# zamling/PSALM

Measured on AMD Instinct MI355X. Metric: images/sec at 1024x1024 COCO-panoptic inference, higher is better.
Workload: dtype f16x3; 1 GPU; BASELINE.json configs[1]: COCO-panoptic 1024x1024 batch=1 per GPU, PSALM (Swin-B + Phi-1.5 24L + Mask2Former head), 134 class prompts, 100 queries, full semantic+instance+panoptic post-processing; parallelism=image-sharded x1 (replicated weights, RCCL broadcast at init), launch=hipGraph replay (one graph per input signature)

## Files before the change

include/psalm_hip.h:

```cpp
#ifndef PSALM_HIP_H
#define PSALM_HIP_H
#include <stdint.h>
#ifdef __cplusplus
extern "C" {
#endif

#define PSALM_F32 0
#define PSALM_BF16 1

const char* psalm_last_error(void);
#define PSALM_ABI_VERSION 15
int psalm_abi_version(void);
const char* psalm_backend(void);

#define PSALM_TUNE_GEMM_XCD_KSPLIT 0
#define PSALM_TUNE_ATTN_XCD_HEADS 1
#define PSALM_TUNE_GEMM_MID 2
#define PSALM_TUNE_DECODER_FUSE 3
#define PSALM_TUNE_ROW_GROUPS 4
#define PSALM_TUNE_MHA_QTILE_WAVES 5
#define PSALM_TUNE_COUNT 8
int psalm_set_tuning(int key, int value);
int psalm_get_tuning(int key);

int psalm_msda_forward(const void* value, int value_dtype, const int64_t* spatial_shapes_host,
                       const int64_t* level_start_host, const float* sampling_loc, const float* attn_weight, void* out,
                       int out_dtype, int B, int S, int M, int D, int L, int Lq, int P, void* stream);
int psalm_msda_forward_dev(const void* value, int value_dtype, const int64_t* spatial_shapes_dev, const int64_t* level_start_dev,
                           const float* sampling_loc, const float* attn_weight, void* out, int out_dtype, int B, int S, int M, int D,
                           int L, int Lq, int P, void* stream);


int psalm_msda_fused(const void* value, int value_dtype, const int64_t* spatial_shapes_host,
                     const int64_t* level_start_host, const float* offsets_logits, void* out, int out_dtype, int B, int S,
                     int M, int D, int L, int P, void* stream);
int psalm_msda_set_policy(int v);


int psalm_gemm(const void* A, int a_dtype, long lda, const void* W, int w_dtype, long ldw, const float* bias,
               const void* residual, long ldr, void* C, int c_dtype, long ldc, int M, int N, int K, int act,
               int act_col_start, void* workspace, long workspace_bytes, void* stream);

int psalm_gemm_ln(const void* A, int a_dtype, long lda, const void* W, int w_dtype, long ldw, const float* bias,
                  const void* residual, long ldr, void* C, int c_dtype, long ldc, int M, int N, int K, int act, int act_col_start,
                  const float* ln_gamma, const float* ln_beta, float ln_eps, void* ln_out, int ln_dtype, long ld_ln, void* workspace,
                  long workspace_bytes, void* stream);
int psalm_conv2d_nhwc(const void* x, int B, int H, int W, int Cin, const void* Wt, int Cout, int ksize, int stride, int pad,
                      const float* bias, const void* residual, long ldr, void* out, int c_dtype, long ldc, int act,
                      const void* zeros, void* workspace, long workspace_bytes, void* stream);
int psalm_split_f16(const float* x, long ldx, void* out, long ldo, float* inv_scale, int rows, int K, void* stream);
int psalm_gemm_x3_set_products(int n);
int psalm_im2col_split_f16(const float* x, void* out, float* inv_scale, int B, int H, int W, int C, int k, int stride, int pad, void* stream);
int psalm_layernorm_split(const float* x, long ldx, float* y, long ldy, const float* gamma, const float* beta, int rows, int C, float eps,
                          void* split1, float* inv1, const float* add, long add_rows, void* split2, float* inv2, void* stream);
int psalm_swin_window_gather_split(const float* x, void* out, float* inv_out, const float* gamma, const float* beta, int B, int H, int W, int C,
                                   int ws, int shift, float eps, void* stream);
int psalm_swin_window_merge_ln_split(const float* win, const float* shortcut, float* out_x, void* h_split, float* h_inv, const float* gamma,
                                     const float* beta, int B, int H, int W, int C, int ws, int shift, float eps, void* stream);
int psalm_gemm_x3(const void* A2, long lda, const float* a_scale, const void* W2, long ldw, const float* w_scale, int Kp,
                  const float* bias, const void* residual, long ldr, void* C, long ldc, int M, int N, int act, int act_col_start,
                  void* workspace, long workspace_bytes, void* stream);
int psalm_gemm_x3_ln_split(const void* A2, long lda, const float* a_scale, const void* W2, long ldw, const float* w_scale, int Kp,
                           const float* bias, const void* residual, long ldr, void* C, long ldc, int M, int N, const float* ln_gamma,
                           const float* ln_beta, float ln_eps, void* ln_out, long ld_ln, void* split_out, float* split_inv,
                           void* workspace, long workspace_bytes, void* stream);
int psalm_gemm_x3_split(const void* A2, long lda, const float* a_scale, const void* W2, long ldw, const float* w_scale, int Kp,
                        const float* bias, void* C, long ldc, int M, int N, int act, int act_col_start, void* split_out, long ld_split,
                        int split_kp, int split_col_off, int split_col_start, int paired, float* split_inv, const float* bound_par,
                        int global_rows, void* workspace, long workspace_bytes, void* stream);

int psalm_image_preprocess(const unsigned char* img, int H, int W, float* out, unsigned char* pad_mask, int S, int nh, int nw,
                           const int* bounds_h, const int* kk_h, int ksize_h, const int* bounds_v, const int* kk_v, int ksize_v,
                           unsigned char* tmp, const float* mean3_host, const float* std3_host, void* stream);

int psalm_semantic_labels(const float* sem, int* labels, int C, long HW, void* stream);
int psalm_confusion_accumulate(const int* pred, const int* gt, long n, int num_classes, int ignore_label, long long* conf, void* stream);
int psalm_panoptic_rgb(const int* ids, unsigned char* rgb, long n, void* stream);
int psalm_mask_rle_count(const void* masks, int dtype_is_u8, int n, int H, int W, int* col_cnt, int* col_off, int* total, void* stream);
int psalm_mask_rle_emit(const void* masks, int dtype_is_u8, int n, int H, int W, const int* col_off, const long* base, int* out, void* stream);
int psalm_iou_counts(const void* pred, int pred_is_u8, const unsigned char* tgt, const int* pred_idx, const int* tgt_idx, int npairs, long HW,
                     long long* counts_zeroed, void* stream);
int psalm_fuse_masks(const void* masks, int dtype_is_u8, const float* scores, int n, long HW, float thr, unsigned char* out, void* stream);

long psalm_mha_attention_f32_workspace(int B, int heads, int Lq, int Lk);
int psalm_mha_attention_f32(const float* q, long ldq, const float* k, long ldk, const float* v, long ldv, float* out, long ldo,
                            const unsigned char* mask, const unsigned char* row_all_masked, void* workspace, int B, int Lq, int Lk, int heads,
                            int head_dim, void* stream);
long psalm_mha_attention_f32_shared_workspace(int B, int heads, int Lq, int Lk);
int psalm_mha_attention_f32_shared(const float* q, long ldq, const float* k, long ldk, const float* v, long ldv, float* out, long ldo,
                                   const unsigned char* mask, const unsigned char* row_all_masked, void* workspace, int B, int Lq, int Lk,
                                   int heads, int head_dim, void* stream);

long psalm_causal_attention_f32_workspace(int B, int L, int heads);
int psalm_causal_attention_f32(const float* qkv, long ld, int q_off, int k_off, int v_off, float* out, long ldo, int o_off,
                               const float* cos_table, const float* sin_table, const unsigned char* key_mask, void* workspace, int B, int L,
                               int heads, int head_dim, int rot, void* stream);
int psalm_causal_attention_f32_split(const float* qkv, long ld, int q_off, int k_off, int v_off, void* split_out, long ld_split, int split_kp,
                                     int split_col_off, const float* split_inv, const float* cos_table, const float* sin_table,
                                     const unsigned char* key_mask, void* workspace, int B, int L, int heads, int head_dim, int rot,
                                     void* stream);

long psalm_causal_attention_f32_prefix_workspace(int N, int S, int heads);
int psalm_causal_attention_f32_prefix(const float* qkv, long ld, int q_off, int k_off, int v_off, const float* k_cache, const float* v_cache,
                                      long ldv, float* out, long ldo, int o_off, const float* cos_table, const float* sin_table,
                                      const unsigned char* key_mask, void* workspace, int N, int S, int P, int heads, int head_dim, int rot,
                                      void* stream);
int psalm_causal_attention_f32_prefix_split(const float* qkv, long ld, int q_off, int k_off, int v_off, const float* k_cache,
                                            const float* v_cache, long ldv, void* split_out, long ld_split, int split_kp, int split_col_off,
                                            const float* split_inv, const float* cos_table, const float* sin_table,
                                            const unsigned char* key_mask, void* workspace, int N, int S, int P, int heads, int head_dim,
                                            int rot, void* stream);
typedef struct {
    const float* k_cache;
    const float* v_cache;
    long ldv;
    int P;
    int pad;
} psalm_prefix_ref;
long psalm_causal_attention_f32_prefix_grouped_workspace(int N, int S, int heads);
int psalm_causal_attention_f32_prefix_grouped(const float* qkv, long ld, int q_off, int k_off, int v_off, const psalm_prefix_ref* refs, int P_max,
                                              float* out, long ldo, int o_off, const float* cos_table, const float* sin_table,
                                              const unsigned char* key_mask, void* workspace, int N, int S, int heads, int head_dim, int rot,
                                              void* stream);
int psalm_causal_attention_f32_prefix_grouped_split(const float* qkv, long ld, int q_off, int k_off, int v_off, const psalm_prefix_ref* refs,
                                                    int P_max, void* split_out, long ld_split, int split_kp, int split_col_off,
                                                    const float* split_inv, const float* cos_table, const float* sin_table,
                                                    const unsigned char* key_mask, void* workspace, int N, int S, int heads, int head_dim,
                                                    int rot, void* stream);
int psalm_phi_prefix_kv_store(const float* qkv, long ld, int k_off, int v_off, const float* cos_table, const float* sin_table, float* k_cache,
                              float* v_cache, long ldv, int P, int heads, int head_dim, int rot, void* stream);

int psalm_memset_zero(void* p, long bytes, void* stream);
int psalm_copy_d2d(void* dst, const void* src, long bytes, void* stream);
int psalm_cast_i32_i64(const int* src, long long* dst, long n, void* stream);
const char* psalm_gemm_last_kernel(void);
int psalm_gemm_describe(int M, int N, int K, int a_dtype, int w_dtype, long workspace_bytes, int* out4);
int psalm_gemm_set_tile_policy(int bm);

int psalm_layernorm(const void* x, int x_dtype, long ldx, void* y, int y_dtype, long ldy, void* y2_bf16, long ldy2,
                    const float* gamma, const float* beta, int rows, int C, float eps, void* stream);
int psalm_layernorm3(const void* x, int x_dtype, long ldx, void* y, int y_dtype, long ldy, void* y2_bf16, long ldy2, const float* add,
                     long add_rows, void* y3_bf16, long ldy3, const float* gamma, const float* beta, int rows, int C, float eps,
                     void* stream);
int psalm_layernorm_chain(const float* x, long ldx, float* y1, long ldy1, const float* g1, const float* b1, const float* add, long add_rows,
                          float* y2, long ldy2, const float* g2, const float* b2, float* y3, long ldy3, int rows, int C, float eps, void* stream);
int psalm_gemm_f32_pair(const float* A0, const float* W0, const float* bias0, float* C0, int M0, int N0, int K0, int act0, const float* A1,
                        const float* W1, const float* bias1, float* C1, int M1, int N1, int K1, int act1, void* stream);
int psalm_gemm_f32_rows(const float* A, long lda, const float* W, long ldw, const float* bias, const float* residual, long ldr, float* C, long ldc,
                        int M, int N, int K, int act, void* stream);
int psalm_gemm_f32_rows_pair(const float* A0, const float* W0, const float* bias0, float* C0, int M0, int N0, int K0, int act0, const float* A1,
                             const float* W1, const float* bias1, float* C1, int M1, int N1, int K1, int act1, void* stream);
int psalm_gemm_f32_grouped(const float* const* A_host, const float* const* W_host, float* const* C_host, const int* M_host, const int* N_host, int K,
                           int count, void* stream);
int psalm_swin_window_gather(const void* x, int x_dtype, void* out, int out_dtype, const float* gamma,
                             const float* beta, int B, int H, int W, int C, int ws, int shift, float eps, void* stream);
int psalm_swin_window_merge(const void* win, int win_dtype, const void* shortcut, void* out, int x_dtype, int B, int H,
                            int W, int C, int ws, int shift, void* stream);
int psalm_swin_window_merge_ln(const void* win, int win_dtype, const float* shortcut, float* out_x, void* out_h, int h_dtype,
                               const float* gamma, const float* beta, int B, int H, int W, int C, int ws, int shift, float eps,
                               void* stream);
int psalm_patch_merge_ln(const void* x, int x_dtype, void* out, int out_dtype, const float* gamma, const float* beta,
                         int B, int H, int W, int C, float eps, void* stream);
int psalm_groupnorm_nhwc(const void* x, int x_dtype, void* y, int y_dtype, const float* gamma, const float* beta,
                         float* workspace, int B, int HW, int C, int G, float eps, int relu, void* stream);
int psalm_add_bcast(const void* a, int a_dtype, const void* b, int b_dtype, void* out, int out_dtype, long rows, int C,
                    long b_rows, void* stream);
int psalm_gather_rows(const void* src0, int dt0, const void* src1, int dt1, const void* src2, int dt2, const void* src3,
                      int dt3, const int* src_id, const int* src_row, void* dst, int dst_dtype, long rows, int C,
                      void* stream);
int psalm_segment_mean(const void* x, int x_dtype, long ldx, const int* seg_offsets, const int* seg_rows, void* out,
                       int out_dtype, int nseg, int C, void* stream);

int psalm_window_attention(const void* qkv, const float* bias_table, void* out, int dtype, int B, int nWh, int nWw, int C,
                           int heads, int ws, int shift, void* stream);
int psalm_window_attention_split(const float* qkv, const float* bias_table, const float* a_inv, const float* bound_par, void* split_out,
                                 int split_kp, float* split_inv, int B, int nWh, int nWw, int C, int heads, int ws, int shift, void* stream);
int psalm_window_attention_mfma(const void* qkv, const float* bias_table, void* out, int B, int nWh, int nWw, int C, int heads,
                                int ws, int shift, void* stream);
int psalm_causal_attention(const void* qkv, int dtype, long ld, int q_off, int k_off, int v_off, void* out, long ldo,
                           int o_off, const float* cos_table, const float* sin_table, const unsigned char* key_mask, int B,
                           int L, int heads, int head_dim, int rot, void* stream);
long psalm_causal_attention_mfma_workspace(int B, int L, int heads);
int psalm_causal_attention_mfma(const void* qkv, long ld, int q_off, int k_off, int v_off, void* out, long ldo, int o_off,
                                const float* cos_table, const float* sin_table, const unsigned char* key_mask,
                                void* workspace, int B, int L, int heads, int head_dim, int rot, void* stream);
int psalm_mha_attention(const void* q, long ldq, const void* k, long ldk, const void* v, long ldv, void* out, long ldo,
                        int dtype, const unsigned char* mask, const unsigned char* row_all_masked, int B, int Lq, int Lk,
                        int heads, int head_dim, void* stream);
long psalm_mha_attention_mfma_workspace(int B, int heads, int Lk);
int psalm_mha_attention_mfma(const void* q, long ldq, const void* k, long ldk, const void* vt, long ldvt, void* out, long ldo,
                             const unsigned char* mask, const unsigned char* row_all_masked, void* workspace, int B, int Lq,
                             int Lk, int heads, int head_dim, void* stream);
int psalm_attn_mask(const float* masks, unsigned char* out, unsigned char* row_all_masked, int BQ, int h, int w, int Ht,
                    int Wt, void* stream);

int psalm_patch_im2col(const float* img, void* out, int out_dtype, int B, int Cin, int H, int W, int ps, int Kpad,
                       void* stream);
int psalm_im2col_nhwc(const void* x, void* out, int dtype, int B, int H, int W, int C, int k, int stride, int pad,
                      void* stream);
int psalm_resize_planes(const void* in, int in_dtype, void* out, int out_dtype, long N, int h, int w, int hc, int wc, int H,
                        int W, void* stream);
int psalm_upsample_add_nhwc(const void* lateral, int lat_dtype, const void* small, int small_dtype, void* out, int out_dtype,
                            int B, int h, int w, int H, int W, int C, void* stream);
int psalm_permute_layout(const void* in, int in_dtype, void* out, int out_dtype, int B, int C, long HW, int to_nhwc,
                         void* stream);
int psalm_region_pool(const float* tokens, const int* img_of_region, const float* pts, float* out, int R, int h, int w, int C,
                      int n, void* stream);

int psalm_class_softmax(const float* cls, float* probs, void* probsT, int probsT_dtype, float* score, int* label, int Q, int C1,
                        int Kpad, void* stream);
int psalm_sigmoid_transpose(const float* mask, void* out, int out_dtype, int Q, long HW, int Kpad, void* stream);
int psalm_semantic_from_masks(const float* mask, const void* probsT_bf16, float* out, float* mask_score, float* workspace, int Q, int C,
                              long HW, int Kpad, void* stream);
int psalm_semantic_from_masks_x3(const float* mask, const float* probsT_f32, float* out, float* mask_score, float* workspace, int Q, int C,
                                 long HW, int Kpad, void* stream);
int psalm_mask_scores(const float* mask, float* score, float* workspace, int Q, long HW, void* stream);
int psalm_topk_select(const float* vals, int Q, int C, int stride, int k, const int* is_thing, const float* mask_score,
                      float* out_score, int* out_class, int* out_query, int* count, int apply_sigmoid, void* stream);
int psalm_binarize_gather(const float* mask, const int* query, const int* count, float* out, int n, long HW, void* stream);
int psalm_panoptic(const float* mask, const float* score, const int* label, const int* is_thing, int* argq, int* counts,
                   int* final_id, int* pan, int* info, int* ninfo, int Q, long HW, int num_classes, float obj_thr,
                   float overlap_thr, void* stream);
int psalm_region_scores(const float* logits, const float* mask_score, float* out, int K, int Q, void* stream);

typedef struct psalm_phi_layer {
    const void* w1; const float* w1_scale; const float* b1;
    const void* w2; const float* w2_scale; const float* b2;
    const float* ln_g; const float* ln_b;
    const float* bnd;
    int paired;
} psalm_phi_layer;
typedef struct psalm_phi_desc {
    int num_layers, hidden, intermediate, heads, head_dim, rot;
    float ln_eps;
    const psalm_phi_layer* layers;
    const float* final_g; const float* final_b;
} psalm_phi_desc;
long psalm_phi_forward_workspace(const psalm_phi_desc* d, int B, int L);
int psalm_phi_forward(const psalm_phi_desc* d, const float* embeds, const unsigned char* key_mask, const float* cos_table, const float* sin_table,
                      int B, int L, float* hidden_out, void* workspace, long workspace_bytes, void* gemm_workspace, long gemm_workspace_bytes,
                      void* stream);

long psalm_phi_prefix_cache_bytes(const psalm_phi_desc* d, int P);
long psalm_phi_prefix_cache_layer_bytes(int hidden, int heads, int P, long* k_bytes, long* v_bytes);
long psalm_phi_prefix_workspace(const psalm_phi_desc* d, int P);
int psalm_phi_prefix(const psalm_phi_desc* d, const float* embeds, const unsigned char* key_mask, const float* cos_table, const float* sin_table,
                     int P, void* cache, long cache_bytes, void* workspace, long workspace_bytes, void* gemm_workspace,
                     long gemm_workspace_bytes, void* stream);
long psalm_phi_suffix_workspace(const psalm_phi_desc* d, int N, int S);
int psalm_phi_suffix(const psalm_phi_desc* d, const float* embeds, const unsigned char* key_mask, const float* cos_table, const float* sin_table,
                     int N, int S, int P, const void* cache, long cache_bytes, float* hidden_out, void* workspace, long workspace_bytes,
                     void* gemm_workspace, long gemm_workspace_bytes, void* stream);
long psalm_phi_suffix_grouped_workspace(const psalm_phi_desc* d, int N, int S);
int psalm_phi_suffix_grouped(const psalm_phi_desc* d, const float* embeds, const unsigned char* key_mask, const float* cos_table,
                             const float* sin_table, int N, int S, const psalm_prefix_ref* refs, int P_max, float* hidden_out, void* workspace,
                             long workspace_bytes, void* gemm_workspace, long gemm_workspace_bytes, void* stream);

typedef struct psalm_swin_block {
    const float* n1_g; const float* n1_b; const float* n2_g; const float* n2_b;
    const void* qkv_w; const float* qkv_ws; const float* qkv_b; const float* qkv_bnd;
    const void* proj_w; const float* proj_ws; const float* proj_b;
    const void* fc1_w; const float* fc1_ws; const float* fc1_b; const float* fc1_bnd; int fc1_paired;
    const void* fc2_w; const float* fc2_ws; const float* fc2_b;
    const float* rpb;
} psalm_swin_block;
typedef struct psalm_swin_stage {
    int depth, heads, dim;
    const psalm_swin_block* blocks;
    const float* out_g; const float* out_b;
    const float* ds_g; const float* ds_b; const void* ds_w; const float* ds_ws;
} psalm_swin_stage;
typedef struct psalm_swin_desc {
    int num_stages, patch, window, pe_kpad, mlp_ratio;
    const void* pe_w; const float* pe_ws; const float* pe_b; const float* pe_ln_g; const float* pe_ln_b;
    const psalm_swin_stage* stages;
} psalm_swin_desc;
long psalm_swin_forward_workspace(const psalm_swin_desc* d, int B, int H, int W);
int psalm_swin_forward(const psalm_swin_desc* d, const float* images, int B, int H, int W, float* const* outs_host, void* workspace,
                       long workspace_bytes, void* gemm_workspace, long gemm_workspace_bytes, void* stream);

typedef struct psalm_projector_desc {
    int in_dim, mid_dim, out_dim;
    const void* c1_w; const float* c1_ws; const float* c1_b;
    const void* c2_w; const float* c2_ws;
    const void* c2f_w; const float* c2f_ws; const float* c2f_b;
    const void* ds_w; const float* ds_ws; const float* ds_b;
    const void* fc_w; const float* fc_ws; const float* fc_b;
} psalm_projector_desc;
long psalm_projector_forward_workspace(const psalm_projector_desc* d, int B, int h, int w);
int psalm_projector_forward(const psalm_projector_desc* d, const float* res5, int B, int h, int w, float* out, void* workspace, long workspace_bytes,
                            void* gemm_workspace, long gemm_workspace_bytes, void* stream);

typedef struct psalm_pd_enc_layer {
    const void* value_w; const float* value_ws; const float* value_b;
    const void* ow_w; const float* ow_ws; const float* ow_b;
    const void* out_w; const float* out_ws; const float* out_b;
    const float* n1_g; const float* n1_b;
    const void* l1_w; const float* l1_ws; const float* l1_b; const float* l1_bnd; int l1_paired;
    const void* l2_w; const float* l2_ws; const float* l2_b;
    const float* n2_g; const float* n2_b;
} psalm_pd_enc_layer;
typedef struct psalm_pd_desc {
    int D, G, M, num_layers, ffn, mask_dim;
    int in_dims[4];
    const void* ip_w[3]; const float* ip_ws[3]; const float* ip_b[3]; const float* ip_gn_g[3]; const float* ip_gn_b[3];
    const void* adapter_w; const float* adapter_ws; const float* adapter_b; const float* adapter_gn_g; const float* adapter_gn_b;
    const void* layer_w; const float* layer_ws; const float* layer_b; const float* layer_gn_g; const float* layer_gn_b;
    const void* mf_w; const float* mf_ws; const float* mf_b;
    const psalm_pd_enc_layer* layers;
} psalm_pd_desc;
long psalm_pixel_decoder_forward_workspace(const psalm_pd_desc* d, const int* hw_host);
int psalm_pixel_decoder_forward(const psalm_pd_desc* d, const float* const* feats_host, const int* hw_host, const float* lvl_pos, float* mask_features,
                                float* ms_out, void* workspace, long workspace_bytes, void* gemm_workspace, long gemm_workspace_bytes, void* stream);

typedef struct psalm_pr_layer {
    const float* cq_w; const float* cq_b; const float* co_w; const float* co_b; const float* cn_g; const float* cn_b;
    const float* sqk_w; const float* sqk_b; const float* sv_w; const float* sv_b; const float* so_w; const float* so_b; const float* sn_g; const float* sn_b;
    const float* f1_w; const float* f1_b; const float* f2_w; const float* f2_b; const float* fn_g; const float* fn_b;
} psalm_pr_layer;
typedef struct psalm_pr_desc {
    int D, heads, Q, num_layers, num_levels, ffn, mask_dim;
    const void* lvl_k_w[3]; const float* lvl_k_ws[3]; const float* lvl_k_b[3];
    const void* lvl_v_w[3]; const float* lvl_v_ws[3]; const float* lvl_v_b[3];
    const float* level_embed; const float* query_embed; const float* dn_g; const float* dn_b;
// ... 82 lines not shown
```

psalm_amd/csrc/api.hip:

```cpp
#include "common.h"
#include "psalm_hip.h"

#include <atomic>
#include <cstring>

static thread_local char g_err[512] = "";

extern "C" void psalm_set_error(const char* msg) {
    strncpy(g_err, msg ? msg : "", sizeof(g_err) - 1);
    g_err[sizeof(g_err) - 1] = 0;
}
extern "C" const char* psalm_last_error() { return g_err; }
static std::atomic<int> g_tuning[PSALM_TUNE_COUNT] = {{1}, {1}, {1}, {1}, {1}, {1}, {0}, {0}};
extern "C" int psalm_set_tuning(int key, int value) {
    if (key < 0 || key >= PSALM_TUNE_COUNT) { psalm_set_error("psalm_set_tuning: unknown key"); return -1; }
    g_tuning[key].store(value, std::memory_order_relaxed);
    return 0;
}
extern "C" int psalm_get_tuning(int key) {
    if (key < 0 || key >= PSALM_TUNE_COUNT) return 0;
    return g_tuning[key].load(std::memory_order_relaxed);
}
extern "C" int psalm_abi_version() { return PSALM_ABI_VERSION; }
extern "C" const char* psalm_backend() {
#ifdef PSALM_EMU_BUILD
    return "emu";
#else
    return "hip-gfx950";
#endif
}

extern "C" int psalm_memset_zero(void* p, long bytes, void* stream) {
    if (bytes <= 0) return 0;
    PSALM_CHECK_ARG(p != nullptr, "psalm_memset_zero: null pointer");
    hipError_t e = hipMemsetAsync(p, 0, (size_t)bytes, (hipStream_t)stream);
    if (e != hipSuccess) { psalm_set_error("psalm_memset_zero: hipMemsetAsync failed"); return (int)e; }
    return 0;
}
__global__ void cast_i32_i64_kernel(const int* __restrict__ src, long long* __restrict__ dst, long n) {
    const long i = (long)blockIdx.x * blockDim.x + threadIdx.x;
    if (i < n) dst[i] = (long long)src[i];
}
extern "C" int psalm_cast_i32_i64(const int* src, long long* dst, long n, void* stream) {
    if (n <= 0) return 0;
    PSALM_CHECK_ARG(dst != nullptr && src != nullptr, "psalm_cast_i32_i64: null pointer");
    hipLaunchKernelGGL(cast_i32_i64_kernel, dim3((unsigned)((n + 255) / 256)), dim3(256), 0, (hipStream_t)stream, src, dst, n);
    PSALM_LAUNCH_END("psalm_cast_i32_i64");
}
extern "C" int psalm_copy_d2d(void* dst, const void* src, long bytes, void* stream) {
    if (bytes <= 0) return 0;
    PSALM_CHECK_ARG(dst != nullptr && src != nullptr, "psalm_copy_d2d: null pointer");
    hipError_t e = hipMemcpyAsync(dst, src, (size_t)bytes, hipMemcpyDeviceToDevice, (hipStream_t)stream);
    if (e != hipSuccess) { psalm_set_error("psalm_copy_d2d: hipMemcpyAsync failed"); return (int)e; }
    return 0;
}
```

psalm_amd/csrc/attention.hip:

```cpp
#include "common.h"
#include "psalm_hip.h"
#include <cstdlib>

template <typename T, int HD>
__global__ void __launch_bounds__(192) window_attention_kernel(const T* __restrict__ qkv, const float* __restrict__ bias_table,
                                                               T* __restrict__ out, int nWh, int nWw, int C, int heads, int ws,
                                                               int shift) {
    HIP_DYNAMIC_SHARED(float, smem)
    const int N = ws * ws;
    float* Ks = smem;
    float* Vs = Ks + N * (HD + 1);
    float* Bs = Vs + N * (HD + 1);
    const int win = blockIdx.x, h = blockIdx.y, tid = threadIdx.x;
    const int nbias = (2 * ws - 1) * (2 * ws - 1);
    const long row0 = (long)win * N;
    for (int e = tid; e < N * HD; e += blockDim.x) {
        const int r = e / HD, c = e % HD;
        const T* p = qkv + (row0 + r) * 3 * C + h * HD + c;
        Ks[r * (HD + 1) + c] = ldf(p + C);
        Vs[r * (HD + 1) + c] = ldf(p + 2 * C);
    }
    for (int e = tid; e < nbias; e += blockDim.x) Bs[e] = bias_table[(long)e * heads + h];
    __syncthreads();
    if (tid >= N) return;
// ... 525 lines not shown
            for (int r = 0; r < 16; ++r) {
                const float p = sacc[r] > -1.0e38f ? __expf(sacc[r] - mn) : 0.f;
                sacc[r] = p;
                psum += p;
            }
            psum += __shfl_xor(psum, 32);
            l = l * alpha + psum;
            m = mn;
#pragma unroll
            for (int r = 0; r < 16; ++r) { o0[r] *= alpha; o1[r] *= alpha; }
            {
                const float* v0 = &Vt[buf][n32 * VS + 4 * hi];
                const float* v1 = &Vt[buf][(32 + n32) * VS + 4 * hi];
#pragma unroll
                for (int g = 0; g < 4; ++g) {
                    const psalm_f32x4 a0 = *reinterpret_cast<const psalm_f32x4*>(v0 + 8 * g);
                    const psalm_f32x4 a1 = *reinterpret_cast<const psalm_f32x4*>(v1 + 8 * g);
                    o0 = __builtin_amdgcn_mfma_f32_32x32x2f32(a0.x, sacc[4 * g], o0, 0, 0, 0);
                    o1 = __builtin_amdgcn_mfma_f32_32x32x2f32(a1.x, sacc[4 * g], o1, 0, 0, 0);
                    o0 = __builtin_amdgcn_mfma_f32_32x32x2f32(a0.y, sacc[4 * g + 1], o0, 0, 0, 0);
                    o1 = __builtin_amdgcn_mfma_f32_32x32x2f32(a1.y, sacc[4 * g + 1], o1, 0, 0, 0);
                    o0 = __builtin_amdgcn_mfma_f32_32x32x2f32(a0.z, sacc[4 * g + 2], o0, 0, 0, 0);
                    o1 = __builtin_amdgcn_mfma_f32_32x32x2f32(a1.z, sacc[4 * g + 2], o1, 0, 0, 0);
                    o0 = __builtin_amdgcn_mfma_f32_32x32x2f32(a0.w, sacc[4 * g + 3], o0, 0, 0, 0);
                    o1 = __builtin_amdgcn_mfma_f32_32x32x2f32(a1.w, sacc[4 * g + 3], o1, 0, 0, 0);
                }
            }
        }
        if (kt + 1 < ntiles) stage(buf ^ 1);
        __syncthreads();
    }
    if (qi < L) {
        const float inv = l > 0.f ? 1.f / l : 0.f;
        float* op = out + (tok0 + qi) * ldo + o_off + h * HD + 4 * hi;
#pragma unroll
        for (int g = 0; g < 4; ++g) {
            *reinterpret_cast<psalm_f32x4*>(op + 8 * g) = psalm_f32x4{o0[4 * g] * inv, o0[4 * g + 1] * inv, o0[4 * g + 2] * inv, o0[4 * g + 3] * inv};
            *reinterpret_cast<psalm_f32x4*>(op + 32 + 8 * g) = psalm_f32x4{o1[4 * g] * inv, o1[4 * g + 1] * inv, o1[4 * g + 2] * inv, o1[4 * g + 3] * inv};
        }
    }
}

template <bool GR = false>
__global__ void __launch_bounds__(256) phi_rope_prep_f32_kernel(const float* __restrict__ base, long ld, int q_off, int k_off,
                                                                const float* __restrict__ cosT, const float* __restrict__ sinT,
                                                                const unsigned char* __restrict__ key_mask, float* __restrict__ Qr,
                                                                float* __restrict__ Kr, unsigned char* __restrict__ Mk,
                                                                unsigned char* __restrict__ Tk, int L, int Lp, int heads, float scale,
                                                                const psalm_prefix_ref* __restrict__ refs) {
    constexpr int HD = 64, ROT = 32, half = 16;
    const int h = blockIdx.y, b = blockIdx.z;
    long pos0 = 0;
    if constexpr (GR) pos0 = refs[b].P;
    const int t = blockIdx.x * 32 + (threadIdx.x >> 3), c0 = (threadIdx.x & 7) * 8;
    if (t >= Lp) return;
    float* qd = Qr + (((long)b * heads + h) * Lp + t) * HD + c0;
    float* kd = Kr + (((long)b * heads + h) * Lp + t) * HD + c0;
    __shared__ int tile_all;
    if (h == 0) {
        const bool valid = t < L && key_mask[(long)b * L + min(t, L - 1)] != 0;
        if (threadIdx.x == 0) tile_all = 1;
        __syncthreads();
        if (c0 == 0) {
            if (t < Lp) Mk[(long)b * Lp + t] = valid ? 1 : 0;
            if (!valid) tile_all = 0;
        }
        __syncthreads();
        if (threadIdx.x == 0) Tk[(long)b * (Lp / 32) + blockIdx.x] = tile_all ? 1 : 0;
    }
    float q[8], k[8];
    if (t < L) {
        const float* p = base + ((long)b * L + t) * ld;
        ld8(p + q_off + h * HD + c0, q);
        ld8(p + k_off + h * HD + c0, k);
        if (c0 < ROT) {
            float qo[8], ko[8], cs[8], sn[8];
            const int oc = c0 < half ? c0 + half : c0 - half;
            ld8(p + q_off + h * HD + oc, qo);
            ld8(p + k_off + h * HD + oc, ko);
            ld8(cosT + (pos0 + t) * ROT + c0, cs);
            ld8(sinT + (pos0 + t) * ROT + c0, sn);
#pragma unroll
            for (int i = 0; i < 8; ++i) {
                q[i] = q[i] * cs[i] + (c0 < half ? -qo[i] : qo[i]) * sn[i];
                k[i] = k[i] * cs[i] + (c0 < half ? -ko[i] : ko[i]) * sn[i];
            }
        }
#pragma unroll
        for (int i = 0; i < 8; ++i) q[i] *= scale;
    } else {
#pragma unroll
        for (int i = 0; i < 8; ++i) { q[i] = 0.f; k[i] = 0.f; }
    }
    st8(qd, q);
    st8(kd, k);
}

template <bool SO>
__global__ void __launch_bounds__(256) PSALM_WAVES_PER_EU(3)
causal_attention_f32_splitk_kernel(const float* __restrict__ Qr, const float* __restrict__ Kr, const unsigned char* __restrict__ Mk,
                                   const unsigned char* __restrict__ Tk, const float* __restrict__ base, long ld, int v_off, float* out, long ldo,
                                   int o_off, int L, int Lp, int heads, const float* __restrict__ so_inv, int so_kp, int pair, int xcd_heads) {
    typedef float f32x16 __attribute__((ext_vector_type(16)));
    constexpr int HD = 64, OS = HD + 4;
    __shared__ __attribute__((aligned(16))) float Os[4][32 * OS];
    __shared__ float Ml[4][2][32];
    const int tid = threadIdx.x, lane = tid & 63, wave = tid >> 6, n32 = lane & 31, hi = lane >> 5;
    const int nqt = Lp / 32;
    int bx = blockIdx.x, h = blockIdx.y, b = blockIdx.z;
    if (xcd_heads) {
        const int lin = (int)(blockIdx.x + gridDim.x * (blockIdx.y + gridDim.y * blockIdx.z));
        const int j = lin >> 3, hb = (lin & 7) + 8 * (j / (int)gridDim.x);
        bx = j % (int)gridDim.x;
        h = hb % heads;
        b = hb / heads;
    }
    const long bh = (long)b * heads + h;
    const int npass = pair ? ((int)(nqt - 1 - bx) > bx ? 2 : 1) : 1;
    for (int pass = 0; pass < npass; ++pass) {
    const int qt = pair ? (pass == 0 ? nqt - 1 - bx : bx) : (int)(gridDim.x - 1 - bx);
    const int w0 = pass ? 3 - wave : wave;
    if (pass) __syncthreads();
    const int qi = qt * 32 + n32;
    float qv[32];
    {
        const float* p = Qr + (bh * Lp + qi) * HD + 32 * hi;
#pragma unroll
        for (int c = 0; c < 32; c += 4) {
            const psalm_f32x4 t = *reinterpret_cast<const psalm_f32x4*>(p + c);
            qv[c] = t.x; qv[c + 1] = t.y; qv[c + 2] = t.z; qv[c + 3] = t.w;
        }
    }
    f32x16 o0, o1;
#pragma unroll
    for (int r = 0; r < 16; ++r) { o0[r] = 0.f; o1[r] = 0.f; }
    float m = -3.0e38f, l = 0.f;
    const psalm_rsrc vrs = psalm_make_rsrc(base + (long)b * L * ld + v_off + h * HD, (unsigned)((((long)L - 1) * ld + HD) * 4));
    const unsigned vvo = (unsigned)((4L * hi * ld + n32) * 4);
    const unsigned vrow = (unsigned)(ld * 4);
    const psalm_rsrc krs = psalm_make_rsrc(Kr + bh * Lp * HD, (unsigned)((long)Lp * HD * 4));
    const unsigned kvo = (unsigned)((n32 * HD + 32 * hi) * 4);
    const int nkt = Lp / 32;
    for (int kt = __builtin_amdgcn_readfirstlane(w0); kt <= qt; kt += 4) {
        psalm_f32x4 kf[8];
#pragma unroll
        for (int c = 0; c < 8; ++c) {
            const psalm_u32x4 t = psalm_buf_load_b128_s(krs, kvo + 16u * c, (unsigned)(kt * 32 * HD * 4));
            kf[c] = psalm_f32x4{__builtin_bit_cast(float, t.x), __builtin_bit_cast(float, t.y), __builtin_bit_cast(float, t.z), __builtin_bit_cast(float, t.w)};
        }
        float va[16], vb[16];
#pragma unroll
        for (int g = 0; g < 4; ++g)
#pragma unroll
            for (int i = 0; i < 4; ++i) {
                const unsigned so_ = (unsigned)(kt * 32 + 8 * g + i) * vrow;
                va[4 * g + i] = psalm_buf_load_f32_s(vrs, vvo, so_);
                vb[4 * g + i] = psalm_buf_load_f32_s(vrs, vvo + 128u, so_);
            }
        const bool plain = __builtin_amdgcn_readfirstlane((int)(kt < qt && Tk[(long)b * nkt + kt] != 0)) != 0;
        f32x16 sacc;
#pragma unroll
        for (int r = 0; r < 16; ++r) sacc[r] = 0.f;
#pragma unroll
        for (int c = 0; c < 8; ++c) {
            sacc = __builtin_amdgcn_mfma_f32_32x32x2f32(kf[c].x, qv[4 * c], sacc, 0, 0, 0);
            sacc = __builtin_amdgcn_mfma_f32_32x32x2f32(kf[c].y, qv[4 * c + 1], sacc, 0, 0, 0);
            sacc = __builtin_amdgcn_mfma_f32_32x32x2f32(kf[c].z, qv[4 * c + 2], sacc, 0, 0, 0);
            sacc = __builtin_amdgcn_mfma_f32_32x32x2f32(kf[c].w, qv[4 * c + 3], sacc, 0, 0, 0);
        }
        float mc = -3.0e38f, mn, alpha, psum = 0.f;
        if (plain) {
#pragma unroll
            for (int r = 0; r < 16; ++r) mc = fmaxf(mc, sacc[r]);
            mc = fmaxf(mc, __shfl_xor(mc, 32));
            mn = fmaxf(m, mc);
            alpha = __expf(m - mn);
#pragma unroll
            for (int r = 0; r < 16; ++r) {
// ... 60 lines not shown
                const psalm_f32x4 c = *reinterpret_cast<const psalm_f32x4*>(&Os[w][q * OS + d0 + 4]);
                acc[0] += a.x * f; acc[1] += a.y * f; acc[2] += a.z * f; acc[3] += a.w * f;
                acc[4] += c.x * f; acc[5] += c.y * f; acc[6] += c.z * f; acc[7] += c.w * f;
            }
            const float inv = Lsum > 0.f ? 1.f / Lsum : 0.f;
#pragma unroll
            for (int i = 0; i < 8; ++i) acc[i] *= inv;
            if constexpr (SO) {
                const long row = (long)b * L + tq;
                const float sc = 1.f / so_inv[row];
                unsigned hw[4], lw[4];
#pragma unroll
                for (int k = 0; k < 4; ++k) {
                    unsigned h0, h1, l0, l1;
                    psalm_split_words(acc[2 * k] * sc, h0, l0);
                    psalm_split_words(acc[2 * k + 1] * sc, h1, l1);
                    hw[k] = h0 | (h1 << 16);
                    lw[k] = l0 | (l1 << 16);
                }
                unsigned short* d = reinterpret_cast<unsigned short*>(out) + row * ldo + o_off + h * HD + d0;
                *reinterpret_cast<psalm_u32x4*>(d) = psalm_u32x4{hw[0], hw[1], hw[2], hw[3]};
                *reinterpret_cast<psalm_u32x4*>(d + so_kp) = psalm_u32x4{lw[0], lw[1], lw[2], lw[3]};
            } else {
                st8(out + ((long)b * L + tq) * ldo + o_off + h * HD + d0, acc);
            }
        }
    }
    }
}

extern "C" long psalm_causal_attention_f32_workspace(int B, int L, int heads) {
    const long Lp = (L + 31) / 32 * 32;
    return 2L * B * heads * Lp * 64 * (long)sizeof(float) + (long)B * Lp + (long)B * (Lp / 32) + 64;
}

static int causal_attention_f32_impl(const float* qkv, long ld, int q_off, int k_off, int v_off, void* out, long ldo, int o_off,
                                     const float* cos_table, const float* sin_table, const unsigned char* key_mask, void* workspace,
                                     int B, int L, int heads, int head_dim, int rot, void* stream, const float* so_inv, int so_kp,
                                     const char* name) {
    PSALM_CHECK_ARG(head_dim == 64 && rot == 32, "psalm_causal_attention_f32: head_dim 64, rotary dim 32 (Phi-1.5)");
    PSALM_CHECK_ARG(ld % 4 == 0 && q_off % 4 == 0 && k_off % 4 == 0 && v_off % 4 == 0 && (uintptr_t)qkv % 16 == 0 &&
                        (uintptr_t)out % 16 == 0 && workspace && (uintptr_t)workspace % 16 == 0 &&
                        (so_inv ? (ldo % 8 == 0 && o_off % 8 == 0 && so_kp % 8 == 0) : (ldo % 4 == 0 && o_off % 4 == 0)),
                    "psalm_causal_attention_f32: 16-byte aligned rows / offsets and a workspace");
    if (B == 0 || L == 0) return 0;
    const int Lp = (L + 31) / 32 * 32;
    float* Qr = (float*)workspace;
    float* Kr = Qr + (long)B * heads * Lp * 64;
    unsigned char* Mk = (unsigned char*)(Kr + (long)B * heads * Lp * 64);
    unsigned char* Tk = Mk + (long)B * Lp;
    PSALM_CHECK_ARG(((long)L - 1) * ld * 4 + 256 < 0x7fffffffL, "psalm_causal_attention_f32: L * ld * 4 must stay below 2 GiB (buffer-descriptor fetches)");
    const float scale = 1.0f / sqrtf((float)head_dim);
    hipStream_t s = (hipStream_t)stream;
    hipLaunchKernelGGL(phi_rope_prep_f32_kernel<false>, dim3(Lp / 32, heads, B), dim3(256), 0, s, qkv, ld, q_off, k_off, cos_table, sin_table, key_mask,
                       Qr, Kr, Mk, Tk, L, Lp, heads, scale, (const psalm_prefix_ref*)nullptr);
    const int pair = 1;
    const int nqt = Lp / 32;
    const dim3 grid(pair ? (nqt + 1) / 2 : nqt, heads, B);
    const int xcd_heads = ((heads * B) % 8 == 0 && psalm_get_tuning(PSALM_TUNE_ATTN_XCD_HEADS)) ? 1 : 0;
    if (so_inv)
        hipLaunchKernelGGL(causal_attention_f32_splitk_kernel<true>, grid, dim3(256), 0, s, (const float*)Qr, (const float*)Kr,
                           (const unsigned char*)Mk, (const unsigned char*)Tk, qkv, ld, v_off, (float*)out, ldo, o_off, L, Lp, heads, so_inv, so_kp, pair, xcd_heads);
    else
        hipLaunchKernelGGL(causal_attention_f32_splitk_kernel<false>, grid, dim3(256), 0, s, (const float*)Qr, (const float*)Kr,
                           (const unsigned char*)Mk, (const unsigned char*)Tk, qkv, ld, v_off, (float*)out, ldo, o_off, L, Lp, heads, (const float*)nullptr, 0, pair, xcd_heads);
    PSALM_LAUNCH_END(name);
}
extern "C" int psalm_causal_attention_f32(const float* qkv, long ld, int q_off, int k_off, int v_off, float* out, long ldo, int o_off,
                                          const float* cos_table, const float* sin_table, const unsigned char* key_mask, void* workspace,
                                          int B, int L, int heads, int head_dim, int rot, void* stream) {
    return causal_attention_f32_impl(qkv, ld, q_off, k_off, v_off, out, ldo, o_off, cos_table, sin_table, key_mask, workspace, B, L, heads,
                                     head_dim, rot, stream, nullptr, 0, "psalm_causal_attention_f32");
}
extern "C" int psalm_causal_attention_f32_split(const float* qkv, long ld, int q_off, int k_off, int v_off, void* split_out, long ld_split,
                                                int split_kp, int split_col_off, const float* split_inv, const float* cos_table,
                                                const float* sin_table, const unsigned char* key_mask, void* workspace, int B, int L,
                                                int heads, int head_dim, int rot, void* stream) {
    PSALM_CHECK_ARG(split_out && split_inv && ld_split >= 2L * split_kp && split_col_off + heads * 64 <= split_kp,
                    "psalm_causal_attention_f32_split: split buffer rows of >= 2*split_kp f16 and the row scales");
    return causal_attention_f32_impl(qkv, ld, q_off, k_off, v_off, split_out, ld_split, split_col_off, cos_table, sin_table, key_mask, workspace,
                                     B, L, heads, head_dim, rot, stream, split_inv, split_kp, "psalm_causal_attention_f32_split");
}

__global__ void __launch_bounds__(256) phi_prefix_kv_store_kernel(const float* __restrict__ base, long ld, int k_off, int v_off,
                                                                  const float* __restrict__ cosT, const float* __restrict__ sinT,
                                                                  float* __restrict__ Kc, float* __restrict__ Vc, long ldv, int P, int Pp, int heads) {
    constexpr int HD = 64, ROT = 32, half = 16;
    const int h = blockIdx.y;
    const int t = blockIdx.x * 32 + (threadIdx.x >> 3), c0 = (threadIdx.x & 7) * 8;
    if (t >= Pp) return;
    float* kd = Kc + ((long)h * Pp + t) * HD + c0;
    float k[8];
    if (t < P) {
        const float* p = base + (long)t * ld;
        ld8(p + k_off + h * HD + c0, k);
        if (c0 < ROT) {
            float ko[8], cs[8], sn[8];
            const int oc = c0 < half ? c0 + half : c0 - half;
            ld8(p + k_off + h * HD + oc, ko);
            ld8(cosT + (long)t * ROT + c0, cs);
            ld8(sinT + (long)t * ROT + c0, sn);
#pragma unroll
            for (int i = 0; i < 8; ++i) k[i] = k[i] * cs[i] + (c0 < half ? -ko[i] : ko[i]) * sn[i];
        }
        float v[8];
        ld8(p + v_off + h * HD + c0, v);
        st8(Vc + (long)t * ldv + h * HD + c0, v);
    } else {
#pragma unroll
        for (int i = 0; i < 8; ++i) k[i] = 0.f;
    }
    st8(kd, k);
}

extern "C" int psalm_phi_prefix_kv_store(const float* qkv, long ld, int k_off, int v_off, const float* cos_table, const float* sin_table,
                                         float* k_cache, float* v_cache, long ldv, int P, int heads, int head_dim, int rot, void* stream) {
    PSALM_CHECK_ARG(head_dim == 64 && rot == 32, "psalm_phi_prefix_kv_store: head_dim 64, rotary dim 32 (Phi-1.5)");
    PSALM_CHECK_ARG(qkv && cos_table && sin_table && k_cache && v_cache && P >= 1 && heads >= 1, "psalm_phi_prefix_kv_store: null argument / empty prefix");
    PSALM_CHECK_ARG(ld % 4 == 0 && k_off % 4 == 0 && v_off % 4 == 0 && ldv % 4 == 0 && ldv >= (long)heads * 64 && (uintptr_t)qkv % 16 == 0 &&
                        (uintptr_t)k_cache % 16 == 0 && (uintptr_t)v_cache % 16 == 0,
                    "psalm_phi_prefix_kv_store: 16-byte aligned rows / offsets, v_cache rows of >= heads * 64 floats");
    const int Pp = (P + 31) / 32 * 32;
    hipLaunchKernelGGL(phi_prefix_kv_store_kernel, dim3(Pp / 32, heads), dim3(256), 0, (hipStream_t)stream, qkv, ld, k_off, v_off, cos_table,
                       sin_table, k_cache, v_cache, ldv, P, Pp, heads);
    PSALM_LAUNCH_END("psalm_phi_prefix_kv_store");
}

template <bool SO, bool GR = false>
__global__ void __launch_bounds__(256) PSALM_WAVES_PER_EU(3)
causal_attention_f32_prefix_kernel(const float* __restrict__ Qr, const float* __restrict__ Kr, const unsigned char* __restrict__ Mk,
                                   const unsigned char* __restrict__ Tk, const float* __restrict__ base, long ld, int v_off,
                                   const float* __restrict__ Kc_, const float* __restrict__ Vc_, long ldv_, int P_, int Pp_, float* out, long ldo,
                                   int o_off, int S, int Sp, int heads, const float* __restrict__ so_inv, int so_kp, int xcd_heads,
                                   const psalm_prefix_ref* __restrict__ refs) {
    typedef float f32x16 __attribute__((ext_vector_type(16)));
    constexpr int HD = 64, OS = HD + 4;
    __shared__ __attribute__((aligned(16))) float Os[4][32 * OS];
    __shared__ float Ml[4][2][32];
    const int tid = threadIdx.x, lane = tid & 63, wave = tid >> 6, n32 = lane & 31, hi = lane >> 5;
    const int nqt = Sp / 32;
    int bx = blockIdx.x, h = blockIdx.y, b = blockIdx.z;
    if (xcd_heads) {
        const int lin = (int)(blockIdx.x + gridDim.x * (blockIdx.y + gridDim.y * blockIdx.z));
        const int j = lin >> 3, hb = (lin & 7) + 8 * (j / (int)gridDim.x);
        bx = j % (int)gridDim.x;
        h = hb % heads;
        b = hb / heads;
    }
    const float* Kc = Kc_;
    const float* Vc = Vc_;
    long ldv = ldv_;
    int P = P_, Pp = Pp_;
    if constexpr (GR) {
        const psalm_prefix_ref r = refs[b];
        Kc = r.k_cache;
        Vc = r.v_cache;
        ldv = r.ldv;
        P = r.P;
        Pp = (P + 31) / 32 * 32;
    }
    const int npt = Pp / 32;
    const long bh = (long)b * heads + h;
    const int qt = nqt - 1 - bx;
    const int qi = qt * 32 + n32;
    float qv[32];
    {
        const float* p = Qr + (bh * Sp + qi) * HD + 32 * hi;
#pragma unroll
        for (int c = 0; c < 32; c += 4) {
            const psalm_f32x4 t = *reinterpret_cast<const psalm_f32x4*>(p + c);
            qv[c] = t.x; qv[c + 1] = t.y; qv[c + 2] = t.z; qv[c + 3] = t.w;
        }
    }
    f32x16 o0, o1;
#pragma unroll
    for (int r = 0; r < 16; ++r) { o0[r] = 0.f; o1[r] = 0.f; }
    float m = -3.0e38f, l = 0.f;
    auto tile = [&](const bool pre, const psalm_rsrc krs, const psalm_rsrc vrs, const unsigned vvo, const unsigned vrow, const int kt) {
        const unsigned kvo = (unsigned)((n32 * HD + 32 * hi) * 4);
        psalm_f32x4 kf[8];
#pragma unroll
        for (int c = 0; c < 8; ++c) {
            const psalm_u32x4 t = psalm_buf_load_b128_s(krs, kvo + 16u * c, (unsigned)(kt * 32 * HD * 4));
            kf[c] = psalm_f32x4{__builtin_bit_cast(float, t.x), __builtin_bit_cast(float, t.y), __builtin_bit_cast(float, t.z), __builtin_bit_cast(float, t.w)};
        }
        float va[16], vb[16];
// ... 748 lines not shown
```

psalm_amd/csrc/common.h:

```cpp
#pragma once
#include <hip/hip_runtime.h>

#include <cstdint>
#include <cstdio>

#define PSALM_F32 0
#define PSALM_BF16 1

typedef unsigned short bf16_t;

__device__ __forceinline__ float bf16_to_f32(bf16_t v) {
    unsigned u = ((unsigned)v) << 16;
    return __builtin_bit_cast(float, u);
}
__device__ __forceinline__ bf16_t f32_to_bf16(float f) {
    unsigned u = __builtin_bit_cast(unsigned, f);
    u += 0x7fffu + ((u >> 16) & 1u);
    return (bf16_t)(u >> 16);
}
typedef float psalm_f32x2_v __attribute__((ext_vector_type(2)));
typedef __bf16 psalm_bf16x2_v __attribute__((ext_vector_type(2)));
__device__ __forceinline__ unsigned pack_bf16x2(float a, float b) {
    const psalm_f32x2_v v = {a, b};
    return __builtin_bit_cast(unsigned, __builtin_convertvector(v, psalm_bf16x2_v));
// ... 12 lines not shown
}
__device__ __forceinline__ void ld8(const bf16_t* p, float* d) {
    const psalm_u32x4 a = *reinterpret_cast<const psalm_u32x4*>(p);
    const unsigned w[4] = {a.x, a.y, a.z, a.w};
#pragma unroll
    for (int i = 0; i < 4; ++i) {
        d[2 * i] = __builtin_bit_cast(float, w[i] << 16);
        d[2 * i + 1] = __builtin_bit_cast(float, w[i] & 0xffff0000u);
    }
}
__device__ __forceinline__ void st8(float* p, const float* v) {
    reinterpret_cast<psalm_f32x4*>(p)[0] = psalm_f32x4{v[0], v[1], v[2], v[3]};
    reinterpret_cast<psalm_f32x4*>(p)[1] = psalm_f32x4{v[4], v[5], v[6], v[7]};
}
__device__ __forceinline__ void st8(bf16_t* p, const float* v) {
    *reinterpret_cast<psalm_u32x4*>(p) =
        psalm_u32x4{pack_bf16x2(v[0], v[1]), pack_bf16x2(v[2], v[3]), pack_bf16x2(v[4], v[5]), pack_bf16x2(v[6], v[7])};
}

__device__ __forceinline__ float wave_sum(float v) {
#pragma unroll
    for (int o = 32; o > 0; o >>= 1) v += __shfl_xor(v, o);
    return v;
}
__device__ __forceinline__ float wave_max(float v) {
#pragma unroll
    for (int o = 32; o > 0; o >>= 1) v = fmaxf(v, __shfl_xor(v, o));
    return v;
}

template <int LPR> __device__ __forceinline__ float seg_sum(float v) {
#pragma unroll
    for (int o = LPR / 2; o > 0; o >>= 1) v += __shfl_xor(v, o);
    return v;
}
template <int LPR> __device__ __forceinline__ float seg_max(float v) {
#pragma unroll
    for (int o = LPR / 2; o > 0; o >>= 1) v = fmaxf(v, __shfl_xor(v, o));
    return v;
}

#ifdef PSALM_EMU_BUILD
#define PSALM_WAVES_PER_EU(n)
#else
#define PSALM_WAVES_PER_EU(n) __attribute__((amdgpu_waves_per_eu(n)))
#endif
#ifdef PSALM_EMU_BUILD
__device__ __forceinline__ void psalm_glds16(const void* g, void* lds_wave_base) { emu::global_load_lds(g, lds_wave_base, 16); }
#else
__device__ __forceinline__ void psalm_glds16(const void* g, void* lds_wave_base) {
    __builtin_amdgcn_global_load_lds((const __attribute__((address_space(1))) void*)g,
                                     (__attribute__((address_space(3))) void*)lds_wave_base, 16, 0, 0);
}
#endif

#ifdef PSALM_EMU_BUILD
#define PSALM_WAIT_VMCNT(N) do { } while (0)
#define PSALM_RAW_BARRIER() __syncthreads()
#define PSALM_SCHED_FENCE() do { } while (0)
#define PSALM_OPAQUE_VGPR(x) do { } while (0)
#define PSALM_OPAQUE_SGPR(x) do { } while (0)
__device__ __forceinline__ float psalm_rcp(float x) { return 1.0f / x; }
__device__ __forceinline__ float psalm_exp2(float x) { return exp2f(x); }
#else
#define PSALM_OPAQUE_VGPR(x) asm volatile("" : "+v"(x))
#define PSALM_OPAQUE_SGPR(x) asm volatile("" : "+s"(x))
#define PSALM_WAIT_VMCNT(N) asm volatile("s_waitcnt vmcnt(" #N ")" ::: "memory")
#define PSALM_RAW_BARRIER() do { asm volatile("s_waitcnt lgkmcnt(0)" ::: "memory"); __builtin_amdgcn_s_barrier(); } while (0)
#define PSALM_SCHED_FENCE() __builtin_amdgcn_sched_barrier(0)
__device__ __forceinline__ float psalm_rcp(float x) { return __builtin_amdgcn_rcpf(x); }
__device__ __forceinline__ float psalm_exp2(float x) { return __builtin_amdgcn_exp2f(x); }
#endif

__device__ __forceinline__ void psalm_split_words(float y, unsigned& hw, unsigned& sw) {
    const _Float16 h = (_Float16)y;
    hw = (unsigned)__builtin_bit_cast(unsigned short, h);
    sw = (unsigned)__builtin_bit_cast(unsigned short, (_Float16)(y - (float)h));
}

#define PSALM_BUF_OOB 0x80000000u
#ifdef PSALM_EMU_BUILD
__device__ __forceinline__ unsigned psalm_swap_adjacent(unsigned v) { return __shfl_xor(v, 1); }
__device__ __forceinline__ unsigned psalm_quad_swap2(unsigned v) { return __shfl_xor(v, 2); }
template <int P> __device__ __forceinline__ unsigned psalm_quad_bcast(unsigned v) { return __shfl(v, ((threadIdx.x & 63) & ~3) | P); }
struct psalm_rsrc { char* base; unsigned bytes; };
__device__ __forceinline__ psalm_rsrc psalm_make_rsrc(const void* p, unsigned bytes) { return psalm_rsrc{(char*)p, bytes}; }
__device__ __forceinline__ void psalm_buf_store_f32(float v, psalm_rsrc r, unsigned off) { if (off < r.bytes && r.bytes - off >= 4u) *reinterpret_cast<float*>(r.base + off) = v; }
__device__ __forceinline__ void psalm_buf_store_u32(unsigned v, psalm_rsrc r, unsigned off) { if (off < r.bytes && r.bytes - off >= 4u) *reinterpret_cast<unsigned*>(r.base + off) = v; }
__device__ __forceinline__ float psalm_buf_load_f32(psalm_rsrc r, unsigned off) { return (off < r.bytes && r.bytes - off >= 4u) ? *reinterpret_cast<const float*>(r.base + off) : 0.f; }
__device__ __forceinline__ psalm_u32x4 psalm_buf_load_b128(psalm_rsrc r, unsigned off) {
    return (off < r.bytes && r.bytes - off >= 16u) ? *reinterpret_cast<const psalm_u32x4*>(r.base + off) : psalm_u32x4{0u, 0u, 0u, 0u};
}
__device__ __forceinline__ void psalm_buf_store_f32_s(float v, psalm_rsrc r, unsigned voff, unsigned soff) { if (voff < PSALM_BUF_OOB) psalm_buf_store_f32(v, r, voff + soff); }
__device__ __forceinline__ float psalm_buf_load_f32_s(psalm_rsrc r, unsigned voff, unsigned soff) { return voff < PSALM_BUF_OOB ? psalm_buf_load_f32(r, voff + soff) : 0.f; }
__device__ __forceinline__ psalm_u32x4 psalm_buf_load_b128_s(psalm_rsrc r, unsigned voff, unsigned soff) {
    return voff < PSALM_BUF_OOB ? psalm_buf_load_b128(r, voff + soff) : psalm_u32x4{0u, 0u, 0u, 0u};
}
#else
__device__ __forceinline__ unsigned psalm_swap_adjacent(unsigned v) {
    return (unsigned)__builtin_amdgcn_mov_dpp((int)v, 0xB1, 0xF, 0xF, true);
}
__device__ __forceinline__ unsigned psalm_quad_swap2(unsigned v) {
    return (unsigned)__builtin_amdgcn_mov_dpp((int)v, 0x4E, 0xF, 0xF, true);
}
template <int P> __device__ __forceinline__ unsigned psalm_quad_bcast(unsigned v) {
    return (unsigned)__builtin_amdgcn_mov_dpp((int)v, P * 0x55, 0xF, 0xF, true);
}
typedef __amdgpu_buffer_rsrc_t psalm_rsrc;
__device__ __forceinline__ psalm_rsrc psalm_make_rsrc(const void* p, unsigned bytes) {
    return __builtin_amdgcn_make_buffer_rsrc(const_cast<void*>(p), 0, (int)bytes, 0x00020000);
}
__device__ __forceinline__ void psalm_buf_store_f32(float v, psalm_rsrc r, unsigned off) {
    __builtin_amdgcn_raw_buffer_store_b32(__builtin_bit_cast(unsigned, v), r, (int)off, 0, 0);
}
__device__ __forceinline__ void psalm_buf_store_u32(unsigned v, psalm_rsrc r, unsigned off) { __builtin_amdgcn_raw_buffer_store_b32(v, r, (int)off, 0, 0); }
__device__ __forceinline__ float psalm_buf_load_f32(psalm_rsrc r, unsigned off) {
    return __builtin_bit_cast(float, __builtin_amdgcn_raw_buffer_load_b32(r, (int)off, 0, 0));
}
typedef unsigned psalm_u32x4_v __attribute__((ext_vector_type(4)));
__device__ __forceinline__ psalm_u32x4 psalm_buf_load_b128(psalm_rsrc r, unsigned off) {
    const psalm_u32x4_v v = __builtin_amdgcn_raw_buffer_load_b128(r, (int)off, 0, 0);
    return psalm_u32x4{v.x, v.y, v.z, v.w};
}
__device__ __forceinline__ void psalm_buf_store_f32_s(float v, psalm_rsrc r, unsigned voff, unsigned soff) {
    __builtin_amdgcn_raw_buffer_store_b32(__builtin_bit_cast(unsigned, v), r, (int)voff, (int)soff, 0);
}
__device__ __forceinline__ float psalm_buf_load_f32_s(psalm_rsrc r, unsigned voff, unsigned soff) {
    return __builtin_bit_cast(float, __builtin_amdgcn_raw_buffer_load_b32(r, (int)voff, (int)soff, 0));
}
__device__ __forceinline__ psalm_u32x4 psalm_buf_load_b128_s(psalm_rsrc r, unsigned voff, unsigned soff) {
    const psalm_u32x4_v v = __builtin_amdgcn_raw_buffer_load_b128(r, (int)voff, (int)soff, 0);
    return psalm_u32x4{v.x, v.y, v.z, v.w};
}
#endif

extern "C" void psalm_set_error(const char* msg);
extern "C" int psalm_get_tuning(int key);
#ifndef PSALM_TUNE_COUNT
#define PSALM_TUNE_GEMM_XCD_KSPLIT 0
#define PSALM_TUNE_ATTN_XCD_HEADS 1
#define PSALM_TUNE_GEMM_MID 2
#define PSALM_TUNE_DECODER_FUSE 3
#define PSALM_TUNE_ROW_GROUPS 4
#define PSALM_TUNE_MHA_QTILE_WAVES 5
#define PSALM_TUNE_COUNT 8
#endif

#define PSALM_CHECK_ARG(cond, msg)                                  \
    do {                                                            \
        if (!(cond)) { psalm_set_error(msg); return -1; }           \
    } while (0)

#define PSALM_LAUNCH_END(name)                                      \
    do {                                                            \
        hipError_t e__ = hipGetLastError();                         \
        if (e__ != hipSuccess) {                                    \
            char buf__[256];                                        \
            snprintf(buf__, sizeof(buf__), "%s: launch failed: %s", name, hipGetErrorString(e__)); \
            psalm_set_error(buf__);                                 \
            return (int)e__ ? (int)e__ : -2;                        \
        }                                                           \
        return 0;                                                   \
    } while (0)

#define PSALM_DISPATCH(code, T, ...)                                \
    do {                                                            \
        if ((code) == PSALM_F32) { typedef float T; __VA_ARGS__; }  \
        else if ((code) == PSALM_BF16) { typedef bf16_t T; __VA_ARGS__; } \
        else { psalm_set_error("bad dtype code"); return -1; }      \
    } while (0)

static inline int cdiv(long a, long b) { return (int)((a + b - 1) / b); }
```

psalm_amd/csrc/gemm.hip:

```cpp
#include "common.h"
#include <algorithm>
#include <atomic>
#include <cstring>
#include <type_traits>

#define ACT_NONE 0
#define ACT_RELU 1
#define ACT_GELU 2
#define ACT_GELU_NEW 3
#define ACT_POST_RESIDUAL 16
#define ACT_BIAS_ROW 32

#ifdef PSALM_GEMM_TIMELINE
__device__ unsigned long long* g_psalm_tl = nullptr;
extern "C" int psalm_gemm_timeline_buffer(void* p) { return (int)hipMemcpyToSymbol(HIP_SYMBOL(g_psalm_tl), &p, sizeof(p)); }
#define PSALM_TL(i)                                                                                                                      \
    do {                                                                                                                                 \
        if (g_psalm_tl && threadIdx.x == 0)                                                                                              \
            g_psalm_tl[((size_t)blockIdx.y * gridDim.x + blockIdx.x) * 8 + (i)] = __builtin_amdgcn_s_memrealtime();                    \
    } while (0)
#define PSALM_TL_DRAIN() asm volatile("s_waitcnt vmcnt(0)" ::: "memory")
__device__ int g_psalm_ablate = 0;
extern "C" int psalm_gemm_ablate(int v) { return (int)hipMemcpyToSymbol(HIP_SYMBOL(g_psalm_ablate), &v, sizeof(v)); }
#define PSALM_ABL() g_psalm_ablate
#else
#define PSALM_TL(i) do { } while (0)
#define PSALM_TL_DRAIN() do { } while (0)
#define PSALM_ABL() 0
#endif

typedef float f32x16 __attribute__((ext_vector_type(16)));
typedef __bf16 bf16x8 __attribute__((ext_vector_type(8)));
typedef _Float16 f16x8 __attribute__((ext_vector_type(8)));
struct alignas(16) u32x4_s { unsigned x, y, z, w; };
struct alignas(8) u32x2_s { unsigned x, y; };
struct alignas(16) f32x4_g { float x, y, z, w; };

__device__ __forceinline__ float psalm_erff(float a) {
    const float t = fabsf(a), s = a * a;
    float r = fmaf(-1.72853470e-5f, t, 3.83197126e-4f);
    const float u = fmaf(-3.88396438e-3f, t, 2.42546219e-2f);
    r = fmaf(r, s, u);
    r = fmaf(r, t, -1.06777877e-1f);
    r = fmaf(r, t, -6.34846687e-1f);
    r = fmaf(r, t, -1.28717512e-1f);
    r = fmaf(r, t, -t);
    r = copysignf(1.0f - __expf(r), a);
    float q = -5.96761703e-4f;
    q = fmaf(q, s, 4.99119423e-3f);
    q = fmaf(q, s, -2.67681349e-2f);
    q = fmaf(q, s, 1.12819925e-1f);
    q = fmaf(q, s, -3.76125336e-1f);
    q = fmaf(q, s, 1.28379166e-1f);
    q = fmaf(q, a, a);
    return t > 0.927734375f ? r : q;
}

__device__ __forceinline__ float apply_act(float v, int act) {
    if (act == ACT_RELU) return fmaxf(v, 0.f);
    if (act == ACT_GELU) { const float hv = 0.5f * v; return fmaf(hv, psalm_erff(v * 0.70710678118654752440f), hv); }
    if (act == ACT_GELU_NEW) {
        const float p = fmaf(v * v, -0.10294324f, -2.3022082f);
        return v * psalm_rcp(1.f + psalm_exp2(v * p));
    }
    return v;
}

template <int A> __device__ __forceinline__ float apply_act_t(float v, int act_rt) { return apply_act(v, A < 0 ? act_rt : A); }
template <int V> struct psalm_ic { static constexpr int value = V; };

__device__ __forceinline__ unsigned pack2(float a, float b) { return pack_bf16x2(a, b); }

__device__ __forceinline__ u32x4_s load8_bf16(const bf16_t* p, bool ok) {
    if (!ok) return u32x4_s{0, 0, 0, 0};
    return *reinterpret_cast<const u32x4_s*>(p);
}
__device__ __forceinline__ u32x4_s load8_bf16(const float* p, bool ok) {
    if (!ok) return u32x4_s{0, 0, 0, 0};
    const f32x4_g a = *reinterpret_cast<const f32x4_g*>(p);
    const f32x4_g b = *reinterpret_cast<const f32x4_g*>(p + 4);
    return u32x4_s{pack2(a.x, a.y), pack2(a.z, a.w), pack2(b.x, b.y), pack2(b.z, b.w)};
}

// ... 94 lines not shown
#pragma unroll
        for (int i = 0; i < B_CHUNKS; ++i) {
            const int c = tid + 256 * i, row = c >> 2, kc = (c & 3) * 8;
            *reinterpret_cast<u32x4_s*>(&Bs[buf][row * LDS_STRIDE + kc]) = rb[i];
        }
    };

    const int nk = (g.K + BK - 1) / BK;
    gload(0);
    lstore(0);
    __syncthreads();
    for (int kt = 0; kt < nk; ++kt) {
        const int buf = kt & 1;
        if (kt + 1 < nk) gload((kt + 1) * BK);
#pragma unroll
        for (int ks = 0; ks < 2; ++ks) {
            bf16x8 af[TM], bfr[2];
            const int koff = ks * 16 + 8 * (lane >> 5);
#pragma unroll
            for (int i = 0; i < TM; ++i) {
                const int row = wm * (BM / 2) + i * 32 + (lane & 31);
                af[i] = __builtin_bit_cast(bf16x8, *reinterpret_cast<const u32x4_s*>(&As[buf][row * LDS_STRIDE + koff]));
            }
#pragma unroll
            for (int j = 0; j < 2; ++j) {
                const int row = wn * 64 + j * 32 + (lane & 31);
                bfr[j] = __builtin_bit_cast(bf16x8, *reinterpret_cast<const u32x4_s*>(&Bs[buf][row * LDS_STRIDE + koff]));
            }
#pragma unroll
            for (int i = 0; i < TM; ++i)
#pragma unroll
                for (int j = 0; j < 2; ++j)
                    acc[i][j] = __builtin_amdgcn_mfma_f32_32x32x16_bf16(af[i], bfr[j], acc[i][j], 0, 0, 0);
        }
        if (kt + 1 < nk) lstore(buf ^ 1);
        __syncthreads();
    }
#pragma unroll
    for (int i = 0; i < TM; ++i)
#pragma unroll
        for (int j = 0; j < 2; ++j)
            epilogue_store<TC>(g, acc[i][j], bm + wm * (BM / 2) + i * 32, bn + wn * 64 + j * 32 + (lane & 31), lane);
}


__device__ __forceinline__ void load8_f32(const float* p, float* d) {
    const f32x4_g a = reinterpret_cast<const f32x4_g*>(p)[0], b = reinterpret_cast<const f32x4_g*>(p)[1];
    d[0] = a.x; d[1] = a.y; d[2] = a.z; d[3] = a.w; d[4] = b.x; d[5] = b.y; d[6] = b.z; d[7] = b.w;
}
__device__ __forceinline__ void load8_f32(const bf16_t* p, float* d) {
    const u32x4_s a = *reinterpret_cast<const u32x4_s*>(p);
    const unsigned w[4] = {a.x, a.y, a.z, a.w};
#pragma unroll
    for (int i = 0; i < 4; ++i) {
        d[2 * i] = __builtin_bit_cast(float, w[i] << 16);
        d[2 * i + 1] = __builtin_bit_cast(float, w[i] & 0xffff0000u);
    }
}
__device__ __forceinline__ void store8(float* p, const float* v) {
    reinterpret_cast<f32x4_g*>(p)[0] = f32x4_g{v[0], v[1], v[2], v[3]};
    reinterpret_cast<f32x4_g*>(p)[1] = f32x4_g{v[4], v[5], v[6], v[7]};
}
__device__ __forceinline__ void store8(bf16_t* p, const float* v) {
    *reinterpret_cast<u32x4_s*>(p) = u32x4_s{pack2(v[0], v[1]), pack2(v[2], v[3]), pack2(v[4], v[5]), pack2(v[6], v[7])};
}

struct GemmFastArgs {
    GemmArgs g;
    float* slab;
    int k_per_split;
    int vec_store;
    int cH, cW, cC, cK, cS, cP, cHo, cWo;
    const bf16_t* zeros;
    const float* a_scale;
    const float* w_scale;
    int x3_kp;
    unsigned short* so = nullptr;
    long ldso = 0;
    int so_kp = 0, so_col_off = 0, so_col_start = 0, so_global = 0;
    int so_paired = 0;
    float* so_inv = nullptr;
    const float* so_par = nullptr;
    int xcd_ksplit = 0;
};
__device__ __forceinline__ void split_scale_from_bound(float bound, float& sc, float& inv) {
    bound = fminf(fmaxf(bound, 7.888609e-31f), 1.2676506e30f);
    const unsigned eb = (__builtin_bit_cast(unsigned, bound) >> 23) & 0xffu;
    sc = __builtin_bit_cast(float, (266u - eb) << 23);
    inv = __builtin_bit_cast(float, (eb - 12u) << 23);
}

template <int N> __device__ __forceinline__ void wait_vmcnt_le() {
    static_assert(N == 0 || N == 4 || N == 6 || N == 8 || N == 12 || N == 16 || N == 18 || N == 24, "add the literal");
    if constexpr (N == 0) PSALM_WAIT_VMCNT(0);
    else if constexpr (N == 4) PSALM_WAIT_VMCNT(4);
    else if constexpr (N == 6) PSALM_WAIT_VMCNT(6);
    else if constexpr (N == 8) PSALM_WAIT_VMCNT(8);
    else if constexpr (N == 12) PSALM_WAIT_VMCNT(12);
    else if constexpr (N == 16) PSALM_WAIT_VMCNT(16);
    else if constexpr (N == 18) PSALM_WAIT_VMCNT(18);
    else PSALM_WAIT_VMCNT(24);
}

template <typename TC, int BM, int BN, int WM, int WN, int NS, bool CONV = false, int BK = 64, int PH8_ = 0, int X3 = 0,
          bool SO = false, bool PAIR = false>
__global__ void __launch_bounds__(64 * (WM * WN + (PH8_ == 6 ? 2 : (PH8_ == 7 ? 4 : 0)))) gemm_bf16_glds_kernel(GemmFastArgs fa) {
    constexpr int PH8 = (PH8_ >= 1 && PH8_ <= 4) ? PH8_ : 0;
    constexpr int NLW = PH8_ == 6 ? 2 : (PH8_ == 7 ? 4 : 0);
    constexpr bool LW = NLW > 0;
    static_assert(PH8_ >= 0 && PH8_ <= 7 && PH8_ != 5, "PH8_: 0 generic loop, 1 - 4 phased 256 x 256 loops, 6 / 7 loader waves");
    static_assert(!LW || (X3 == 2 && (NS == 3 || NS == 2) && BK == 32 && !CONV), "LW: slice form on 32-deep slices, three (or two) stages");
    static_assert(!PAIR || SO, "paired stores: a form of the split-f16 output");
    static_assert(!SO || X3 == 1 || (X3 == 2 && BK == 32 && (NS == 2 || LW)), "split-f16 output: K-panel form, or 32-deep slices in two stages (three with loader waves)");
    static_assert(X3 >= 0 && X3 <= 2, "X3: 0 bf16 operands, 1 split-f16 K-panel form, 2 split-f16 slice form");
    static_assert(!PH8 || (BM == 256 && BN == 256 && WM == 2 && WN == 4 && NS == 2 && (BK == 64 || (BK == 32 && X3 == 2 && (PH8 == 3 || PH8 == 4))) && !CONV), "PH8 configuration");
    static_assert(!X3 || !CONV, "split-f16 variants: plain GEMM");
    static_assert(X3 != 1 || BK == 64, "split-f16 K-panel form: 64-deep K tiles");
    static_assert(X3 != 2 || ((!PH8 && (BK == 64 || BK == 32)) || ((PH8 == 3 || PH8 == 4) && BK == 32)), "split-f16 slice form: generic K loop, or the phased 256 x 256 loop on 32-deep slices");
    constexpr int XS = X3 == 2 ? 2 : 1;
    const GemmArgs& g = fa.g;
    constexpr int NW = WM * WN, NT = 64 * NW;
    constexpr int TM = BM / WM / 32, TN = BN / WN / 32;
    constexpr int RPC = 512 / BK;
    constexpr int SLOTS = BK / 8;
    constexpr int SWS = BK == 128 ? 0 : (BK == 64 ? 1 : 2);
    static_assert(BK == 128 || BK == 64 || BK == 32, "BK");
    static_assert(!CONV || BK == 64, "implicit-GEMM convolution uses 64-deep K tiles");
    constexpr int NCW = LW ? NLW : NW;
    constexpr int A_CH = BM / RPC / NCW, B_CH = BN / RPC / NCW;
    static_assert(A_CH >= 1 && B_CH >= 1 && TM >= 1 && TN >= 1, "tile / wave configuration");
    constexpr int SMEM_BYTES = NS * (BM + BN) * BK * 2 * XS;
    constexpr int EP = (BM * BN * 4 > SMEM_BYTES) ? WM : 1;
    static_assert(BM / EP * BN * 4 <= SMEM_BYTES, "epilogue slab must fit in the operand buffers");
    static_assert(NS >= 2 && NS <= 4, "ring depth");
    __shared__ __attribute__((aligned(16))) bf16_t smem[NS][(BM + BN) * BK * XS];

    const int tid = threadIdx.x, lane = tid & 63;
    PSALM_TL(0);
    const int wave = (PH8 || LW) ? __builtin_amdgcn_readfirstlane(tid >> 6) : tid >> 6;
    const int cw = LW ? max(wave - NW, 0) : wave;
    const int wm = wave / WN, wn = wave % WN;
    int tile, ksl;
    if (fa.xcd_ksplit) {
        const int lin = blockIdx.x + gridDim.x * blockIdx.y;
        ksl = lin % (int)gridDim.y;
        tile = lin / (int)gridDim.y;
    } else {
        tile = xcd_remap(blockIdx.x, g.tiles_m * g.tiles_n);
        ksl = blockIdx.y;
    }
    const int bm = (g.row_fast ? tile % g.tiles_m : tile / g.tiles_n) * BM;
    const int bn = (g.row_fast ? tile / g.tiles_m : tile % g.tiles_n) * BN;
    const int kbeg = ksl * fa.k_per_split;
    const int kend = min(g.K, kbeg + fa.k_per_split);
    const bf16_t* A = (const bf16_t*)g.A;
    const bf16_t* W = (const bf16_t*)g.W;

    constexpr bool PHS = PH8 != 0 && X3 == 2;
    auto a_chunk = [&](int i) -> int {
        if constexpr (PHS) return 4 * i + (wave & 3) + 8 * (wave >> 2);
        else return cw + NCW * i;
    };
    const bf16_t* asrc[A_CH];
    const bf16_t* bsrc[B_CH];
    const int lrow = lane / SLOTS, slot = lane % SLOTS;
    int ay[A_CH], ax[A_CH];
// ... 372 lines not shown
#undef PH8_BAR
    } else {
#pragma unroll
    for (int p = 0; p < NS - 1; ++p)
        if (p < nk) issue(p, p * BK);
    PSALM_TL(1);
    for (int kt = 0; kt < nk; ++kt) {
        const int buf = kt % NS;
        if constexpr (NS == 2) {
            wait_vmcnt_le<0>();
        } else {
            const int ahead = min(nk - 1 - kt, NS - 2);
            if (NS >= 4 && ahead >= 2) wait_vmcnt_le<(NS >= 4 ? 2 * LPT : 0)>();
            else if (ahead >= 1) wait_vmcnt_le<LPT>();
            else wait_vmcnt_le<0>();
        }
        if (!(PSALM_ABL() & 8)) PSALM_RAW_BARRIER();
        if (kt == 0) PSALM_TL(2);
        if (kt + NS - 1 < nk && !(PSALM_ABL() & 1)) issue((kt + NS - 1) % NS, (kt + NS - 1) * BK);
        const bf16_t* As = smem[buf];
        const bf16_t* Bs = smem[buf] + BM * BK;
        bf16x8 af[2][TM], bfr[2][TN];
        auto load_frags = [&](int kk, int slot_) {
            const int co = ((2 * kk + hi) ^ fsw) * 8;
#pragma unroll
            for (int i = 0; i < TM; ++i)
                af[slot_][i] = __builtin_bit_cast(bf16x8, *reinterpret_cast<const u32x4_s*>(&As[(a_row0 + 32 * i) * BK + co]));
#pragma unroll
            for (int j = 0; j < TN; ++j)
                bfr[slot_][j] = __builtin_bit_cast(bf16x8, *reinterpret_cast<const u32x4_s*>(&Bs[(b_row0 + 32 * j) * BK + co]));
        };
        if constexpr (X3 == 2) {
            const bf16_t* Al = As + (BM + BN) * BK;
            const bf16_t* Bl = Al + BM * BK;
#pragma unroll
            for (int kk = 0; kk < BK / 16; ++kk) {
                const int co = ((2 * kk + hi) ^ fsw) * 8;
                bf16x8 ah[TM] = {}, al[TM] = {}, bh[TN] = {}, bl[TN] = {};
                if (!(PSALM_ABL() & 2)) {
#pragma unroll
                    for (int i = 0; i < TM; ++i) {
                        ah[i] = __builtin_bit_cast(bf16x8, *reinterpret_cast<const u32x4_s*>(&As[(a_row0 + 32 * i) * BK + co]));
                        al[i] = __builtin_bit_cast(bf16x8, *reinterpret_cast<const u32x4_s*>(&Al[(a_row0 + 32 * i) * BK + co]));
                    }
#pragma unroll
                    for (int j = 0; j < TN; ++j) {
                        bh[j] = __builtin_bit_cast(bf16x8, *reinterpret_cast<const u32x4_s*>(&Bs[(b_row0 + 32 * j) * BK + co]));
                        bl[j] = __builtin_bit_cast(bf16x8, *reinterpret_cast<const u32x4_s*>(&Bl[(b_row0 + 32 * j) * BK + co]));
                    }
                }
                if (PSALM_ABL() & 4) continue;
#pragma unroll
                for (int i = 0; i < TM; ++i)
#pragma unroll
                    for (int j = 0; j < TN; ++j) {
                        acc[i][j] = mma16(ah[i], bh[j], acc[i][j]);
                        acc[i][j] = mma16(al[i], bh[j], acc[i][j]);
                        acc[i][j] = mma16(ah[i], bl[j], acc[i][j]);
                    }
            }
            continue;
        }
        constexpr bool PIN = (TM * TN <= 4);
        load_frags(0, 0);
#pragma unroll
        for (int kk = 0; kk < BK / 16; ++kk) {
            if (kk + 1 < BK / 16) load_frags(kk + 1, (kk + 1) & 1);
            if constexpr (PIN) __builtin_amdgcn_sched_barrier(0);
#pragma unroll
            for (int i = 0; i < TM; ++i)
#pragma unroll
                for (int j = 0; j < TN; ++j)
                    acc[i][j] = mma16(af[kk & 1][i], bfr[kk & 1][j], acc[i][j]);
        }
    }
    }
    PSALM_TL(3);
    if constexpr (std::is_same<TC, float>::value) {
        const bool split = fa.slab != nullptr;
        const int act = g.act & 15;
        bool lds_path = !split && ((act != ACT_NONE && act != ACT_RELU && bn + BN > g.act_col_start) || (g.act & ACT_BIAS_ROW) != 0);
        if constexpr (SO) lds_path = lds_path || (fa.so != nullptr && bn + BN > fa.so_col_start);
        if (!lds_path) {
            const bool post = (g.act & ACT_POST_RESIDUAL) != 0;
            float* Cb = split ? fa.slab + (long)ksl * g.M * g.N : (float*)g.C;
            const long ldo = split ? (long)g.N : g.ldc;
            const int rows_here = min(g.M - bm, BM);
            const psalm_rsrc rc = psalm_make_rsrc(Cb + (long)bm * ldo, (unsigned)min((long)rows_here * ldo * 4, 0x7ffff000L));
            const float* R = split ? nullptr : (const float*)g.res;
            const psalm_rsrc rr = psalm_make_rsrc(R ? R + (long)bm * g.ldr : Cb, R ? (unsigned)min((long)rows_here * g.ldr * 4, 0x7ffff000L) : 0u);
            float wsc[TN], bias_c[TN];
            unsigned coff[TN];
            bool actc[TN];
#pragma unroll
            for (int j = 0; j < TN; ++j) {
                const int col = bn + wn * (BN / WN) + j * 32 + n32;
                const bool ok = col < g.N;
                coff[j] = ok ? (unsigned)col * 4u : PSALM_BUF_OOB;
                if constexpr (EPF) {
                    wsc[j] = pf_wsc[j];
                    bias_c[j] = pf_bias[j];
                } else {
                    wsc[j] = 1.f;
                    if constexpr (X3) wsc[j] = fa.w_scale[min(col, g.N - 1)];
                    bias_c[j] = (!split && g.bias) ? g.bias[min(col, g.N - 1)] : 0.f;
                }
                actc[j] = !split && act != ACT_NONE && col >= g.act_col_start;
            }
            auto row_off = [&](int i, int r) { return wm * (BM / WM) + i * 32 + 4 * hi + (r & 3) + 8 * (r >> 2); };
            float asc[16], rv[16];
#pragma unroll
            for (int r = 0; r < 16; ++r) {
                if constexpr (EPF) asc[r] = pf_asc[r];
                else {
                    asc[r] = 1.f;
                    if constexpr (X3) asc[r] = fa.a_scale[min(bm + row_off(0, r), g.M - 1)];
                }
                rv[r] = psalm_buf_load_f32(rr, (unsigned)((long)row_off(0, r) * g.ldr * 4) + coff[0]);
            }
#pragma unroll
            for (int t = 0; t < TM * TN; ++t) {
                const int i = t / TN, j = t % TN, i2 = (t + 1) / TN, j2 = (t + 1) % TN;
                float x[16];
#pragma unroll
                for (int r = 0; r < 16; ++r) {
                    x[r] = acc[i][j][r];
                    if constexpr (X3) x[r] = fmaf(x[r], asc[r] * wsc[j], bias_c[j]);
                    else x[r] += bias_c[j];
                    if (actc[j] && !post) x[r] = fmaxf(x[r], 0.f);
                    x[r] += rv[r];
                    if (actc[j] && post) x[r] = fmaxf(x[r], 0.f);
                }
                if (t + 1 < TM * TN) {
#pragma unroll
                    for (int r = 0; r < 16; ++r) {
                        if constexpr (X3) { if (j2 == 0) asc[r] = fa.a_scale[min(bm + row_off(i2, r), g.M - 1)]; }
                        rv[r] = psalm_buf_load_f32(rr, (unsigned)((long)row_off(i2, r) * g.ldr * 4) + coff[j2]);
                    }
                }
#pragma unroll
                for (int r = 0; r < 16; ++r) psalm_buf_store_f32(x[r], rc, (unsigned)((long)row_off(i, r) * ldo * 4) + coff[j]);
            }
            PSALM_TL(4);
            PSALM_TL_DRAIN();
            PSALM_TL(5);
            return;
        }
    }
    __syncthreads();
    if constexpr (SO) {
        if (fa.so != nullptr && bn + BN > fa.so_col_start) {
            constexpr int EPS = (BM * BN * 4 > SMEM_BYTES) ? 2 : 1;
            static_assert(TM % EPS == 0 && BM / EPS * BN * 4 <= SMEM_BYTES, "split-output epilogue: pass geometry");
            constexpr int TMP = TM / EPS, ROWS_P = BM / EPS, BAND = ROWS_P / WM;
            constexpr int TPR = BN / 8, RPI = NT / TPR, NIT = ROWS_P / RPI;
            unsigned* Cw = reinterpret_cast<unsigned*>(&smem[0][0]);
            const int act = g.act & 15;
            float gmax = 0.f;
            if (fa.so_global) {
                for (int r0 = 0; r0 < g.M; r0 += 512) {
                    float t8[8];
#pragma unroll
                    for (int k = 0; k < 8; ++k) t8[k] = fa.a_scale[min(r0 + 64 * k + lane, g.M - 1)];
#pragma unroll
                    for (int k = 0; k < 8; ++k) gmax = fmaxf(gmax, t8[k]);
                }
// ... 1249 lines not shown
    for (int c = sub * 8; c < Kp; c += LPR * 8) {
        float v[8];
        if (c < K) load8_f32(xr + c, v);
        else {
#pragma unroll
            for (int k = 0; k < 8; ++k) v[k] = 0.f;
        }
        unsigned hw[4], lw[4];
#pragma unroll
        for (int k = 0; k < 4; ++k) {
            unsigned h0, h1, l0, l1;
            psalm_split_words(v[2 * k] * sc, h0, l0);
            psalm_split_words(v[2 * k + 1] * sc, h1, l1);
            hw[k] = h0 | (h1 << 16);
            lw[k] = l0 | (l1 << 16);
        }
        *reinterpret_cast<u32x4_s*>(orow + c) = u32x4_s{hw[0], hw[1], hw[2], hw[3]};
        *reinterpret_cast<u32x4_s*>(orow + Kp + c) = u32x4_s{lw[0], lw[1], lw[2], lw[3]};
    }
}

__global__ void __launch_bounds__(256) split_f16_row_kernel(const float* __restrict__ x, long ldx, unsigned short* __restrict__ out, long ldo,
                                                            float* __restrict__ inv_scale, int K, int Kp) {
    __shared__ float red[4];
    const int tid = threadIdx.x;
    const long row = blockIdx.x;
    const float* xr = x + row * ldx;
    float amax = 0.f;
    for (int c = tid * 8; c < K; c += 2048) {
        float v[8];
        load8_f32(xr + c, v);
#pragma unroll
        for (int k = 0; k < 8; ++k) amax = fmaxf(amax, fabsf(v[k]));
    }
    amax = wave_max(amax);
    if ((tid & 63) == 0) red[tid >> 6] = amax;
    __syncthreads();
    amax = fmaxf(fmaxf(red[0], red[1]), fmaxf(red[2], red[3]));
    int e = (int)((__builtin_bit_cast(unsigned, amax) >> 23) & 0xffu) - 127;
    int se = 13 - e;
    se = se > 100 ? 100 : (se < -100 ? -100 : se);
    const bool zero = !(amax > 0.f) || !(amax < 3.0e38f);
    const float sc = zero ? 1.f : __builtin_bit_cast(float, (unsigned)(127 + se) << 23);
    const float inv = zero ? 1.f : __builtin_bit_cast(float, (unsigned)(127 - se) << 23);
    if (tid == 0) inv_scale[row] = inv;
    unsigned short* orow = out + row * ldo;
    for (int c = tid * 8; c < Kp; c += 2048) {
        float v[8];
        if (c < K) load8_f32(xr + c, v);
        else {
#pragma unroll
            for (int k = 0; k < 8; ++k) v[k] = 0.f;
        }
        unsigned hw[4], lw[4];
#pragma unroll
        for (int k = 0; k < 4; ++k) {
            unsigned h0, h1, l0, l1;
            psalm_split_words(v[2 * k] * sc, h0, l0);
            psalm_split_words(v[2 * k + 1] * sc, h1, l1);
            hw[k] = h0 | (h1 << 16);
            lw[k] = l0 | (l1 << 16);
        }
        *reinterpret_cast<u32x4_s*>(orow + c) = u32x4_s{hw[0], hw[1], hw[2], hw[3]};
        *reinterpret_cast<u32x4_s*>(orow + Kp + c) = u32x4_s{lw[0], lw[1], lw[2], lw[3]};
    }
}

extern "C" int psalm_split_f16(const float* x, long ldx, void* out, long ldo, float* inv_scale, int rows, int K, void* stream) {
    if (rows == 0) return 0;
    const int Kp = (K + 63) / 64 * 64;
    PSALM_CHECK_ARG(K > 0 && K % 8 == 0 && (uintptr_t)x % 16 == 0 && (ldx * 4) % 16 == 0, "psalm_split_f16: K % 8 == 0, 16-byte aligned input rows");
    PSALM_CHECK_ARG((uintptr_t)out % 16 == 0 && (ldo * 2) % 16 == 0 && ldo >= 2L * Kp, "psalm_split_f16: output rows of >= 2*ceil64(K) f16, 16-byte aligned");
    hipStream_t s = (hipStream_t)stream;
    if (Kp >= 1024 && rows <= 4096) {
        hipLaunchKernelGGL(split_f16_row_kernel, dim3(rows), dim3(256), 0, s, x, ldx, (unsigned short*)out, ldo, inv_scale, K, Kp);
        PSALM_LAUNCH_END("psalm_split_f16");
    }
    if (Kp <= 128) hipLaunchKernelGGL((split_f16_kernel<16>), dim3(cdiv(rows, 16)), dim3(256), 0, s, x, ldx, (unsigned short*)out, ldo, inv_scale, rows, K, Kp);
    else if (Kp <= 256) hipLaunchKernelGGL((split_f16_kernel<32>), dim3(cdiv(rows, 8)), dim3(256), 0, s, x, ldx, (unsigned short*)out, ldo, inv_scale, rows, K, Kp);
    else hipLaunchKernelGGL((split_f16_kernel<64>), dim3(cdiv(rows, 4)), dim3(256), 0, s, x, ldx, (unsigned short*)out, ldo, inv_scale, rows, K, Kp);
    PSALM_LAUNCH_END("psalm_split_f16");
}

struct SplitOut { void* so; long ldso; int so_kp, so_col_off, so_col_start, so_global; float* so_inv; const float* so_par; int so_paired; };
static int gemm_x3_impl(const void* A2, long lda, const float* a_scale, const void* W2, long ldw, const float* w_scale, int Kp,
                        const float* bias, const void* residual, long ldr, void* C, long ldc, int M, int N, int act,
                        int act_col_start, void* workspace, long workspace_bytes, void* stream, const SplitOut* so, const char* name,
                        const LnEpilogue* ln = nullptr, int select_m = 0) {
    if (M == 0 || N == 0) return 0;
    PSALM_CHECK_ARG(Kp > 0 && Kp % 64 == 0, "psalm_gemm_x3: Kp must be a positive multiple of 64");
    PSALM_CHECK_ARG((uintptr_t)A2 % 16 == 0 && (lda * 2) % 16 == 0 && (uintptr_t)W2 % 16 == 0 && (ldw * 2) % 16 == 0 && lda >= 2L * Kp && ldw >= 2L * Kp,
                    "psalm_gemm_x3: 16-byte aligned operand rows of >= 2*Kp f16");
    PSALM_CHECK_ARG(a_scale && w_scale, "psalm_gemm_x3: scales required");
    GemmArgs g;
    g.A = A2; g.W = W2; g.bias = bias; g.res = residual; g.C = C;
    g.lda = lda; g.ldw = ldw; g.ldr = ldr; g.ldc = ldc;
    g.M = M; g.N = N; g.K = 3 * Kp; g.act = act; g.act_col_start = act_col_start;
    g.row_fast = 0; g.tiles_m = g.tiles_n = 0;
    hipStream_t s = (hipStream_t)stream;
    if (!so && !ln && (select_m > 0 ? select_m : M) <= 128 && N <= g_skinny_nmax && !g_tile_policy) {
        const dim3 grid(cdiv(N, 32), cdiv(M, 32));
        g.K = g_x3_products * Kp;
        snprintf(g_last_kernel, sizeof(g_last_kernel), "gemm_bf16_skinny_kernel<float, true>");
        hipLaunchKernelGGL((gemm_bf16_skinny_kernel<float, true>), grid, dim3(256), 0, s, g, SkinnyX3{a_scale, w_scale, Kp});
        PSALM_LAUNCH_END(name);
    }
    GemmFastArgs fa;
    fa.cH = fa.cW = fa.cC = fa.cK = fa.cS = fa.cP = fa.cHo = fa.cWo = 0;
    fa.zeros = nullptr;
    fa.a_scale = a_scale; fa.w_scale = w_scale;
    fa.x3_kp = Kp;
    if (so) {
        fa.so = (unsigned short*)so->so; fa.ldso = so->ldso; fa.so_kp = so->so_kp; fa.so_col_off = so->so_col_off;
        fa.so_col_start = so->so_col_start; fa.so_global = so->so_global; fa.so_inv = so->so_inv; fa.so_par = so->so_par;
        fa.so_paired = so->so_paired;
    }
    return launch_fast(g, fa, false, PSALM_F32, workspace, workspace_bytes, s, ln, true, select_m);
}
int gemm_x3_select_rows(const void* A2, long lda, const float* a_scale, const void* W2, long ldw, const float* w_scale, int Kp, void* C, long ldc,
                        int M, int N, int select_m, void* workspace, long workspace_bytes, void* stream) {
    return gemm_x3_impl(A2, lda, a_scale, W2, ldw, w_scale, Kp, nullptr, nullptr, 0, C, ldc, M, N, 0, 0, workspace, workspace_bytes, stream, nullptr,
                        "psalm_gemm_x3", nullptr, select_m);
}
extern "C" int psalm_gemm_x3(const void* A2, long lda, const float* a_scale, const void* W2, long ldw, const float* w_scale, int Kp,
                             const float* bias, const void* residual, long ldr, void* C, long ldc, int M, int N, int act,
                             int act_col_start, void* workspace, long workspace_bytes, void* stream) {
    return gemm_x3_impl(A2, lda, a_scale, W2, ldw, w_scale, Kp, bias, residual, ldr, C, ldc, M, N, act, act_col_start, workspace,
                        workspace_bytes, stream, nullptr, "psalm_gemm_x3");
}

extern "C" int psalm_gemm_x3_split(const void* A2, long lda, const float* a_scale, const void* W2, long ldw, const float* w_scale, int Kp,
                                   const float* bias, void* C, long ldc, int M, int N, int act, int act_col_start, void* split_out,
                                   long ld_split, int split_kp, int split_col_off, int split_col_start, int paired, float* split_inv,
                                   const float* bound_par, int global_rows, void* workspace, long workspace_bytes, void* stream) {
    PSALM_CHECK_ARG(paired == 0 || paired == 1, "psalm_gemm_x3_split: paired is 0 or 1");
    PSALM_CHECK_ARG(!paired || (split_col_start % 256 == 0 && (N - split_col_start) % 64 == 0 && (long)M * ld_split * 2 < (1L << 31)),
                    "psalm_gemm_x3_split: paired output needs split_col_start % 256 == 0, (N - split_col_start) % 64 == 0, split_out < 2 GiB");
    PSALM_CHECK_ARG(split_out && split_inv && bound_par, "psalm_gemm_x3_split: split output, scale array and bound parameters required");
    PSALM_CHECK_ARG(N % 8 == 0 && split_col_start % 8 == 0 && split_col_start >= 0 && split_col_start < N && split_col_off % 8 == 0 &&
                        split_col_off >= 0 && split_kp % 8 == 0 && (uintptr_t)split_out % 16 == 0 && (ld_split * 2) % 16 == 0 &&
                        split_col_off + (N - split_col_start) <= split_kp && ld_split >= 2L * split_kp,
                    "psalm_gemm_x3_split: N / column offsets multiples of 8, 16-byte aligned split rows of >= 2*split_kp f16");
    PSALM_CHECK_ARG(C || split_col_start == 0, "psalm_gemm_x3_split: C required for the columns below split_col_start");
    SplitOut so{split_out, ld_split, split_kp, split_col_off, split_col_start, global_rows, split_inv, bound_par, paired};
    return gemm_x3_impl(A2, lda, a_scale, W2, ldw, w_scale, Kp, bias, nullptr, 0, C, ldc, M, N, act, act_col_start, workspace, workspace_bytes,
                        stream, &so, "psalm_gemm_x3_split");
}


extern "C" int psalm_gemm_x3_ln_split(const void* A2, long lda, const float* a_scale, const void* W2, long ldw, const float* w_scale, int Kp,
                                      const float* bias, const void* residual, long ldr, void* C, long ldc, int M, int N,
                                      const float* ln_gamma, const float* ln_beta, float ln_eps, void* ln_out, long ld_ln, void* split_out,
                                      float* split_inv, void* workspace, long workspace_bytes, void* stream) {
    PSALM_CHECK_ARG(N % 64 == 0 && N <= 2048 && split_out && split_inv && C, "psalm_gemm_x3_ln_split: N % 64 == 0, N <= 2048, outputs required");
    PSALM_CHECK_ARG((uintptr_t)C % 16 == 0 && (ldc * 4) % 16 == 0 && (uintptr_t)ln_gamma % 16 == 0 && (uintptr_t)ln_beta % 16 == 0 &&
                        (uintptr_t)split_out % 16 == 0 && (!ln_out || ((uintptr_t)ln_out % 16 == 0 && (ld_ln * 4) % 16 == 0)) &&
                        (!residual || ((uintptr_t)residual % 16 == 0 && (ldr * 4) % 16 == 0)),
                    "psalm_gemm_x3_ln_split: 16-byte aligned rows");
    LnEpilogue ln{ln_gamma, ln_beta, ln_eps, ln_out, PSALM_F32, ld_ln, split_out, split_inv};
    return gemm_x3_impl(A2, lda, a_scale, W2, ldw, w_scale, Kp, bias, residual, ldr, C, ldc, M, N, 0, 0, workspace, workspace_bytes, stream,
                        nullptr, "psalm_gemm_x3_ln_split", &ln);
}
```

psalm_amd/csrc/stages.hip:

```cpp
#include "common.h"
#include "psalm_hip.h"

static inline long al256(long v) { return (v + 255) / 256 * 256; }

struct PhiLayout {
    long x0, x1, h, hinv, big, a2, inv2, attn, total;
    int Kp;
};
static PhiLayout phi_layout(const psalm_phi_desc* d, int B, int L) {
    PhiLayout o;
    const long M = (long)B * L, H = d->hidden, I = d->intermediate;
    o.Kp = (int)((H + 63) / 64 * 64);
    long p = 0;
    o.x0 = p; p += al256(M * H * 4);
    o.x1 = p; p += al256(M * H * 4);
    o.h = p; p += al256(M * 2 * o.Kp * 2);
    o.hinv = p; p += al256(M * 4);
    o.big = p; p += al256(M * 3 * H * 4);
    o.a2 = p; p += al256(M * 2 * (H + I) * 2);
    o.inv2 = p; p += al256(M * 4);
    o.attn = p; p += al256(psalm_causal_attention_f32_workspace(B, L, d->heads));
    o.total = p;
    return o;
}

static int phi_check(const psalm_phi_desc* d) {
    PSALM_CHECK_ARG(d && d->layers && d->num_layers >= 1, "psalm_phi_forward: descriptor with >= 1 layer");
    PSALM_CHECK_ARG(d->head_dim == 64 && d->rot == 32 && d->hidden == d->heads * d->head_dim, "psalm_phi_forward: head_dim 64, rotary dim 32 (Phi-1.5)");
    PSALM_CHECK_ARG((d->hidden + d->intermediate) % 64 == 0 && d->hidden % 8 == 0 && d->intermediate % 8 == 0,
                    "psalm_phi_forward: (hidden + intermediate) % 64 == 0, hidden % 8 == 0");
    return 0;
}

extern "C" long psalm_phi_forward_workspace(const psalm_phi_desc* d, int B, int L) {
    if (phi_check(d) != 0 || B <= 0 || L <= 0) return -1;
    return phi_layout(d, B, L).total;
}

extern "C" int psalm_phi_forward(const psalm_phi_desc* d, const float* embeds, const unsigned char* key_mask, const float* cos_table,
                                 const float* sin_table, int B, int L, float* hidden_out, void* workspace, long workspace_bytes,
                                 void* gemm_workspace, long gemm_workspace_bytes, void* stream) {
    if (phi_check(d) != 0) return -1;
    PSALM_CHECK_ARG(embeds && key_mask && cos_table && sin_table && hidden_out && workspace && B > 0 && L > 0, "psalm_phi_forward: null argument");
    const PhiLayout lo = phi_layout(d, B, L);
    PSALM_CHECK_ARG(workspace_bytes >= lo.total && (uintptr_t)workspace % 256 == 0, "psalm_phi_forward: workspace of psalm_phi_forward_workspace() bytes, 256-byte aligned");
    char* ws = (char*)workspace;
    const int M = B * L, H = d->hidden, I = d->intermediate, Kp = lo.Kp, K2 = H + I;
    float* x[2] = {(float*)(ws + lo.x0), (float*)(ws + lo.x1)};
    void* h = ws + lo.h;
    float* hinv = (float*)(ws + lo.hinv);
    float* big = (float*)(ws + lo.big);
    void* a2 = ws + lo.a2;
    float* inv2 = (float*)(ws + lo.inv2);
    void* attn = ws + lo.attn;
    int rc;
    const psalm_phi_layer* l0 = &d->layers[0];
    rc = psalm_layernorm_split(embeds, H, nullptr, H, l0->ln_g, l0->ln_b, M, H, d->ln_eps, h, hinv, nullptr, 0, nullptr, nullptr, stream);
    if (rc) return rc;
    const float* xin = embeds;
    int cur = 0;
    for (int i = 0; i < d->num_layers; ++i) {
        const psalm_phi_layer* ly = &d->layers[i];
        const bool last = i == d->num_layers - 1;
        PSALM_CHECK_ARG(ly->w1 && ly->w1_scale && ly->b1 && ly->w2 && ly->w2_scale && ly->b2 && ly->bnd, "psalm_phi_forward: layer weights missing");
        rc = psalm_gemm_x3_split(h, 2L * Kp, hinv, ly->w1, 2L * Kp, ly->w1_scale, Kp, ly->b1, big, 3L * H, M, 3 * H + I,  3, 3 * H, a2,
                                 2L * K2, K2, H, 3 * H, ly->paired, inv2, ly->bnd, 1, gemm_workspace, gemm_workspace_bytes, stream);
        if (rc) return rc;
        rc = psalm_causal_attention_f32_split(big, 3L * H, 2 * H, 0, H, a2, 2L * K2, K2, 0, inv2, cos_table, sin_table, key_mask, attn, B, L, d->heads,
                                              d->head_dim, d->rot, stream);
        if (rc) return rc;
        float* xout = x[cur];
        if (last || H % 64 != 0 || H > 2048) {
            rc = psalm_gemm_x3(a2, 2L * K2, inv2, ly->w2, 2L * K2, ly->w2_scale, K2, ly->b2, xin, H, xout, H, M, H, 0, 0, gemm_workspace,
                               gemm_workspace_bytes, stream);
            if (rc) return rc;
            if (last) {
                rc = psalm_layernorm(xout, PSALM_F32, H, hidden_out, PSALM_F32, H, nullptr, 0, d->final_g, d->final_b, M, H, d->ln_eps, stream);
            } else {
                const psalm_phi_layer* nx = &d->layers[i + 1];
                rc = psalm_layernorm_split(xout, H, nullptr, H, nx->ln_g, nx->ln_b, M, H, d->ln_eps, h, hinv, nullptr, 0, nullptr, nullptr, stream);
            }
            if (rc) return rc;
        } else {
            const psalm_phi_layer* nx = &d->layers[i + 1];
            rc = psalm_gemm_x3_ln_split(a2, 2L * K2, inv2, ly->w2, 2L * K2, ly->w2_scale, K2, ly->b2, xin, H, xout, H, M, H, nx->ln_g, nx->ln_b,
                                        d->ln_eps, nullptr, H, h, hinv, gemm_workspace, gemm_workspace_bytes, stream);
            if (rc) return rc;
        }
        xin = xout;
        cur ^= 1;
    }
    return 0;
}

struct PhiCacheLayout { long k_bytes, v_bytes, stride; int Pp; };
static PhiCacheLayout phi_cache_layout(int hidden, int heads, int P) {
    PhiCacheLayout c;
    c.Pp = (P + 31) / 32 * 32;
    c.k_bytes = al256((long)heads * c.Pp * 64 * 4);
    c.v_bytes = al256((long)P * hidden * 4);
    c.stride = c.k_bytes + c.v_bytes;
    return c;
}
static PhiCacheLayout phi_cache_layout(const psalm_phi_desc* d, int P) { return phi_cache_layout(d->hidden, d->heads, P); }

extern "C" long psalm_phi_prefix_cache_layer_bytes(int hidden, int heads, int P, long* k_bytes, long* v_bytes) {
    if (hidden <= 0 || heads <= 0 || P <= 0) return -1;
    const PhiCacheLayout c = phi_cache_layout(hidden, heads, P);
    if (k_bytes) *k_bytes = c.k_bytes;
    if (v_bytes) *v_bytes = c.v_bytes;
    return c.stride;
}

extern "C" long psalm_phi_prefix_cache_bytes(const psalm_phi_desc* d, int P) {
    if (phi_check(d) != 0 || P <= 0) return -1;
    return phi_cache_layout(d, P).stride * d->num_layers;
}
extern "C" long psalm_phi_prefix_workspace(const psalm_phi_desc* d, int P) {
    if (phi_check(d) != 0 || P <= 0) return -1;
    return phi_layout(d, 1, P).total;
}
extern "C" long psalm_phi_suffix_workspace(const psalm_phi_desc* d, int N, int S) {
    if (phi_check(d) != 0 || N <= 0 || S <= 0) return -1;
    return phi_layout(d, N, S).total;
}

static int phi_session_pass(const psalm_phi_desc* d, bool suffix, const float* embeds, const unsigned char* key_mask, const float* cos_table,
                            const float* sin_table, int B, int L, int P, char* cache, long cache_bytes, float* hidden_out, void* workspace,
                            long workspace_bytes, void* gemm_workspace, long gemm_workspace_bytes, void* stream,
                            const psalm_prefix_ref* refs = nullptr) {
    const PhiLayout lo = phi_layout(d, B, L);
    const PhiCacheLayout cl = phi_cache_layout(d, P);
    PSALM_CHECK_ARG(workspace_bytes >= lo.total && (uintptr_t)workspace % 256 == 0, "psalm_phi_prefix / _suffix: workspace of the _workspace() function's bytes, 256-byte aligned");
    PSALM_CHECK_ARG(refs || (cache_bytes >= cl.stride * d->num_layers && (uintptr_t)cache % 256 == 0), "psalm_phi_prefix / _suffix: cache of psalm_phi_prefix_cache_bytes() bytes, 256-byte aligned");
    char* ws = (char*)workspace;
    const int M = B * L, H = d->hidden, I = d->intermediate, Kp = lo.Kp, K2 = H + I;
    float* x[2] = {(float*)(ws + lo.x0), (float*)(ws + lo.x1)};
    void* h = ws + lo.h;
    float* hinv = (float*)(ws + lo.hinv);
    float* big = (float*)(ws + lo.big);
    void* a2 = ws + lo.a2;
    float* inv2 = (float*)(ws + lo.inv2);
    void* attn = ws + lo.attn;
    int rc;
    const psalm_phi_layer* l0 = &d->layers[0];
    rc = psalm_layernorm_split(embeds, H, nullptr, H, l0->ln_g, l0->ln_b, M, H, d->ln_eps, h, hinv, nullptr, 0, nullptr, nullptr, stream);
    if (rc) return rc;
    const float* xin = embeds;
    int cur = 0;
    for (int i = 0; i < d->num_layers; ++i) {
        const psalm_phi_layer* ly = &d->layers[i];
        const bool last = i == d->num_layers - 1;
        PSALM_CHECK_ARG(ly->w1 && ly->w1_scale && ly->b1 && ly->w2 && ly->w2_scale && ly->b2 && ly->bnd, "psalm_phi_prefix / _suffix: layer weights missing");
// ... 945 lines not shown
```

psalm_amd/hip_ops.py:

```python
from __future__ import annotations

import ctypes
import math
import os
import sys
from ctypes import c_char_p, c_float, c_int, c_long, c_void_p
from typing import Optional, Sequence

import numpy as np
import torch

_HERE = os.path.dirname(os.path.abspath(__file__))
DEFAULT_LIB = os.path.join(_HERE, "lib", "libpsalm_hip.so")

F32, BF16 = 0, 1
ACT_NONE, ACT_RELU, ACT_GELU, ACT_GELU_NEW = 0, 1, 2, 3
ACT_POST_RESIDUAL = 16
ACT_BIAS_ROW = 32
_DT = {torch.float32: F32, torch.bfloat16: BF16}


_DEBUG_SYNC = os.environ.get("PSALM_DEBUG_SYNC", "0") not in ("", "0")
_DEBUG_BOUNDS = os.environ.get("PSALM_DEBUG_BOUNDS", "0") not in ("", "0")
BOUND_LOOSENESS_LIMIT = 2.0 ** 14


class PsalmHipError(RuntimeError):
    pass


def _dt(t: torch.Tensor) -> int:
    try:
        return _DT[t.dtype]
    except KeyError:
        raise PsalmHipError(f"unsupported dtype {t.dtype} (float32 / bfloat16 only)")


ABI_VERSION = 15


class _ProfiledLib:

    def __init__(self, cdll):
        object.__setattr__(self, "_cdll", cdll)
        object.__setattr__(self, "records", None)
        object.__setattr__(self, "calls", None)

    def __getattr__(self, name):
        fn = getattr(self._cdll, name)
        if not name.startswith("psalm_") or name in ("psalm_last_error", "psalm_backend", "psalm_abi_version", "psalm_gemm_last_kernel",
                                                         "psalm_gemm_set_tile_policy", "psalm_gemm_x3_set_products", "psalm_set_tuning",
                                                         "psalm_get_tuning") or name.endswith("_workspace"):
            return fn

        def call(*args):
            rec = self.records
            if self.calls is not None:
                self.calls.append(name)
            if _DEBUG_SYNC:
                sys.stderr.write(f"[psalm launch] {name}\n"); sys.stderr.flush()
                rc = fn(*args)
                if torch.cuda.is_available() and not torch.cuda.is_current_stream_capturing():
                    torch.cuda.synchronize()
                sys.stderr.write(f"[psalm ok] {name}\n"); sys.stderr.flush()
                return rc
            if rec is None:
                return fn(*args)
            e0, e1 = torch.cuda.Event(enable_timing=True), torch.cuda.Event(enable_timing=True)
            e0.record()
            rc = fn(*args)
            e1.record()
            kern = None
            if name.startswith(("psalm_gemm", "psalm_conv2d")):
                kern = self._cdll.psalm_gemm_last_kernel().decode()
            rec.append((name, tuple(a.value if hasattr(a, "value") else a for a in args), e0, e1, kern))
            return rc
        return call

    def __setattr__(self, k, v):
        if k in ("records", "calls"):
            object.__setattr__(self, k, v)
        else:
            setattr(self._cdll, k, v)


class SplitF16:
    __slots__ = ("t", "inv_scale", "K", "Kp")

    def __init__(self, t, inv_scale, K):
        self.t, self.inv_scale, self.K, self.Kp = t, inv_scale, K, t.shape[1] // 2

    @property
    def shape(self):
        return (self.t.shape[0], self.K)

    @property
    def dtype(self):
        return torch.float32


class _PostDesc(ctypes.Structure):
    _fields_ = [(n, c_int) for n in ("task", "Q", "h", "w", "Hpad", "Wpad", "crop_h", "crop_w", "out_h", "out_w", "C1", "n_region")] + \
               [("obj_thr", c_float), ("overlap_thr", c_float)]


class _PostIO(ctypes.Structure):
    _fields_ = [(n, c_void_p) for n in ("pred_masks", "mask_up", "cls_logits", "seg_logits", "region_logits", "is_thing", "mask_pred", "sem_seg", "scores",
                                        "classes", "query", "inst_masks", "boxes", "pan", "counts")]


class _PhiLayer(ctypes.Structure):
    _fields_ = [("w1", c_void_p), ("w1_scale", c_void_p), ("b1", c_void_p), ("w2", c_void_p), ("w2_scale", c_void_p), ("b2", c_void_p),
                ("ln_g", c_void_p), ("ln_b", c_void_p), ("bnd", c_void_p), ("paired", c_int)]


class _PhiDesc(ctypes.Structure):
    _fields_ = [("num_layers", c_int), ("hidden", c_int), ("intermediate", c_int), ("heads", c_int), ("head_dim", c_int), ("rot", c_int),
                ("ln_eps", c_float), ("layers", ctypes.POINTER(_PhiLayer)), ("final_g", c_void_p), ("final_b", c_void_p)]


class _SwinBlock(ctypes.Structure):
    _fields_ = [(n, c_void_p) for n in ("n1_g", "n1_b", "n2_g", "n2_b", "qkv_w", "qkv_ws", "qkv_b", "qkv_bnd", "proj_w", "proj_ws", "proj_b",
                                         "fc1_w", "fc1_ws", "fc1_b", "fc1_bnd")] + [("fc1_paired", c_int)] + \
               [(n, c_void_p) for n in ("fc2_w", "fc2_ws", "fc2_b", "rpb")]


class _SwinStage(ctypes.Structure):
    _fields_ = [("depth", c_int), ("heads", c_int), ("dim", c_int), ("blocks", ctypes.POINTER(_SwinBlock)), ("out_g", c_void_p), ("out_b", c_void_p),
                ("ds_g", c_void_p), ("ds_b", c_void_p), ("ds_w", c_void_p), ("ds_ws", c_void_p)]


class _SwinDesc(ctypes.Structure):
    _fields_ = [("num_stages", c_int), ("patch", c_int), ("window", c_int), ("pe_kpad", c_int), ("mlp_ratio", c_int), ("pe_w", c_void_p),
                ("pe_ws", c_void_p), ("pe_b", c_void_p), ("pe_ln_g", c_void_p), ("pe_ln_b", c_void_p), ("stages", ctypes.POINTER(_SwinStage))]


class _ProjDesc(ctypes.Structure):
    _fields_ = [("in_dim", c_int), ("mid_dim", c_int), ("out_dim", c_int)] + \
               [(n, c_void_p) for n in ("c1_w", "c1_ws", "c1_b", "c2_w", "c2_ws", "c2f_w", "c2f_ws", "c2f_b", "ds_w", "ds_ws", "ds_b", "fc_w", "fc_ws", "fc_b")]


class _PdEncLayer(ctypes.Structure):
    _fields_ = [(n, c_void_p) for n in ("value_w", "value_ws", "value_b", "ow_w", "ow_ws", "ow_b", "out_w", "out_ws", "out_b", "n1_g", "n1_b",
                                         "l1_w", "l1_ws", "l1_b", "l1_bnd")] + [("l1_paired", c_int)] + \
               [(n, c_void_p) for n in ("l2_w", "l2_ws", "l2_b", "n2_g", "n2_b")]


class _PdDesc(ctypes.Structure):
    _fields_ = [("D", c_int), ("G", c_int), ("M", c_int), ("num_layers", c_int), ("ffn", c_int), ("mask_dim", c_int), ("in_dims", c_int * 4),
                ("ip_w", c_void_p * 3), ("ip_ws", c_void_p * 3), ("ip_b", c_void_p * 3), ("ip_gn_g", c_void_p * 3), ("ip_gn_b", c_void_p * 3)] + \
               [(n, c_void_p) for n in ("adapter_w", "adapter_ws", "adapter_b", "adapter_gn_g", "adapter_gn_b", "layer_w", "layer_ws", "layer_b",
                                         "layer_gn_g", "layer_gn_b", "mf_w", "mf_ws", "mf_b")] + [("layers", ctypes.POINTER(_PdEncLayer))]


class _PrLayer(ctypes.Structure):
    _fields_ = [(n, c_void_p) for n in ("cq_w", "cq_b", "co_w", "co_b", "cn_g", "cn_b", "sqk_w", "sqk_b", "sv_w", "sv_b", "so_w", "so_b", "sn_g", "sn_b",
                                         "f1_w", "f1_b", "f2_w", "f2_b", "fn_g", "fn_b")]


class _PrDesc(ctypes.Structure):
    _fields_ = [(n, c_int) for n in ("D", "heads", "Q", "num_layers", "num_levels", "ffn", "mask_dim")] + \
               [(n, c_void_p * 3) for n in ("lvl_k_w", "lvl_k_ws", "lvl_k_b", "lvl_v_w", "lvl_v_ws", "lvl_v_b")] + \
               [(n, c_void_p) for n in ("level_embed", "query_embed", "dn_g", "dn_b")] + [("mask_embed_w", c_void_p * 3), ("mask_embed_b", c_void_p * 3)] + \
               [(n, c_void_p * 2) for n in ("SEG_w", "SEG_b", "CLASS_w", "CLASS_b", "REGION_w", "REGION_b")] + [("layers", ctypes.POINTER(_PrLayer))]


class Ops:
    GEMM_X3_256_DEFAULT = 2582

    def __init__(self, lib_path: str = DEFAULT_LIB):
        if not os.path.exists(lib_path):
            raise PsalmHipError(
                f"{lib_path} not found: build the HIP kernels first (python -m psalm_amd.build). "
                "psalm_amd has no CPU / PyTorch fallback by design.")
        cdll = ctypes.CDLL(lib_path)
        got = cdll.psalm_abi_version() if hasattr(cdll, "psalm_abi_version") else -1
        if got != ABI_VERSION:
            raise PsalmHipError(f"{lib_path}: psalm_abi_version() = {got}, this binding needs {ABI_VERSION}: rebuild the library "
                                "(python -m psalm_amd.build --force)")
        cdll.psalm_last_error.restype = c_char_p
        cdll.psalm_backend.restype = c_char_p
        cdll.psalm_gemm_last_kernel.restype = c_char_p
        self._cdll_raw = cdll
        self.lib = _ProfiledLib(cdll)
        self.backend = self.lib.psalm_backend().decode()
        self.is_emu = self.backend == "emu"
        self.device = torch.device("cpu") if self.is_emu else torch.device("cuda", torch.cuda.current_device())
        self.lib_path = lib_path
        self._ws = {}
        self._msda_tables = set()
        self.debug_bounds = False
        self.bound_looseness_max = 1.0
        self.x3 = False

    def _stream(self):
        if self.is_emu:
# ... 61 lines not shown
            dst.copy_(src)
            return dst
        self._check(self.lib.psalm_copy_d2d(self._p(dst), self._p(src), c_long(dst.numel() * dst.element_size()), self._stream()), "psalm_copy_d2d")
        return dst

    def gemm(self, a, w, bias=None, residual=None, act=ACT_NONE, act_col_start=0, out=None, out_dtype=None):
        if isinstance(a, SplitF16) or isinstance(w, SplitF16) or (self.x3 and a.dtype == torch.float32 and w.dtype == torch.float32):
            return self.gemm_x3(a, w, bias, residual, act, act_col_start, out, out_dtype)
        if a.dim() != 2 or w.dim() != 2 or a.shape[1] != w.shape[1]:
            raise PsalmHipError(f"gemm shape mismatch {tuple(a.shape)} x {tuple(w.shape)}")
        M, K = a.shape
        N = w.shape[0]
        if out is None:
            out = self.empty(M, N, dtype=out_dtype or (torch.float32 if w.dtype == torch.float32 else a.dtype))
        for t in (a, w, out) + ((residual,) if residual is not None else ()):
            if t.stride(-1) != 1:
                raise PsalmHipError("gemm operands need a contiguous last dimension")
        if residual is not None and (residual.dtype != out.dtype or residual.shape != out.shape):
            raise PsalmHipError("gemm residual must match the output's dtype and shape")
        if bias is not None and (bias.dtype != torch.float32 or bias.numel() != (M if act & ACT_BIAS_ROW else N)):
            raise PsalmHipError("gemm bias must be float32 (N,) -- or (M,) with ACT_BIAS_ROW")
        rc = self.lib.psalm_gemm(self._pv(a), _dt(a), c_long(a.stride(0)), self._pv(w), _dt(w), c_long(w.stride(0)),
                                 self._pv(bias), self._pv(residual), c_long(residual.stride(0) if residual is not None else 0),
                                 self._pv(out), _dt(out), c_long(out.stride(0)), M, N, K, act, act_col_start,
                                 self._p(self._gemm_ws()), c_long(self.GEMM_WS_BYTES), self._stream())
        self._check(rc, "psalm_gemm")
        return out

    def split_f16(self, x):
        if isinstance(x, SplitF16):
            return x
        if x.dim() != 2 or x.dtype != torch.float32 or x.stride(1) != 1:
            raise PsalmHipError("split_f16: 2-D float32 input with a contiguous last dimension")
        rows, K = x.shape
        Kp = (K + 63) // 64 * 64
        t = self.empty(rows, 2 * Kp, dtype=torch.float16)
        inv = self.empty(rows, dtype=torch.float32)
        rc = self.lib.psalm_split_f16(self._pv(x), c_long(x.stride(0)), self._p(t), c_long(2 * Kp), self._p(inv), rows, K, self._stream())
        self._check(rc, "psalm_split_f16")
        return SplitF16(t, inv, K)

    def _x3_operands(self, a, w):
        a, w = self.split_f16(a), self.split_f16(w)
        if a.K != w.K or a.Kp != w.Kp:
            raise PsalmHipError(f"gemm shape mismatch {a.shape} x {w.shape}")
        return a, w

    def gemm_x3(self, a, w, bias=None, residual=None, act=ACT_NONE, act_col_start=0, out=None, out_dtype=None):
        a, w = self._x3_operands(a, w)
        M, N = a.t.shape[0], w.t.shape[0]
        if out is None:
            if out_dtype not in (None, torch.float32):
                raise PsalmHipError("gemm_x3: float32 output only")
            out = self.empty(M, N, dtype=torch.float32)
        for t in (out,) + ((residual,) if residual is not None else ()):
            if t.dtype != torch.float32 or t.stride(-1) != 1 or tuple(t.shape) != (M, N):
                raise PsalmHipError("gemm_x3: float32 (M,N) output / residual with a contiguous last dimension")
        if bias is not None and (bias.dtype != torch.float32 or bias.numel() != (M if act & ACT_BIAS_ROW else N)):
            raise PsalmHipError("gemm bias must be float32 (N,) -- or (M,) with ACT_BIAS_ROW")
        rc = self.lib.psalm_gemm_x3(self._p(a.t), c_long(a.t.stride(0)), self._p(a.inv_scale), self._p(w.t), c_long(w.t.stride(0)),
                                    self._p(w.inv_scale), a.Kp, self._pv(bias), self._pv(residual),
                                    c_long(residual.stride(0) if residual is not None else 0), self._pv(out), c_long(out.stride(0)),
                                    M, N, act, act_col_start, self._p(self._gemm_ws()), c_long(self.GEMM_WS_BYTES), self._stream())
        self._check(rc, "psalm_gemm_x3")
        return out

    def gemm_x3_ln_split(self, a, w, bias, residual, gamma, beta, eps, want_y=False):
        a, w = self._x3_operands(a, w)
        M, N = a.t.shape[0], w.t.shape[0]
        if residual is not None and (residual.dtype != torch.float32 or tuple(residual.shape) != (M, N) or residual.stride(-1) != 1):
            raise PsalmHipError("gemm_x3_ln_split: float32 (M,N) residual")
        x = self.empty(M, N, dtype=torch.float32)
        y = self.empty(M, N, dtype=torch.float32) if want_y else None
        so, inv = self.empty(M, 2 * N, dtype=torch.float16), self.empty(M, dtype=torch.float32)
        rc = self.lib.psalm_gemm_x3_ln_split(self._p(a.t), c_long(a.t.stride(0)), self._p(a.inv_scale), self._p(w.t), c_long(w.t.stride(0)),
                                             self._p(w.inv_scale), a.Kp, self._pv(bias), self._pv(residual),
                                             c_long(residual.stride(0) if residual is not None else 0), self._p(x), c_long(N), M, N,
                                             self._p(gamma), self._p(beta), c_float(eps), self._pv(y), c_long(N), self._p(so), self._p(inv),
                                             self._p(self._gemm_ws()), c_long(self.GEMM_WS_BYTES), self._stream())
        self._check(rc, "psalm_gemm_x3_ln_split")
        return x, SplitF16(so, inv, N), y

    def gemm_x3_split(self, a, w, bias, act, split_out, split_inv, bound_par, split_col_off=0, split_col_start=0, act_col_start=0,
                      out=None, global_rows=False, paired=False):
        a, w = self._x3_operands(a, w)
        M, N = a.t.shape[0], w.t.shape[0]
        if split_out.dtype != torch.float16 or split_out.dim() != 2 or split_out.shape[0] != M or split_out.stride(1) != 1:
            raise PsalmHipError("gemm_x3_split: split_out must be a (M, 2*Kp) float16 buffer")
        if split_inv.dtype != torch.float32 or split_inv.numel() != M or bound_par.dtype != torch.float32 or bound_par.numel() != 4:
            raise PsalmHipError("gemm_x3_split: split_inv (M,) / bound_par (4,) float32")
        if split_col_start > 0 and (out is None or out.dtype != torch.float32 or out.shape[0] != M or out.stride(-1) != 1):
            raise PsalmHipError("gemm_x3_split: float32 `out` required for the columns below split_col_start")
        if bias is not None and (bias.dtype != torch.float32 or bias.numel() != N):
            raise PsalmHipError("gemm bias must be float32 (N,)")
        rc = self.lib.psalm_gemm_x3_split(self._p(a.t), c_long(a.t.stride(0)), self._p(a.inv_scale), self._p(w.t), c_long(w.t.stride(0)),
                                          self._p(w.inv_scale), a.Kp, self._pv(bias), self._pv(out),
                                          c_long(out.stride(0) if out is not None else 0), M, N, act, act_col_start,
                                          self._p(split_out), c_long(split_out.stride(0)), split_out.shape[1] // 2, split_col_off,
                                          split_col_start, int(bool(paired)), self._p(split_inv), self._p(bound_par), int(bool(global_rows)),
                                          self._p(self._gemm_ws()), c_long(self.GEMM_WS_BYTES), self._stream())
        self._check(rc, "psalm_gemm_x3_split")
        if _DEBUG_BOUNDS or self.debug_bounds:
            self.check_split_bound(split_out, split_col_off, N - split_col_start, "gemm_x3_split")
        return split_out

    @staticmethod
    def so_pair_perm(n: int) -> torch.Tensor:
        if n % 64:
            raise PsalmHipError("so_pair_perm: n % 64 == 0")
        p = torch.arange(n)
        return (p // 64) * 64 + 2 * (p % 32) + (p % 64) // 32

    def check_split_bound(self, split_out, col_off, ncols, what=""):
        hi = split_out[:, col_off:col_off + ncols].float().abs().amax(1)
        live = hi > 0
        if not bool(live.any()):
            return 1.0
        loose = float((2.0 ** 13 / hi[live]).max())
        self.bound_looseness_max = max(self.bound_looseness_max, loose)
        if loose > BOUND_LOOSENESS_LIMIT:
            raise PsalmHipError(f"{what}: the magnitude bound behind the split-f16 output scale is 2^{math.log2(loose):.1f} above the "
                                f"actual row maximum (limit 2^14): lo is reaching the f16 subnormal floor -- run this GEMM without the "
                                "fused split output (PSALM.fuse_split = False) or tighten its bound")
        return loose

    def gemm_ln(self, a, w, bias, residual, gamma, beta, eps=1e-5, ln_dtype=torch.bfloat16, act=ACT_NONE):
        M, K = a.shape
        N = w.shape[0]
        out = self.empty(M, N, dtype=torch.float32)
        ln_out = self.empty(M, N, dtype=ln_dtype)
        if residual is not None and (residual.dtype != torch.float32 or residual.shape != out.shape):
            raise PsalmHipError("gemm_ln: residual must be float32 (M,N)")
        rc = self.lib.psalm_gemm_ln(self._pv(a), _dt(a), c_long(a.stride(0)), self._pv(w), _dt(w), c_long(w.stride(0)), self._p(bias),
                                    self._pv(residual), c_long(residual.stride(0) if residual is not None else 0), self._p(out), F32,
                                    c_long(N), M, N, K, act, 0, self._p(gamma), self._p(beta), c_float(eps), self._p(ln_out), _dt(ln_out),
                                    c_long(N), self._p(self._gemm_ws()), c_long(self.GEMM_WS_BYTES), self._stream())
        self._check(rc, "psalm_gemm_ln")
        return out, ln_out

    def conv2d_nhwc(self, x, B, H, W, wt, ksize, stride, pad, bias=None, residual=None, act=ACT_NONE, out_dtype=None):
        Cin, Cout = x.shape[-1], wt.shape[0]
        if x.dtype != torch.bfloat16 or wt.dtype != torch.bfloat16 or wt.shape[1] != ksize * ksize * Cin:
            raise PsalmHipError("conv2d_nhwc: bf16 operands, weight (Cout, k*k*Cin)")
        Ho, Wo = (H + 2 * pad - ksize) // stride + 1, (W + 2 * pad - ksize) // stride + 1
        out = self.empty(B * Ho * Wo, Cout, dtype=out_dtype or x.dtype)
        if residual is not None and (residual.dtype != out.dtype or residual.shape != out.shape):
            raise PsalmHipError("conv2d_nhwc: residual must match the output")
        z = self._ws.get("zeros")
        if z is None:
            z = self._ws["zeros"] = torch.zeros(256, dtype=torch.uint8, device=self.device)
        rc = self.lib.psalm_conv2d_nhwc(self._p(x), B, H, W, Cin, self._p(wt), Cout, ksize, stride, pad, self._p(bias), self._pv(residual),
                                        c_long(residual.stride(0) if residual is not None else 0), self._p(out), _dt(out),
                                        c_long(out.stride(0)), act, self._p(z), self._p(self._gemm_ws()), c_long(self.GEMM_WS_BYTES),
                                        self._stream())
        self._check(rc, "psalm_conv2d_nhwc")
        return out

    def gemm_describe(self, M, N, K, a_bf16=True, w_bf16=True, x3=False):
        out = (c_int * 4)()
        if x3:
            self._cdll_raw.psalm_gemm_describe(M, N, K, 2, 2, c_long(self.GEMM_WS_BYTES), out)
            return tuple(out)
        self._cdll_raw.psalm_gemm_describe(M, N, K, BF16 if a_bf16 else F32, BF16 if w_bf16 else F32, c_long(self.GEMM_WS_BYTES), out)
        return tuple(out)

    def gemm_last_kernel(self) -> str:
        return self._cdll_raw.psalm_gemm_last_kernel().decode()

    def phi_desc(self, layers, hidden, intermediate, heads, head_dim, rot, ln_eps, final_g, final_b):
        arr = (_PhiLayer * len(layers))()
        keep = []
        for i, ly in enumerate(layers):
            w1, w2 = ly["w1"], ly["w2"]
            if not (isinstance(w1, SplitF16) and isinstance(w2, SplitF16)):
                raise PsalmHipError("phi_desc: split-f16 weights (precision 'f16x3')")
            arr[i] = _PhiLayer(self._p(w1.t), self._p(w1.inv_scale), self._p(ly["b1"]), self._p(w2.t), self._p(w2.inv_scale), self._p(ly["b2"]),
                               self._p(ly["ln_g"]), self._p(ly["ln_b"]), self._p(ly["bnd"]), int(bool(ly["paired"])))
            keep.append(ly)
        d = _PhiDesc(len(layers), hidden, intermediate, heads, head_dim, rot, ln_eps, ctypes.cast(arr, ctypes.POINTER(_PhiLayer)),
                     self._p(final_g), self._p(final_b))
        d._keep = (arr, keep, final_g, final_b)
        return d

    def swin_desc(self, w, depths, heads, dims, patch, window, pe_kpad, mlp_ratio, paired):
# ... 229 lines not shown
                    raise PsalmHipError(f"predictor_forward_batched: the {name} counts do not add up to the embedding rows")
            o_ = [int(v) for v in o_]
            if len(o_) != B + 1 or o_[-1] > emb.shape[0]:
                raise PsalmHipError(f"predictor_forward_batched: (B + 1) {name} offsets within the embedding rows")
            return (c_int * (B + 1))(*o_), max(o_[-1], 0)

        c_off, n_c = offs("cls", class_emb, cls_counts)
        s_off, n_s = offs("seg", seg_emb, seg_counts)
        r_off, n_r = offs("region", region_emb, reg_counts)
        hw = (c_int * (2 * len(shapes)))(*[int(v) for s_ in shapes for v in s_])
        self.lib.psalm_predictor_forward_batched_workspace.restype = c_long
        nbytes = self.lib.psalm_predictor_forward_batched_workspace(ctypes.byref(desc), hw, H2, W2, B, n_r)
        if nbytes < 0:
            raise PsalmHipError(f"psalm_predictor_forward_batched_workspace: {self.lib.psalm_last_error().decode()}")
        kws, koff, kbytes, _ = kv
        if kbytes < self.predictor_kv_bytes(desc, shapes, mf_size):
            raise PsalmHipError("predictor_forward_batched: the K / V workspace was prepared for another geometry")
        ws = self._stage_ws("predictor_batched", nbytes + 256)
        off = (-ws.data_ptr()) % 256
        masks = self.empty(B * Q, H2 * W2, dtype=torch.float32)
        cls = self.empty(Q * n_c, dtype=torch.float32) if class_emb is not None else None
        seg = self.empty(Q * n_s, dtype=torch.float32) if seg_emb is not None else None
        reg = self.empty(n_r * Q, dtype=torch.float32) if region_emb is not None else None
        rc = self.lib.psalm_predictor_forward_batched(ctypes.byref(desc), hw, c_void_p(kws.data_ptr() + koff), self._p(mf), H2, W2, B, self._p(seg_query),
                                                      self._p(class_emb), c_off, self._p(seg_emb), s_off, self._p(region_emb), r_off, self._p(masks),
                                                      self._p(cls), self._p(seg), self._p(reg), c_void_p(ws.data_ptr() + off), c_long(nbytes),
                                                      self._p(self._gemm_ws()), c_long(self.GEMM_WS_BYTES), self._stream())
        self._check(rc, "psalm_predictor_forward_batched")
        return masks, cls, seg, reg

    POST_TASKS = {"semantic": 0, "instance": 1, "panoptic": 2, "referring": 3, "region": 4}

    def postprocess(self, task, sizes, pred_masks=None, mask_up=None, cls_logits=None, seg_logits=None, region_logits=None, is_thing=None,
                    obj_thr=0.8, overlap_thr=0.8, counts_extra=0):
        Hpad, Wpad, oh, ow, height, width = [int(v) for v in sizes]
        src = pred_masks if pred_masks is not None else mask_up
        Q = int(src.shape[0])
        h_, w_ = (int(pred_masks.shape[1]), int(pred_masks.shape[2])) if pred_masks is not None else (Hpad, Wpad)
        C1 = int(cls_logits.shape[1]) if cls_logits is not None else 0
        k = int(region_logits.shape[0]) if region_logits is not None else 0
        code = self.POST_TASKS[task]
        d = _PostDesc(code, Q, h_, w_, Hpad, Wpad, oh, ow, height, width, C1, k, float(obj_thr), float(overlap_thr))
        self.lib.psalm_postprocess_workspace.restype = c_long
        nbytes = self.lib.psalm_postprocess_workspace(ctypes.byref(d), 1 if mask_up is not None else 0)
        if nbytes < 0:
            raise PsalmHipError(f"psalm_postprocess_workspace: {self.lib.psalm_last_error().decode()}")
        ws = self._stage_ws("postprocess", nbytes + 256)
        off = (-ws.data_ptr()) % 256
        resize_after = (oh, ow, height, width) != (Hpad, Wpad, Hpad, Wpad)
        out = {}
        if task == "semantic":
            if mask_up is None:
                out["mask_pred"] = self.empty(Q, Hpad, Wpad)
            out["sem_seg"] = self.empty(C1 - 1, height, width)
        else:
            if resize_after or mask_up is None:
                out["mask_pred"] = self.empty(Q, height, width)
            out["scores"] = self.empty(Q, k) if task == "region" else self.empty(Q)
            out["inst_masks"] = self.empty(Q, height, width)
            out["boxes"] = self.empty(Q, 4)
            out["counts"] = self.empty(2 + 3 * Q + int(counts_extra), dtype=torch.int32)
            if task in ("instance", "panoptic"):
                out["classes"] = self.empty(Q, dtype=torch.int64)
            if task != "region":
                out["query"] = self.empty(Q, dtype=torch.int64)
            if task == "panoptic":
                out["sem_seg"] = self.empty(C1 - 1, height, width)
                out["pan"] = self.empty(height, width, dtype=torch.int32)
        io = _PostIO(*[self._pi(t) for t in (pred_masks, mask_up, cls_logits, seg_logits, region_logits, is_thing, out.get("mask_pred"), out.get("sem_seg"),
                                             out.get("scores"), out.get("classes"), out.get("query"), out.get("inst_masks"), out.get("boxes"), out.get("pan"),
                                             out.get("counts"))])
        which = c_int(0)
        fn = getattr(self.lib, "psalm_postprocess_" + task)
        rc = fn(ctypes.byref(d), ctypes.byref(io), ctypes.byref(which), c_void_p(ws.data_ptr() + off), c_long(nbytes), self._stream())
        self._check(rc, "psalm_postprocess_" + task)
        if which.value == 1:
            out["mask_pred"] = mask_up
        return out

    @staticmethod
    def _pi(t):
        return None if t is None else t.data_ptr()

    def phi_forward(self, desc, embeds, key_mask, cos, sin, B, L):
        if embeds.dtype != torch.float32 or embeds.dim() != 2 or embeds.shape[0] != B * L or embeds.shape[1] != desc.hidden:
            raise PsalmHipError("phi_forward: float32 (B*L, hidden) embeddings")
        self.lib.psalm_phi_forward_workspace.restype = c_long
        nbytes = self.lib.psalm_phi_forward_workspace(ctypes.byref(desc), B, L)
        if nbytes < 0:
            raise PsalmHipError(f"psalm_phi_forward_workspace: {self.lib.psalm_last_error().decode()}")
        ws = self._stage_ws("phi", nbytes + 256)
        off = (-ws.data_ptr()) % 256
        out = self.empty(B * L, desc.hidden, dtype=torch.float32)
        rc = self.lib.psalm_phi_forward(ctypes.byref(desc), self._p(embeds), self._p(key_mask), self._p(cos), self._p(sin), B, L, self._p(out),
                                        c_void_p(ws.data_ptr() + off), c_long(nbytes), self._p(self._gemm_ws()), c_long(self.GEMM_WS_BYTES),
                                        self._stream())
        self._check(rc, "psalm_phi_forward")
        return out

    def phi_prefix_cache(self, hidden, heads, P, num_layers):
        self.lib.psalm_phi_prefix_cache_layer_bytes.restype = c_long
        kb, vb = c_long(0), c_long(0)
        stride = self.lib.psalm_phi_prefix_cache_layer_bytes(hidden, heads, P, ctypes.byref(kb), ctypes.byref(vb))
        if stride <= 0:
            raise PsalmHipError("phi_prefix_cache: hidden, heads, P >= 1")
        kb, Pp = kb.value, (P + 31) // 32 * 32
        raw = torch.empty(stride * num_layers + 256, dtype=torch.uint8, device=self.device)
        off = (-raw.data_ptr()) % 256
        buf = raw[off:off + stride * num_layers]
        views = []
        for i in range(num_layers):
            o0 = stride * i
            views.append((buf[o0:o0 + heads * Pp * 64 * 4].view(torch.float32).view(heads, Pp, 64),
                          buf[o0 + kb:o0 + kb + P * hidden * 4].view(torch.float32).view(P, hidden)))
        return buf, views

    def phi_prefix(self, desc, embeds, key_mask, cos, sin, P, cache):
        if embeds.dtype != torch.float32 or embeds.dim() != 2 or embeds.shape[0] != P or embeds.shape[1] != desc.hidden or key_mask.numel() != P:
            raise PsalmHipError("phi_prefix: float32 (P, hidden) embeddings, key mask of P bytes")
        self.lib.psalm_phi_prefix_workspace.restype = c_long
        self.lib.psalm_phi_prefix_cache_bytes.restype = c_long
        nbytes = self.lib.psalm_phi_prefix_workspace(ctypes.byref(desc), P)
        cbytes = self.lib.psalm_phi_prefix_cache_bytes(ctypes.byref(desc), P)
        if nbytes < 0 or cbytes < 0:
            raise PsalmHipError(f"psalm_phi_prefix_workspace: {self.lib.psalm_last_error().decode()}")
        if cache.numel() < cbytes or cache.data_ptr() % 256:
            raise PsalmHipError("phi_prefix: cache of psalm_phi_prefix_cache_bytes() bytes, 256-byte aligned")
        ws = self._stage_ws("phi_prefix", nbytes + 256)
        off = (-ws.data_ptr()) % 256
        rc = self.lib.psalm_phi_prefix(ctypes.byref(desc), self._p(embeds), self._p(key_mask), self._p(cos), self._p(sin), P, self._p(cache),
                                       c_long(cache.numel()), c_void_p(ws.data_ptr() + off), c_long(nbytes), self._p(self._gemm_ws()),
                                       c_long(self.GEMM_WS_BYTES), self._stream())
        self._check(rc, "psalm_phi_prefix")

    def phi_suffix(self, desc, embeds, key_mask, cos, sin, N, S, P, cache):
        if embeds.dtype != torch.float32 or embeds.dim() != 2 or embeds.shape[0] != N * S or embeds.shape[1] != desc.hidden or key_mask.numel() != N * S \
                or cos.shape[0] < P + S:
            raise PsalmHipError("phi_suffix: float32 (N*S, hidden) embeddings, key mask (N, S), tables of >= P + S rows")
        self.lib.psalm_phi_suffix_workspace.restype = c_long
        self.lib.psalm_phi_prefix_cache_bytes.restype = c_long
        nbytes = self.lib.psalm_phi_suffix_workspace(ctypes.byref(desc), N, S)
        cbytes = self.lib.psalm_phi_prefix_cache_bytes(ctypes.byref(desc), P)
        if nbytes < 0 or cbytes < 0:
            raise PsalmHipError(f"psalm_phi_suffix_workspace: {self.lib.psalm_last_error().decode()}")
        if cache.numel() < cbytes or cache.data_ptr() % 256:
            raise PsalmHipError("phi_suffix: cache of psalm_phi_prefix_cache_bytes() bytes, 256-byte aligned")
        ws = self._stage_ws("phi_suffix", nbytes + 256)
        off = (-ws.data_ptr()) % 256
        out = self.empty(N * S, desc.hidden, dtype=torch.float32)
        rc = self.lib.psalm_phi_suffix(ctypes.byref(desc), self._p(embeds), self._p(key_mask), self._p(cos), self._p(sin), N, S, P, self._p(cache),
                                       c_long(cache.numel()), self._p(out), c_void_p(ws.data_ptr() + off), c_long(nbytes),
                                       self._p(self._gemm_ws()), c_long(self.GEMM_WS_BYTES), self._stream())
        self._check(rc, "psalm_phi_suffix")
        return out

    def phi_suffix_grouped(self, desc, embeds, key_mask, cos, sin, N, S, refs, P_max, table=None):
        if embeds.dtype != torch.float32 or embeds.dim() != 2 or embeds.shape[0] != N * S or embeds.shape[1] != desc.hidden or key_mask.numel() != N * S \
                or cos.shape[0] < P_max + S:
            raise PsalmHipError("phi_suffix_grouped: float32 (N*S, hidden) embeddings, key mask (N, S), tables of >= P_max + S rows")
        refs = self._prefix_refs(refs, table, desc.num_layers * N, P_max, desc.heads, "phi_suffix_grouped")
        self.lib.psalm_phi_suffix_grouped_workspace.restype = c_long
        nbytes = self.lib.psalm_phi_suffix_grouped_workspace(ctypes.byref(desc), N, S)
        if nbytes < 0:
            raise PsalmHipError(f"psalm_phi_suffix_grouped_workspace: {self.lib.psalm_last_error().decode()}")
        ws = self._stage_ws("phi_suffix", nbytes + 256)
        off = (-ws.data_ptr()) % 256
        out = self.empty(N * S, desc.hidden, dtype=torch.float32)
        rc = self.lib.psalm_phi_suffix_grouped(ctypes.byref(desc), self._p(embeds), self._p(key_mask), self._p(cos), self._p(sin), N, S,
                                               self._p(refs) if refs is not None else None, P_max, self._p(out),
                                               c_void_p(ws.data_ptr() + off), c_long(nbytes), self._p(self._gemm_ws()),
                                               c_long(self.GEMM_WS_BYTES), self._stream())
        self._check(rc, "psalm_phi_suffix_grouped")
        return out

    def x3_products(self, n: int):
        self._check(self.lib.psalm_gemm_x3_set_products(int(n)), "psalm_gemm_x3_set_products")

    TUNE_GEMM_XCD_KSPLIT, TUNE_ATTN_XCD_HEADS, TUNE_GEMM_MID, TUNE_DECODER_FUSE, TUNE_ROW_GROUPS, TUNE_MHA_QTILE_WAVES = 0, 1, 2, 3, 4, 5

    def set_tuning(self, key: int, value: int):
        self._check(self.lib.psalm_set_tuning(int(key), int(value)), "psalm_set_tuning")

    def get_tuning(self, key: int) -> int:
        return int(self.lib.psalm_get_tuning(int(key)))

    def gemm_tile_policy(self, bm: int):
        self._check(self.lib.psalm_gemm_set_tile_policy(bm), "psalm_gemm_set_tile_policy")

    def layernorm(self, x, gamma, beta, eps=1e-5, out=None, out_dtype=None, out2=None, add=None, out3=None):
        rows, C = x.shape
        if out is None:
            out = self.empty(rows, C, dtype=out_dtype or x.dtype)
        for t in (out2, out3):
            if t is not None and t.dtype != torch.bfloat16:
                raise PsalmHipError("layernorm: out2 / out3 must be bfloat16")
        if out3 is not None and (add is None or add.dtype != torch.float32 or add.shape[1] != C):
            raise PsalmHipError("layernorm: out3 needs a float32 (r,C) `add` table")
        rc = self.lib.psalm_layernorm3(self._pv(x), _dt(x), c_long(x.stride(0)), self._pv(out), _dt(out), c_long(out.stride(0)),
                                       self._pv(out2), c_long(out2.stride(0) if out2 is not None else 0),
                                       self._p(add) if out3 is not None else c_void_p(0), c_long(add.shape[0] if out3 is not None else 0),
                                       self._pv(out3), c_long(out3.stride(0) if out3 is not None else 0),
                                       self._p(gamma), self._p(beta), rows, C, c_float(eps), self._stream())
        self._check(rc, "psalm_layernorm3")
        return out

    def layernorm_split(self, x, gamma, beta, eps=1e-5, want_y=False, want_split=True, add=None):
        rows, C = x.shape
        if x.dtype != torch.float32 or x.stride(1) != 1:
            raise PsalmHipError("layernorm_split: float32 rows")
        Kp = (C + 63) // 64 * 64
        y = self.empty(rows, C, dtype=torch.float32) if want_y else None
        s1 = i1 = s2 = i2 = None
        if want_split:
            s1, i1 = self.empty(rows, 2 * Kp, dtype=torch.float16), self.empty(rows, dtype=torch.float32)
        if add is not None:
            if add.dtype != torch.float32 or add.shape[1] != C:
                raise PsalmHipError("layernorm_split: float32 (r,C) `add` table")
            s2, i2 = self.empty(rows, 2 * Kp, dtype=torch.float16), self.empty(rows, dtype=torch.float32)
        rc = self.lib.psalm_layernorm_split(self._pv(x), c_long(x.stride(0)), self._p(y), c_long(C), self._p(gamma), self._p(beta), rows, C,
                                            c_float(eps), self._p(s1), self._p(i1), self._p(add), c_long(add.shape[0] if add is not None else 0),
                                            self._p(s2), self._p(i2), self._stream())
        self._check(rc, "psalm_layernorm_split")
        return y, (SplitF16(s1, i1, C) if want_split else None), (SplitF16(s2, i2, C) if add is not None else None)

    def swin_window_gather(self, x, gamma, beta, B, H, W, ws, shift, eps=1e-5, out_dtype=None):
        C = x.shape[-1]
        nWh, nWw = (H + ws - 1) // ws, (W + ws - 1) // ws
        out = self.empty(B * nWh * nWw * ws * ws, C, dtype=out_dtype or x.dtype)
        rc = self.lib.psalm_swin_window_gather(self._p(x), _dt(x), self._p(out), _dt(out), self._p(gamma), self._p(beta), B, H, W,
                                               C, ws, shift, c_float(eps), self._stream())
        self._check(rc, "psalm_swin_window_gather")
        return out

    def swin_window_gather_split(self, x, gamma, beta, B, H, W, ws, shift, eps=1e-5):
        C = x.shape[-1]
        if x.dtype != torch.float32 or C % 8 or C > 2048:
            raise PsalmHipError("swin_window_gather_split: float32, C % 8 == 0, C <= 2048")
        nWh, nWw = (H + ws - 1) // ws, (W + ws - 1) // ws
        rows, Kp = B * nWh * nWw * ws * ws, (C + 63) // 64 * 64
        t = self.empty(rows, 2 * Kp, dtype=torch.float16)
        inv = self.empty(rows, dtype=torch.float32)
        rc = self.lib.psalm_swin_window_gather_split(self._p(x), self._p(t), self._p(inv), self._p(gamma), self._p(beta), B, H, W, C, ws, shift,
                                                     c_float(eps), self._stream())
        self._check(rc, "psalm_swin_window_gather_split")
        return SplitF16(t, inv, C)

    def swin_window_merge_ln_split(self, win, shortcut, gamma, beta, B, H, W, ws, shift, eps=1e-5):
        C = shortcut.shape[-1]
        if shortcut.dtype != torch.float32 or win.dtype != torch.float32 or C % 8 or C > 2048:
            raise PsalmHipError("swin_window_merge_ln_split: float32 operands, C % 8 == 0, C <= 2048")
        rows, Kp = shortcut.shape[0], (C + 63) // 64 * 64
        out_x = torch.empty_like(shortcut)
        t = self.empty(rows, 2 * Kp, dtype=torch.float16)
        inv = self.empty(rows, dtype=torch.float32)
        rc = self.lib.psalm_swin_window_merge_ln_split(self._p(win), self._p(shortcut), self._p(out_x), self._p(t), self._p(inv), self._p(gamma),
                                                       self._p(beta), B, H, W, C, ws, shift, c_float(eps), self._stream())
        self._check(rc, "psalm_swin_window_merge_ln_split")
        return out_x, SplitF16(t, inv, C)

    def swin_window_merge(self, win, shortcut, B, H, W, ws, shift, out=None):
        C = shortcut.shape[-1]
# ... 93 lines not shown
        self._check(rc, "psalm_add_bcast")
        return out

    def gather_rows(self, srcs, src_id, src_row, C, out_dtype=torch.float32):
        srcs = list(srcs) + [None] * (4 - len(srcs))
        rows = src_id.numel()
        out = self.empty(rows, C, dtype=out_dtype)
        args = []
        for t in srcs:
            args += [self._p(t), _dt(t) if t is not None else 0]
        rc = self.lib.psalm_gather_rows(*args, self._p(src_id), self._p(src_row), self._p(out), _dt(out), c_long(rows), C,
                                        self._stream())
        self._check(rc, "psalm_gather_rows")
        return out

    def segment_mean(self, x, seg_offsets, seg_rows, out_dtype=None):
        nseg = seg_offsets.numel() - 1
        C = x.shape[-1]
        out = self.empty(nseg, C, dtype=out_dtype or x.dtype)
        rc = self.lib.psalm_segment_mean(self._pv(x), _dt(x), c_long(x.stride(0)), self._p(seg_offsets), self._p(seg_rows),
                                         self._p(out), _dt(out), nseg, C, self._stream())
        self._check(rc, "psalm_segment_mean")
        return out

    def window_attention(self, qkv, bias_table, B, nWh, nWw, heads, ws, shift):
        C = qkv.shape[-1] // 3
        out = self.empty(qkv.shape[0], C, dtype=qkv.dtype)
        if qkv.dtype == torch.bfloat16 and ws == 12:
            rc = self.lib.psalm_window_attention_mfma(self._p(qkv), self._p(bias_table), self._p(out), B, nWh, nWw, C, heads, ws,
                                                      shift, self._stream())
            self._check(rc, "psalm_window_attention_mfma")
            return out
        rc = self.lib.psalm_window_attention(self._p(qkv), self._p(bias_table), self._p(out), _dt(qkv), B, nWh, nWw, C, heads, ws,
                                             shift, self._stream())
        self._check(rc, "psalm_window_attention")
        return out

    def window_attention_split(self, qkv, bias_table, a_inv, bound_par, B, nWh, nWw, heads, ws, shift):
        C = qkv.shape[-1] // 3
        if qkv.dtype != torch.float32 or ws != 12 or a_inv.numel() != qkv.shape[0]:
            raise PsalmHipError("window_attention_split: float32 qkv, 12 x 12 windows, one operand scale per row")
        Kp = (C + 63) // 64 * 64
        so = (self.empty if Kp == C else self.zeros)(qkv.shape[0], 2 * Kp, dtype=torch.float16)
        inv = self.empty(qkv.shape[0], dtype=torch.float32)
        rc = self.lib.psalm_window_attention_split(self._p(qkv), self._p(bias_table), self._p(a_inv), self._p(bound_par), self._p(so), Kp,
                                                   self._p(inv), B, nWh, nWw, C, heads, ws, shift, self._stream())
        self._check(rc, "psalm_window_attention_split")
        return SplitF16(so, inv, C)

    def causal_attention(self, buf, q_off, k_off, v_off, out, o_off, cos, sin, key_mask, B, L, heads, head_dim, rot):
        if buf.dtype != out.dtype:
            raise PsalmHipError("causal_attention: buf/out dtype mismatch")
        if buf.dtype == torch.bfloat16:
            self.lib.psalm_causal_attention_mfma_workspace.restype = c_long
            nbytes = self.lib.psalm_causal_attention_mfma_workspace(B, L, heads)
            key = ("causal_ws", nbytes)
            ws = self._ws.get(key)
            if ws is None:
                ws = self._ws[key] = torch.empty(nbytes, dtype=torch.uint8, device=self.device)
            rc = self.lib.psalm_causal_attention_mfma(self._pv(buf), c_long(buf.stride(0)), q_off, k_off, v_off, self._pv(out),
                                                      c_long(out.stride(0)), o_off, self._p(cos), self._p(sin), self._p(key_mask),
                                                      self._p(ws), B, L, heads, head_dim, rot, self._stream())
            self._check(rc, "psalm_causal_attention_mfma")
            return out
        if (buf.dtype == torch.float32 and head_dim == 64 and rot == 32 and buf.stride(0) % 4 == 0 and out.stride(0) % 4 == 0
                and all(v % 4 == 0 for v in (q_off, k_off, v_off, o_off)) and buf.data_ptr() % 16 == 0 and out.data_ptr() % 16 == 0):
            self.lib.psalm_causal_attention_f32_workspace.restype = c_long
            nbytes = self.lib.psalm_causal_attention_f32_workspace(B, L, heads)
            key = ("causal_f32_ws", nbytes)
            ws = self._ws.get(key)
            if ws is None:
                ws = self._ws[key] = torch.empty(nbytes, dtype=torch.uint8, device=self.device)
            rc = self.lib.psalm_causal_attention_f32(self._pv(buf), c_long(buf.stride(0)), q_off, k_off, v_off, self._pv(out),
                                                     c_long(out.stride(0)), o_off, self._p(cos), self._p(sin), self._p(key_mask), self._p(ws),
                                                     B, L, heads, head_dim, rot, self._stream())
            self._check(rc, "psalm_causal_attention_f32")
            return out
        rc = self.lib.psalm_causal_attention(self._pv(buf), _dt(buf), c_long(buf.stride(0)), q_off, k_off, v_off, self._pv(out),
                                             c_long(out.stride(0)), o_off, self._p(cos), self._p(sin), self._p(key_mask), B, L,
                                             heads, head_dim, rot, self._stream())
        self._check(rc, "psalm_causal_attention")
        return out

    def causal_attention_split(self, buf, q_off, k_off, v_off, split_out, split_inv, split_col_off, cos, sin, key_mask, B, L, heads,
                               head_dim, rot):
        if buf.dtype != torch.float32 or split_out.dtype != torch.float16 or split_inv.dtype != torch.float32:
            raise PsalmHipError("causal_attention_split: float32 qkv buffer, float16 split buffer, float32 scales")
        self.lib.psalm_causal_attention_f32_workspace.restype = c_long
        nbytes = self.lib.psalm_causal_attention_f32_workspace(B, L, heads)
        key = ("causal_f32_ws", nbytes)
        ws = self._ws.get(key)
        if ws is None:
            ws = self._ws[key] = torch.empty(nbytes, dtype=torch.uint8, device=self.device)
        rc = self.lib.psalm_causal_attention_f32_split(self._pv(buf), c_long(buf.stride(0)), q_off, k_off, v_off, self._p(split_out),
                                                       c_long(split_out.stride(0)), split_out.shape[1] // 2, split_col_off,
                                                       self._p(split_inv), self._p(cos), self._p(sin), self._p(key_mask), self._p(ws),
                                                       B, L, heads, head_dim, rot, self._stream())
        self._check(rc, "psalm_causal_attention_f32_split")
        return split_out

    def _prefix_attn_ws(self, N, S, heads):
        self.lib.psalm_causal_attention_f32_prefix_workspace.restype = c_long
        nbytes = self.lib.psalm_causal_attention_f32_prefix_workspace(N, S, heads)
        key = ("causal_prefix_ws", nbytes)
        ws = self._ws.get(key)
        if ws is None:
            ws = self._ws[key] = torch.empty(nbytes, dtype=torch.uint8, device=self.device)
        return ws

    @staticmethod
    def _check_prefix_cache(k_cache, v_cache, P, heads):
        Pp = (P + 31) // 32 * 32
        if (k_cache.dtype != torch.float32 or v_cache.dtype != torch.float32 or not k_cache.is_contiguous() or k_cache.numel() != heads * Pp * 64
                or v_cache.dim() != 2 or v_cache.shape[0] != P or v_cache.shape[1] < heads * 64 or v_cache.stride(1) != 1):
            raise PsalmHipError("prefix cache: K (heads, ceil32(P), 64) float32 contiguous, V (P, >= heads*64) float32 rows")

    def phi_prefix_kv_store(self, buf, k_off, v_off, cos, sin, k_cache, v_cache, P, heads, head_dim, rot):
        if buf.dtype != torch.float32 or buf.shape[0] < P:
            raise PsalmHipError("phi_prefix_kv_store: float32 buffer of >= P rows")
        self._check_prefix_cache(k_cache, v_cache, P, heads)
        rc = self.lib.psalm_phi_prefix_kv_store(self._pv(buf), c_long(buf.stride(0)), k_off, v_off, self._p(cos), self._p(sin), self._p(k_cache),
                                                self._pv(v_cache), c_long(v_cache.stride(0)), P, heads, head_dim, rot, self._stream())
        self._check(rc, "psalm_phi_prefix_kv_store")

    def causal_attention_prefix(self, buf, q_off, k_off, v_off, k_cache, v_cache, out, o_off, cos, sin, key_mask, N, S, P, heads, head_dim, rot):
        if buf.dtype != torch.float32 or out.dtype != torch.float32 or cos.shape[0] < P + S or key_mask.numel() != N * S:
            raise PsalmHipError("causal_attention_prefix: float32 buffers, cos / sin tables of >= P + S rows, key_mask (N, S)")
        self._check_prefix_cache(k_cache, v_cache, P, heads)
        ws = self._prefix_attn_ws(N, S, heads)
        rc = self.lib.psalm_causal_attention_f32_prefix(self._pv(buf), c_long(buf.stride(0)), q_off, k_off, v_off, self._p(k_cache),
                                                        self._pv(v_cache), c_long(v_cache.stride(0)), self._pv(out), c_long(out.stride(0)), o_off,
                                                        self._p(cos), self._p(sin), self._p(key_mask), self._p(ws), N, S, P, heads, head_dim, rot,
                                                        self._stream())
        self._check(rc, "psalm_causal_attention_f32_prefix")
        return out

    def causal_attention_prefix_split(self, buf, q_off, k_off, v_off, k_cache, v_cache, split_out, split_inv, split_col_off, cos, sin, key_mask,
                                      N, S, P, heads, head_dim, rot):
        if (buf.dtype != torch.float32 or split_out.dtype != torch.float16 or split_inv.dtype != torch.float32 or cos.shape[0] < P + S
                or key_mask.numel() != N * S):
            raise PsalmHipError("causal_attention_prefix_split: float32 qkv buffer, float16 split buffer, float32 scales, tables of >= P + S rows")
        self._check_prefix_cache(k_cache, v_cache, P, heads)
        ws = self._prefix_attn_ws(N, S, heads)
        rc = self.lib.psalm_causal_attention_f32_prefix_split(self._pv(buf), c_long(buf.stride(0)), q_off, k_off, v_off, self._p(k_cache),
                                                              self._pv(v_cache), c_long(v_cache.stride(0)), self._p(split_out),
                                                              c_long(split_out.stride(0)), split_out.shape[1] // 2, split_col_off,
                                                              self._p(split_inv), self._p(cos), self._p(sin), self._p(key_mask), self._p(ws),
                                                              N, S, P, heads, head_dim, rot, self._stream())
        self._check(rc, "psalm_causal_attention_f32_prefix_split")
        return split_out

    PREFIX_REF = np.dtype([("k_cache", "<u8"), ("v_cache", "<u8"), ("ldv", "<i8"), ("P", "<i4"), ("pad", "<i4")])

    def prefix_ref_table(self, caches, prompt_cache, layers=None):
        if not len(caches) or not len(prompt_cache):
            raise PsalmHipError("prefix_ref_table: at least one cache and one prompt")
        layers = range(len(caches[0][1])) if layers is None else layers
        per = np.zeros((len(layers), len(caches)), self.PREFIX_REF)
        for c, (_, views) in enumerate(caches):
            for j, i in enumerate(layers):
                kc, vc = views[i]
                if kc.dtype != torch.float32 or vc.dtype != torch.float32 or not kc.is_contiguous() or vc.dim() != 2 or vc.stride(1) != 1 \
                        or kc.dim() != 3 or kc.shape[1] != (vc.shape[0] + 31) // 32 * 32 or kc.shape[2] != 64 or vc.shape[1] < kc.shape[0] * 64:
                    raise PsalmHipError("prefix cache: K (heads, ceil32(P), 64) float32 contiguous, V (P, >= heads*64) float32 rows")
                per[j, c] = (kc.data_ptr(), vc.data_ptr(), vc.stride(0), vc.shape[0], 0)
        idx = np.asarray(prompt_cache, np.int64)
# ... 696 lines not shown
```

Before: 55.90 images/s.

## Fuse Phi RoPE and Q/K relayout into the QKV GEMM epilogue

Adds a RoPE epilogue to the paired split-output x3 GEMM. Rotated, pre-scaled Q and K are written straight into the attention workspace layout, so the attention kernel's separate rotary/prep pass is skipped. A small per-forward tables kernel builds the key mask tiles and zero-pads Q/K once, and a new prepared attention entry point consumes them. The tuning knob is on by default. A new rope_elem helper tries to reproduce the old rounding per dimension (fma on some lanes only), which adds numerical coupling risk.

```diff
diff --git a/include/psalm_hip.h b/include/psalm_hip.h
--- a/include/psalm_hip.h
+++ b/include/psalm_hip.h
@@ -9,7 +9,7 @@
 #define PSALM_BF16 1
 
 const char* psalm_last_error(void);
-#define PSALM_ABI_VERSION 15
+#define PSALM_ABI_VERSION 16
 int psalm_abi_version(void);
 const char* psalm_backend(void);
 
@@ -19,6 +19,7 @@
 #define PSALM_TUNE_DECODER_FUSE 3
 #define PSALM_TUNE_ROW_GROUPS 4
 #define PSALM_TUNE_MHA_QTILE_WAVES 5
+#define PSALM_TUNE_PHI_ROPE_EPILOGUE 6
 #define PSALM_TUNE_COUNT 8
 int psalm_set_tuning(int key, int value);
 int psalm_get_tuning(int key);
@@ -68,6 +69,19 @@
                         const float* bias, void* C, long ldc, int M, int N, int act, int act_col_start, void* split_out, long ld_split,
                         int split_kp, int split_col_off, int split_col_start, int paired, float* split_inv, const float* bound_par,
                         int global_rows, void* workspace, long workspace_bytes, void* stream);
+typedef struct psalm_rope_out {
+    float* Qr;
+    float* Kr;
+    const float* cos_table;
+    const float* sin_table;
+    int q_col, k_col, heads, B, L, Lp;
+    float scale;
+    int pad_;
+} psalm_rope_out;
+int psalm_gemm_x3_split_rope(const void* A2, long lda, const float* a_scale, const void* W2, long ldw, const float* w_scale, int Kp,
+                             const float* bias, void* C, long ldc, int M, int N, int act, int act_col_start, void* split_out, long ld_split,
+                             int split_kp, int split_col_off, int split_col_start, int paired, float* split_inv, const float* bound_par,
+                             int global_rows, const psalm_rope_out* rope, void* workspace, long workspace_bytes, void* stream);
 
 int psalm_image_preprocess(const unsigned char* img, int H, int W, float* out, unsigned char* pad_mask, int S, int nh, int nw,
                            const int* bounds_h, const int* kk_h, int ksize_h, const int* bounds_v, const int* kk_v, int ksize_v,
@@ -99,6 +113,10 @@
                                      int split_col_off, const float* split_inv, const float* cos_table, const float* sin_table,
                                      const unsigned char* key_mask, void* workspace, int B, int L, int heads, int head_dim, int rot,
                                      void* stream);
+int psalm_phi_attention_tables(const unsigned char* key_mask, void* workspace, int B, int L, int heads, void* stream);
+int psalm_causal_attention_f32_split_prepared(const float* qkv, long ld, int v_off, void* split_out, long ld_split, int split_kp,
+                                              int split_col_off, const float* split_inv, void* workspace, int B, int L, int heads,
+                                              int head_dim, void* stream);
 
 long psalm_causal_attention_f32_prefix_workspace(int N, int S, int heads);
 int psalm_causal_attention_f32_prefix(const float* qkv, long ld, int q_off, int k_off, int v_off, const float* k_cache, const float* v_cache,
@@ -240,6 +258,7 @@
 int psalm_phi_forward(const psalm_phi_desc* d, const float* embeds, const unsigned char* key_mask, const float* cos_table, const float* sin_table,
                       int B, int L, float* hidden_out, void* workspace, long workspace_bytes, void* gemm_workspace, long gemm_workspace_bytes,
                       void* stream);
+int psalm_phi_forward_plan(const psalm_phi_desc* d, int B, int L, int* out3);
 
 long psalm_phi_prefix_cache_bytes(const psalm_phi_desc* d, int P);
 long psalm_phi_prefix_cache_layer_bytes(int hidden, int heads, int P, long* k_bytes, long* v_bytes);
diff --git a/psalm_amd/csrc/api.hip b/psalm_amd/csrc/api.hip
--- a/psalm_amd/csrc/api.hip
+++ b/psalm_amd/csrc/api.hip
@@ -11,7 +11,7 @@
     g_err[sizeof(g_err) - 1] = 0;
 }
 extern "C" const char* psalm_last_error() { return g_err; }
-static std::atomic<int> g_tuning[PSALM_TUNE_COUNT] = {{1}, {1}, {1}, {1}, {1}, {1}, {0}, {0}};
+static std::atomic<int> g_tuning[PSALM_TUNE_COUNT] = {{1}, {1}, {1}, {1}, {1}, {1}, {1}, {0}};
 extern "C" int psalm_set_tuning(int key, int value) {
     if (key < 0 || key >= PSALM_TUNE_COUNT) { psalm_set_error("psalm_set_tuning: unknown key"); return -1; }
     g_tuning[key].store(value, std::memory_order_relaxed);
diff --git a/psalm_amd/csrc/attention.hip b/psalm_amd/csrc/attention.hip
--- a/psalm_amd/csrc/attention.hip
+++ b/psalm_amd/csrc/attention.hip
@@ -631,8 +631,8 @@
             ld8(sinT + (pos0 + t) * ROT + c0, sn);
 #pragma unroll
             for (int i = 0; i < 8; ++i) {
-                q[i] = q[i] * cs[i] + (c0 < half ? -qo[i] : qo[i]) * sn[i];
-                k[i] = k[i] * cs[i] + (c0 < half ? -ko[i] : ko[i]) * sn[i];
+                q[i] = psalm_rope_elem(q[i], qo[i], cs[i], sn[i], c0 < half, psalm_rope_fused_dim(i));
+                k[i] = psalm_rope_elem(k[i], ko[i], cs[i], sn[i], c0 < half, psalm_rope_fused_dim(i));
             }
         }
 #pragma unroll
@@ -643,6 +643,31 @@
     }
     st8(qd, q);
     st8(kd, k);
+}
+
+__global__ void __launch_bounds__(256) phi_attention_tables_kernel(const unsigned char* __restrict__ key_mask, float* __restrict__ Qr,
+                                                                   float* __restrict__ Kr, unsigned char* __restrict__ Mk,
+                                                                   unsigned char* __restrict__ Tk, int L, int Lp, int heads) {
+    constexpr int HD = 64;
+    const int b = blockIdx.y;
+    const int t = blockIdx.x * 32 + (threadIdx.x >> 3), c0 = (threadIdx.x & 7) * 8;
+    __shared__ int tile_all;
+    const bool valid = t < L && key_mask[(long)b * L + min(t, L - 1)] != 0;
+    if (threadIdx.x == 0) tile_all = 1;
+    __syncthreads();
+    if (c0 == 0) {
+        Mk[(long)b * Lp + t] = valid ? 1 : 0;
+        if (!valid) tile_all = 0;
+    }
+    __syncthreads();
+    if (threadIdx.x == 0) Tk[(long)b * (Lp / 32) + blockIdx.x] = tile_all ? 1 : 0;
+    if (t >= L) {
+        const float z[8] = {0.f, 0.f, 0.f, 0.f, 0.f, 0.f, 0.f, 0.f};
+        for (int h = 0; h < heads; ++h) {
+            st8(Qr + (((long)b * heads + h) * Lp + t) * HD + c0, z);
+            st8(Kr + (((long)b * heads + h) * Lp + t) * HD + c0, z);
+        }
+    }
 }
 
 template <bool SO>
@@ -869,6 +894,42 @@
                                      B, L, heads, head_dim, rot, stream, split_inv, split_kp, "psalm_causal_attention_f32_split");
 }
 
+extern "C" int psalm_phi_attention_tables(const unsigned char* key_mask, void* workspace, int B, int L, int heads, void* stream) {
+    PSALM_CHECK_ARG(key_mask && workspace && (uintptr_t)workspace % 16 == 0 && B >= 0 && L >= 0 && heads >= 1,
+                    "psalm_phi_attention_tables: key mask and a 16-byte aligned workspace");
+    if (B == 0 || L == 0) return 0;
+    const int Lp = (L + 31) / 32 * 32;
+    float* Qr = (float*)workspace;
+    float* Kr = Qr + (long)B * heads * Lp * 64;
+    unsigned char* Mk = (unsigned char*)(Kr + (long)B * heads * Lp * 64);
+    unsigned char* Tk = Mk + (long)B * Lp;
+    hipLaunchKernelGGL(phi_attention_tables_kernel, dim3(Lp / 32, B), dim3(256), 0, (hipStream_t)stream, key_mask, Qr, Kr, Mk, Tk, L, Lp, heads);
+    PSALM_LAUNCH_END("psalm_phi_attention_tables");
+}
+extern "C" int psalm_causal_attention_f32_split_prepared(const float* qkv, long ld, int v_off, void* split_out, long ld_split, int split_kp,
+                                                         int split_col_off, const float* split_inv, void* workspace, int B, int L, int heads,
+                                                         int head_dim, void* stream) {
+    PSALM_CHECK_ARG(head_dim == 64, "psalm_causal_attention_f32_split_prepared: head_dim 64 (Phi-1.5)");
+    PSALM_CHECK_ARG(split_out && split_inv && ld_split >= 2L * split_kp && split_col_off + heads * 64 <= split_kp,
+                    "psalm_causal_attention_f32_split_prepared: split buffer rows of >= 2*split_kp f16 and the row scales");
+    PSALM_CHECK_ARG(ld % 4 == 0 && v_off % 4 == 0 && (uintptr_t)qkv % 16 == 0 && (uintptr_t)split_out % 16 == 0 && workspace &&
+                        (uintptr_t)workspace % 16 == 0 && ld_split % 8 == 0 && split_col_off % 8 == 0 && split_kp % 8 == 0,
+                    "psalm_causal_attention_f32_split_prepared: 16-byte aligned rows / offsets and a workspace");
+    if (B == 0 || L == 0) return 0;
+    PSALM_CHECK_ARG(((long)L - 1) * ld * 4 + 256 < 0x7fffffffL, "psalm_causal_attention_f32_split_prepared: L * ld * 4 must stay below 2 GiB (buffer-descriptor fetches)");
+    const int Lp = (L + 31) / 32 * 32;
+    const float* Qr = (const float*)workspace;
+    const float* Kr = Qr + (long)B * heads * Lp * 64;
+    const unsigned char* Mk = (const unsigned char*)(Kr + (long)B * heads * Lp * 64);
+    const unsigned char* Tk = Mk + (long)B * Lp;
+    const int pair = 1, nqt = Lp / 32;
+    const dim3 grid(pair ? (nqt + 1) / 2 : nqt, heads, B);
+    const int xcd_heads = ((heads * B) % 8 == 0 && psalm_get_tuning(PSALM_TUNE_ATTN_XCD_HEADS)) ? 1 : 0;
+    hipLaunchKernelGGL(causal_attention_f32_splitk_kernel<true>, grid, dim3(256), 0, (hipStream_t)stream, Qr, Kr, Mk, Tk, qkv, ld, v_off,
+                       (float*)split_out, ld_split, split_col_off, L, Lp, heads, split_inv, split_kp, pair, xcd_heads);
+    PSALM_LAUNCH_END("psalm_causal_attention_f32_split_prepared");
+}
+
 __global__ void __launch_bounds__(256) phi_prefix_kv_store_kernel(const float* __restrict__ base, long ld, int k_off, int v_off,
                                                                   const float* __restrict__ cosT, const float* __restrict__ sinT,
                                                                   float* __restrict__ Kc, float* __restrict__ Vc, long ldv, int P, int Pp, int heads) {
@@ -888,7 +949,7 @@
             ld8(cosT + (long)t * ROT + c0, cs);
             ld8(sinT + (long)t * ROT + c0, sn);
 #pragma unroll
-            for (int i = 0; i < 8; ++i) k[i] = k[i] * cs[i] + (c0 < half ? -ko[i] : ko[i]) * sn[i];
+            for (int i = 0; i < 8; ++i) k[i] = psalm_rope_elem(k[i], ko[i], cs[i], sn[i], c0 < half, psalm_rope_fused_dim(i));
         }
         float v[8];
         ld8(p + v_off + h * HD + c0, v);
diff --git a/psalm_amd/csrc/common.h b/psalm_amd/csrc/common.h
--- a/psalm_amd/csrc/common.h
+++ b/psalm_amd/csrc/common.h
@@ -118,6 +118,7 @@
 #ifdef PSALM_EMU_BUILD
 __device__ __forceinline__ unsigned psalm_swap_adjacent(unsigned v) { return __shfl_xor(v, 1); }
 __device__ __forceinline__ unsigned psalm_quad_swap2(unsigned v) { return __shfl_xor(v, 2); }
+__device__ __forceinline__ unsigned psalm_swap_row16(unsigned v) { return __shfl_xor(v, 16); }
 template <int P> __device__ __forceinline__ unsigned psalm_quad_bcast(unsigned v) { return __shfl(v, ((threadIdx.x & 63) & ~3) | P); }
 struct psalm_rsrc { char* base; unsigned bytes; };
 __device__ __forceinline__ psalm_rsrc psalm_make_rsrc(const void* p, unsigned bytes) { return psalm_rsrc{(char*)p, bytes}; }
@@ -139,6 +140,7 @@
 __device__ __forceinline__ unsigned psalm_quad_swap2(unsigned v) {
     return (unsigned)__builtin_amdgcn_mov_dpp((int)v, 0x4E, 0xF, 0xF, true);
 }
+__device__ __forceinline__ unsigned psalm_swap_row16(unsigned v) { return (unsigned)__builtin_amdgcn_ds_swizzle((int)v, 0x401F); }
 template <int P> __device__ __forceinline__ unsigned psalm_quad_bcast(unsigned v) {
     return (unsigned)__builtin_amdgcn_mov_dpp((int)v, P * 0x55, 0xF, 0xF, true);
 }
@@ -169,6 +171,14 @@
     return psalm_u32x4{v.x, v.y, v.z, v.w};
 }
 #endif
+
+__device__ __forceinline__ float psalm_rope_elem(float x, float xo, float cs, float sn, bool neg, bool fused) {
+#pragma clang fp contract(off)
+    const float t = (neg ? -xo : xo) * sn;
+    const float p = x * cs;
+    return fused ? fmaf(x, cs, t) : p + t;
+}
+__device__ __forceinline__ bool psalm_rope_fused_dim(int c) { return (c & 7) < 6; }
 
 extern "C" void psalm_set_error(const char* msg);
 extern "C" int psalm_get_tuning(int key);
@@ -179,6 +189,7 @@
 #define PSALM_TUNE_DECODER_FUSE 3
 #define PSALM_TUNE_ROW_GROUPS 4
 #define PSALM_TUNE_MHA_QTILE_WAVES 5
+#define PSALM_TUNE_PHI_ROPE_EPILOGUE 6
 #define PSALM_TUNE_COUNT 8
 #endif
 
diff --git a/psalm_amd/csrc/gemm.hip b/psalm_amd/csrc/gemm.hip
--- a/psalm_amd/csrc/gemm.hip
+++ b/psalm_amd/csrc/gemm.hip
@@ -1,4 +1,5 @@
 #include "common.h"
+#include "psalm_hip.h"
 #include <algorithm>
 #include <atomic>
 #include <cstring>
@@ -259,6 +260,12 @@
     float* so_inv = nullptr;
     const float* so_par = nullptr;
     int xcd_ksplit = 0;
+    float* rope_qr = nullptr;
+    float* rope_kr = nullptr;
+    const float* rope_cos = nullptr;
+    const float* rope_sin = nullptr;
+    int rope_q_col = 0, rope_k_col = 0, rope_heads = 0, rope_B = 0, rope_L = 0, rope_Lp = 0;
+    float rope_scale = 0.f;
 };
 __device__ __forceinline__ void split_scale_from_bound(float bound, float& sc, float& inv) {
     bound = fminf(fmaxf(bound, 7.888609e-31f), 1.2676506e30f);
@@ -797,6 +804,58 @@
         bool lds_path = !split && ((act != ACT_NONE && act != ACT_RELU && bn + BN > g.act_col_start) || (g.act & ACT_BIAS_ROW) != 0);
         if constexpr (SO) lds_path = lds_path || (fa.so != nullptr && bn + BN > fa.so_col_start);
         if (!lds_path) {
+            if constexpr (SO && PAIR) {
+                if (fa.rope_qr != nullptr) {
+                    static_assert(BN / WN == 64 && TN == 2 && X3 != 0, "RoPE epilogue: a wavefront's columns are one 64-wide head");
+                    const int wc0 = bn + wn * (BN / WN), nrot = fa.rope_heads * 64;
+                    const bool is_q = wc0 >= fa.rope_q_col && wc0 < fa.rope_q_col + nrot;
+                    const bool is_k = wc0 >= fa.rope_k_col && wc0 < fa.rope_k_col + nrot;
+                    if (is_q || is_k) {
+                        const int L = fa.rope_L, Lp = fa.rope_Lp;
+                        const int head = (wc0 - (is_q ? fa.rope_q_col : fa.rope_k_col)) >> 6;
+                        const psalm_rsrc rd = psalm_make_rsrc(is_q ? fa.rope_qr : fa.rope_kr, (unsigned)((long)fa.rope_B * fa.rope_heads * Lp * 256));
+                        const psalm_rsrc rcs = psalm_make_rsrc(fa.rope_cos, (unsigned)L * 128u), rsn = psalm_make_rsrc(fa.rope_sin, (unsigned)L * 128u);
+                        const unsigned hoff = (unsigned)head * (unsigned)Lp * 256u;
+                        const unsigned next_seq = (unsigned)(fa.rope_heads * Lp - L) * 256u;
+                        const float qs = is_q ? fa.rope_scale : 1.f;
+                        const bool neg = n32 < 16, fused = psalm_rope_fused_dim(n32);
+                        const int c0 = wc0 + n32;
+                        const float wsc0 = fa.w_scale[c0], wsc1 = fa.w_scale[c0 + 32];
+                        const float bias0 = g.bias ? g.bias[c0] : 0.f, bias1 = g.bias ? g.bias[c0 + 32] : 0.f;
+#pragma unroll
+                        for (int i = 0; i < TM; ++i) {
+                            const int rbase = bm + wm * (BM / WM) + i * 32;
+                            const int sb = rbase / L, t0 = rbase - sb * L;
+                            const unsigned seq0 = ((unsigned)(sb * fa.rope_heads) * (unsigned)Lp + (unsigned)t0) * 256u;
+                            float asc[16], cs[16], sn[16];
+                            unsigned off[16];
+#pragma unroll
+                            for (int r = 0; r < 16; ++r) {
+                                const int rr = 4 * hi + (r & 3) + 8 * (r >> 2), row = rbase + rr;
+                                const bool ok = row < g.M, wrap = t0 + rr >= L;
+                                const int t = wrap ? t0 + rr - L : t0 + rr;
+                                asc[r] = fa.a_scale[min(row, g.M - 1)];
+                                const unsigned toff = ok ? (unsigned)t * 128u + (unsigned)n32 * 4u : PSALM_BUF_OOB;
+                                cs[r] = psalm_buf_load_f32(rcs, toff);
+                                sn[r] = psalm_buf_load_f32(rsn, toff);
+                                off[r] = ok ? seq0 + (unsigned)rr * 256u + (wrap ? next_seq : 0u) + (unsigned)n32 * 4u : PSALM_BUF_OOB;
+                            }
+#pragma unroll
+                            for (int r = 0; r < 16; ++r) {
+                                const float x0 = fmaf(acc[i][0][r], asc[r] * wsc0, bias0) + 0.f, x1 = fmaf(acc[i][1][r], asc[r] * wsc1, bias1) + 0.f;
+                                const float xo = __builtin_bit_cast(float, psalm_swap_row16(__builtin_bit_cast(unsigned, x0)));
+                                const float y0 = psalm_rope_elem(x0, xo, cs[r], sn[r], neg, fused) * qs, y1 = x1 * qs;
+                                psalm_buf_store_f32_s(y0, rd, off[r], hoff);
+                                psalm_buf_store_f32_s(y1, rd, off[r] == PSALM_BUF_OOB ? off[r] : off[r] + 128u, hoff);
+                            }
+                        }
+                        PSALM_TL(4);
+                        PSALM_TL_DRAIN();
+                        PSALM_TL(5);
+                        return;
+                    }
+                }
+            }
             const bool post = (g.act & ACT_POST_RESIDUAL) != 0;
             float* Cb = split ? fa.slab + (long)ksl * g.M * g.N : (float*)g.C;
             const long ldo = split ? (long)g.N : g.ldc;
@@ -2212,7 +2271,8 @@
     PSALM_LAUNCH_END("psalm_split_f16");
 }
 
-struct SplitOut { void* so; long ldso; int so_kp, so_col_off, so_col_start, so_global; float* so_inv; const float* so_par; int so_paired; };
+struct SplitOut { void* so; long ldso; int so_kp, so_col_off, so_col_start, so_global; float* so_inv; const float* so_par; int so_paired;
+                  const psalm_rope_out* rope = nullptr; };
 static int gemm_x3_impl(const void* A2, long lda, const float* a_scale, const void* W2, long ldw, const float* w_scale, int Kp,
                         const float* bias, const void* residual, long ldr, void* C, long ldc, int M, int N, int act,
                         int act_col_start, void* workspace, long workspace_bytes, void* stream, const SplitOut* so, const char* name,
@@ -2244,6 +2304,12 @@
         fa.so = (unsigned short*)so->so; fa.ldso = so->ldso; fa.so_kp = so->so_kp; fa.so_col_off = so->so_col_off;
         fa.so_col_start = so->so_col_start; fa.so_global = so->so_global; fa.so_inv = so->so_inv; fa.so_par = so->so_par;
         fa.so_paired = so->so_paired;
+        if (so->rope) {
+            const psalm_rope_out* ro = so->rope;
+            fa.rope_qr = ro->Qr; fa.rope_kr = ro->Kr; fa.rope_cos = ro->cos_table; fa.rope_sin = ro->sin_table;
+            fa.rope_q_col = ro->q_col; fa.rope_k_col = ro->k_col; fa.rope_heads = ro->heads; fa.rope_B = ro->B; fa.rope_L = ro->L; fa.rope_Lp = ro->Lp;
+            fa.rope_scale = ro->scale;
+        }
     }
     return launch_fast(g, fa, false, PSALM_F32, workspace, workspace_bytes, s, ln, true, select_m);
 }
@@ -2276,6 +2342,38 @@
     return gemm_x3_impl(A2, lda, a_scale, W2, ldw, w_scale, Kp, bias, nullptr, 0, C, ldc, M, N, act, act_col_start, workspace, workspace_bytes,
                         stream, &so, "psalm_gemm_x3_split");
 }
+extern "C" int psalm_gemm_x3_split_rope(const void* A2, long lda, const float* a_scale, const void* W2, long ldw, const float* w_scale, int Kp,
+                                        const float* bias, void* C, long ldc, int M, int N, int act, int act_col_start, void* split_out,
+                                        long ld_split, int split_kp, int split_col_off, int split_col_start, int paired, float* split_inv,
+                                        const float* bound_par, int global_rows, const psalm_rope_out* rope, void* workspace,
+                                        long workspace_bytes, void* stream) {
+    PSALM_CHECK_ARG(rope && rope->Qr && rope->Kr && rope->cos_table && rope->sin_table, "psalm_gemm_x3_split_rope: Qr, Kr and the cos / sin tables required");
+    PSALM_CHECK_ARG(paired == 1, "psalm_gemm_x3_split_rope: the RoPE epilogue belongs to the paired split-output forms");
+    const long nrot = 64L * rope->heads;
+    PSALM_CHECK_ARG(rope->heads >= 1 && rope->q_col >= 0 && rope->k_col >= 0 && rope->q_col % 64 == 0 && rope->k_col % 64 == 0 &&
+                        rope->q_col + nrot <= split_col_start && rope->k_col + nrot <= split_col_start &&
+                        (rope->q_col + nrot <= rope->k_col || rope->k_col + nrot <= rope->q_col),
+                    "psalm_gemm_x3_split_rope: q / k are heads * 64 columns each, at multiples of 64 below split_col_start, disjoint");
+    PSALM_CHECK_ARG((act & ~15) == 0 && ((act & 15) == 0 || (act_col_start % 256 == 0 && rope->q_col + nrot <= act_col_start &&
+                                                               rope->k_col + nrot <= act_col_start)),
+                    "psalm_gemm_x3_split_rope: q / k columns carry no activation, act_col_start % 256 == 0, no activation flags");
+    PSALM_CHECK_ARG(rope->B >= 1 && rope->L >= 1 && (long)rope->B * rope->L == M && rope->Lp == (rope->L + 31) / 32 * 32 &&
+                        (rope->B == 1 || rope->L >= 32),
+                    "psalm_gemm_x3_split_rope: M == B * L rows, Lp == ceil32(L), L >= 32 when B > 1");
+    PSALM_CHECK_ARG((long)rope->B * rope->heads * rope->Lp * 256 < 0x7ffff000L && (long)rope->L * 128 < 0x7ffff000L,
+                    "psalm_gemm_x3_split_rope: Qr / Kr must stay below 2 GiB each (buffer-descriptor stores)");
+    PSALM_CHECK_ARG(split_col_start % 256 == 0 && (N - split_col_start) % 64 == 0 && (long)M * ld_split * 2 < (1L << 31),
+                    "psalm_gemm_x3_split: paired output needs split_col_start % 256 == 0, (N - split_col_start) % 64 == 0, split_out < 2 GiB");
+    PSALM_CHECK_ARG(split_out && split_inv && bound_par, "psalm_gemm_x3_split: split output, scale array and bound parameters required");
+    PSALM_CHECK_ARG(N % 8 == 0 && split_col_start % 8 == 0 && split_col_start >= 0 && split_col_start < N && split_col_off % 8 == 0 &&
+                        split_col_off >= 0 && split_kp % 8 == 0 && (uintptr_t)split_out % 16 == 0 && (ld_split * 2) % 16 == 0 &&
+                        split_col_off + (N - split_col_start) <= split_kp && ld_split >= 2L * split_kp,
+                    "psalm_gemm_x3_split: N / column offsets multiples of 8, 16-byte aligned split rows of >= 2*split_kp f16");
+    PSALM_CHECK_ARG(C || split_col_start == 0, "psalm_gemm_x3_split: C required for the columns below split_col_start");
+    SplitOut so{split_out, ld_split, split_kp, split_col_off, split_col_start, global_rows, split_inv, bound_par, paired, rope};
+    return gemm_x3_impl(A2, lda, a_scale, W2, ldw, w_scale, Kp, bias, nullptr, 0, C, ldc, M, N, act, act_col_start, workspace, workspace_bytes,
+                        stream, &so, "psalm_gemm_x3_split_rope");
+}
 
 
 extern "C" int psalm_gemm_x3_ln_split(const void* A2, long lda, const float* a_scale, const void* W2, long ldw, const float* w_scale, int Kp,
diff --git a/psalm_amd/csrc/stages.hip b/psalm_amd/csrc/stages.hip
--- a/psalm_amd/csrc/stages.hip
+++ b/psalm_amd/csrc/stages.hip
@@ -35,6 +35,23 @@
 extern "C" long psalm_phi_forward_workspace(const psalm_phi_desc* d, int B, int L) {
     if (phi_check(d) != 0 || B <= 0 || L <= 0) return -1;
     return phi_layout(d, B, L).total;
+}
+
+static bool phi_rope_epilogue(const psalm_phi_desc* d, int B, int L) {
+    const long Lp = (L + 31) / 32 * 32;
+    bool ok = psalm_get_tuning(PSALM_TUNE_PHI_ROPE_EPILOGUE) != 0 && d->head_dim == 64 && d->rot == 32 && (3 * d->hidden) % 256 == 0 &&
+              (B == 1 || L >= 32) && (long)B * d->heads * Lp * 256 < 0x7ffff000L && (long)L * 128 < 0x7ffff000L;
+    for (int i = 0; i < d->num_layers && ok; ++i) ok = d->layers[i].paired == 1;
+    return ok;
+}
+extern "C" int psalm_phi_forward_plan(const psalm_phi_desc* d, int B, int L, int* out3) {
+    if (phi_check(d) != 0) return -1;
+    PSALM_CHECK_ARG(out3 && B > 0 && L > 0, "psalm_phi_forward_plan: null argument");
+    const bool ep = phi_rope_epilogue(d, B, L);
+    out3[0] = ep ? 1 : 0;
+    out3[1] = ep ? 4 : 5;
+    out3[2] = ep ? 2 : 1;
+    return 0;
 }
 
 extern "C" int psalm_phi_forward(const psalm_phi_desc* d, const float* embeds, const unsigned char* key_mask, const float* cos_table,
@@ -57,18 +74,35 @@
     const psalm_phi_layer* l0 = &d->layers[0];
     rc = psalm_layernorm_split(embeds, H, nullptr, H, l0->ln_g, l0->ln_b, M, H, d->ln_eps, h, hinv, nullptr, 0, nullptr, nullptr, stream);
     if (rc) return rc;
+    const int Lp = (L + 31) / 32 * 32;
+    const bool rope_ep = phi_rope_epilogue(d, B, L);
+    const float* Qr = (const float*)attn;
+    const psalm_rope_out rope{(float*)Qr, (float*)Qr + (long)B * d->heads * Lp * 64, cos_table, sin_table, 2 * H, 0, d->heads, B, L, Lp,
+                              1.0f / sqrtf((float)d->head_dim), 0};
+    if (rope_ep) {
+        rc = psalm_phi_attention_tables(key_mask, attn, B, L, d->heads, stream);
+        if (rc) return rc;
+    }
     const float* xin = embeds;
     int cur = 0;
     for (int i = 0; i < d->num_layers; ++i) {
         const psalm_phi_layer* ly = &d->layers[i];
         const bool last = i == d->num_layers - 1;
         PSALM_CHECK_ARG(ly->w1 && ly->w1_scale && ly->b1 && ly->w2 && ly->w2_scale && ly->b2 && ly->bnd, "psalm_phi_forward: layer weights missing");
-        rc = psalm_gemm_x3_split(h, 2L * Kp, hinv, ly->w1, 2L * Kp, ly->w1_scale, Kp, ly->b1, big, 3L * H, M, 3 * H + I,  3, 3 * H, a2,
-                                 2L * K2, K2, H, 3 * H, ly->paired, inv2, ly->bnd, 1, gemm_workspace, gemm_workspace_bytes, stream);
-        if (rc) return rc;
-        rc = psalm_causal_attention_f32_split(big, 3L * H, 2 * H, 0, H, a2, 2L * K2, K2, 0, inv2, cos_table, sin_table, key_mask, attn, B, L, d->heads,
-                                              d->head_dim, d->rot, stream);
-        if (rc) return rc;
+        if (rope_ep) {
+            rc = psalm_gemm_x3_split_rope(h, 2L * Kp, hinv, ly->w1, 2L * Kp, ly->w1_scale, Kp, ly->b1, big, 3L * H, M, 3 * H + I,  3, 3 * H,
+                                          a2, 2L * K2, K2, H, 3 * H, ly->paired, inv2, ly->bnd, 1, &rope, gemm_workspace, gemm_workspace_bytes, stream);
+            if (rc) return rc;
+            rc = psalm_causal_attention_f32_split_prepared(big, 3L * H, H, a2, 2L * K2, K2, 0, inv2, attn, B, L, d->heads, d->head_dim, stream);
+            if (rc) return rc;
+        } else {
+            rc = psalm_gemm_x3_split(h, 2L * Kp, hinv, ly->w1, 2L * Kp, ly->w1_scale, Kp, ly->b1, big, 3L * H, M, 3 * H + I,  3, 3 * H, a2,
+                                     2L * K2, K2, H, 3 * H, ly->paired, inv2, ly->bnd, 1, gemm_workspace, gemm_workspace_bytes, stream);
+            if (rc) return rc;
+            rc = psalm_causal_attention_f32_split(big, 3L * H, 2 * H, 0, H, a2, 2L * K2, K2, 0, inv2, cos_table, sin_table, key_mask, attn, B, L, d->heads,
+                                                  d->head_dim, d->rot, stream);
+            if (rc) return rc;
+        }
         float* xout = x[cur];
         if (last || H % 64 != 0 || H > 2048) {
             rc = psalm_gemm_x3(a2, 2L * K2, inv2, ly->w2, 2L * K2, ly->w2_scale, K2, ly->b2, xin, H, xout, H, M, H, 0, 0, gemm_workspace,
diff --git a/psalm_amd/hip_ops.py b/psalm_amd/hip_ops.py
--- a/psalm_amd/hip_ops.py
+++ b/psalm_amd/hip_ops.py
@@ -36,7 +36,7 @@
         raise PsalmHipError(f"unsupported dtype {t.dtype} (float32 / bfloat16 only)")
 
 
-ABI_VERSION = 15
+ABI_VERSION = 16
 
 
 class _ProfiledLib:
@@ -112,6 +112,11 @@
 class _PhiLayer(ctypes.Structure):
     _fields_ = [("w1", c_void_p), ("w1_scale", c_void_p), ("b1", c_void_p), ("w2", c_void_p), ("w2_scale", c_void_p), ("b2", c_void_p),
                 ("ln_g", c_void_p), ("ln_b", c_void_p), ("bnd", c_void_p), ("paired", c_int)]
+
+
+class _RopeOut(ctypes.Structure):
+    _fields_ = [("Qr", c_void_p), ("Kr", c_void_p), ("cos_table", c_void_p), ("sin_table", c_void_p), ("q_col", c_int), ("k_col", c_int),
+                ("heads", c_int), ("B", c_int), ("L", c_int), ("Lp", c_int), ("scale", c_float), ("pad_", c_int)]
 
 
 class _PhiDesc(ctypes.Structure):
@@ -339,7 +344,7 @@
         return x, SplitF16(so, inv, N), y
 
     def gemm_x3_split(self, a, w, bias, act, split_out, split_inv, bound_par, split_col_off=0, split_col_start=0, act_col_start=0,
-                      out=None, global_rows=False, paired=False):
+                      out=None, global_rows=False, paired=False, rope=None):
         a, w = self._x3_operands(a, w)
         M, N = a.t.shape[0], w.t.shape[0]
         if split_out.dtype != torch.float16 or split_out.dim() != 2 or split_out.shape[0] != M or split_out.stride(1) != 1:
@@ -350,13 +355,24 @@
             raise PsalmHipError("gemm_x3_split: float32 `out` required for the columns below split_col_start")
         if bias is not None and (bias.dtype != torch.float32 or bias.numel() != N):
             raise PsalmHipError("gemm bias must be float32 (N,)")
-        rc = self.lib.psalm_gemm_x3_split(self._p(a.t), c_long(a.t.stride(0)), self._p(a.inv_scale), self._p(w.t), c_long(w.t.stride(0)),
-                                          self._p(w.inv_scale), a.Kp, self._pv(bias), self._pv(out),
-                                          c_long(out.stride(0) if out is not None else 0), M, N, act, act_col_start,
-                                          self._p(split_out), c_long(split_out.stride(0)), split_out.shape[1] // 2, split_col_off,
-                                          split_col_start, int(bool(paired)), self._p(split_inv), self._p(bound_par), int(bool(global_rows)),
-                                          self._p(self._gemm_ws()), c_long(self.GEMM_WS_BYTES), self._stream())
-        self._check(rc, "psalm_gemm_x3_split")
+        head = (self._p(a.t), c_long(a.t.stride(0)), self._p(a.inv_scale), self._p(w.t), c_long(w.t.stride(0)), self._p(w.inv_scale), a.Kp,
+                self._pv(bias), self._pv(out), c_long(out.stride(0) if out is not None else 0), M, N, act, act_col_start, self._p(split_out),
+                c_long(split_out.stride(0)), split_out.shape[1] // 2, split_col_off, split_col_start, int(bool(paired)), self._p(split_inv),
+                self._p(bound_par), int(bool(global_rows)))
+        tail = (self._p(self._gemm_ws()), c_long(self.GEMM_WS_BYTES), self._stream())
+        if rope is not None:
+            B, L, heads = rope["B"], rope["L"], rope["heads"]
+            Lp = (L + 31) // 32 * 32
+            ws = rope["ws"]
+            if ws.dtype != torch.uint8 or ws.numel() < self.causal_attention_workspace_bytes(B, L, heads) or ws.data_ptr() % 16:
+                raise PsalmHipError("gemm_x3_split: rope['ws'] is a causal_attention_workspace(B, L, heads)")
+            ro = _RopeOut(ws.data_ptr(), ws.data_ptr() + B * heads * Lp * 64 * 4, rope["cos"].data_ptr(), rope["sin"].data_ptr(), rope["q_col"],
+                          rope["k_col"], heads, B, L, Lp, 1.0 / math.sqrt(64.0), 0)
+            rc = self.lib.psalm_gemm_x3_split_rope(*head, ctypes.byref(ro), *tail)
+            self._check(rc, "psalm_gemm_x3_split_rope")
+        else:
+            rc = self.lib.psalm_gemm_x3_split(*head, *tail)
+            self._check(rc, "psalm_gemm_x3_split")
         if _DEBUG_BOUNDS or self.debug_bounds:
             self.check_split_bound(split_out, split_col_off, N - split_col_start, "gemm_x3_split")
         return split_out
@@ -752,6 +768,11 @@
     def _pi(t):
         return None if t is None else t.data_ptr()
 
+    def phi_forward_plan(self, desc, B, L):
+        out = (c_int * 3)()
+        self._check(self._cdll_raw.psalm_phi_forward_plan(ctypes.byref(desc), B, L, out), "psalm_phi_forward_plan")
+        return bool(out[0]), out[1], out[2]
+
     def phi_forward(self, desc, embeds, key_mask, cos, sin, B, L):
         if embeds.dtype != torch.float32 or embeds.dim() != 2 or embeds.shape[0] != B * L or embeds.shape[1] != desc.hidden:
             raise PsalmHipError("phi_forward: float32 (B*L, hidden) embeddings")
@@ -847,6 +868,7 @@
         self._check(self.lib.psalm_gemm_x3_set_products(int(n)), "psalm_gemm_x3_set_products")
 
     TUNE_GEMM_XCD_KSPLIT, TUNE_ATTN_XCD_HEADS, TUNE_GEMM_MID, TUNE_DECODER_FUSE, TUNE_ROW_GROUPS, TUNE_MHA_QTILE_WAVES = 0, 1, 2, 3, 4, 5
+    TUNE_PHI_ROPE_EPILOGUE = 6
 
     def set_tuning(self, key: int, value: int):
         self._check(self.lib.psalm_set_tuning(int(key), int(value)), "psalm_set_tuning")
@@ -1106,6 +1128,36 @@
         self._check(rc, "psalm_causal_attention")
         return out
 
+    def causal_attention_workspace_bytes(self, B, L, heads):
+        self.lib.psalm_causal_attention_f32_workspace.restype = c_long
+        return self.lib.psalm_causal_attention_f32_workspace(B, L, heads)
+
+    def causal_attention_workspace(self, B, L, heads):
+        nbytes = self.causal_attention_workspace_bytes(B, L, heads)
+        key = ("causal_f32_ws", nbytes)
+        ws = self._ws.get(key)
+        if ws is None:
+            ws = self._ws[key] = torch.empty(nbytes, dtype=torch.uint8, device=self.device)
+        return ws
+
+    def phi_attention_tables(self, key_mask, ws, B, L, heads):
+        if key_mask.dtype != torch.uint8 or key_mask.numel() != B * L or not key_mask.is_contiguous():
+            raise PsalmHipError("phi_attention_tables: contiguous uint8 key mask (B, L)")
+        if ws.dtype != torch.uint8 or ws.numel() < self.causal_attention_workspace_bytes(B, L, heads):
+            raise PsalmHipError("phi_attention_tables: workspace of causal_attention_workspace(B, L, heads)")
+        self._check(self.lib.psalm_phi_attention_tables(self._p(key_mask), self._p(ws), B, L, heads, self._stream()), "psalm_phi_attention_tables")
+
+    def causal_attention_split_prepared(self, buf, v_off, split_out, split_inv, split_col_off, ws, B, L, heads, head_dim):
+        if buf.dtype != torch.float32 or split_out.dtype != torch.float16 or split_inv.dtype != torch.float32:
+            raise PsalmHipError("causal_attention_split_prepared: float32 v buffer, float16 split buffer, float32 scales")
+        if ws.dtype != torch.uint8 or ws.numel() < self.causal_attention_workspace_bytes(B, L, heads):
+            raise PsalmHipError("causal_attention_split_prepared: workspace of causal_attention_workspace(B, L, heads)")
+        rc = self.lib.psalm_causal_attention_f32_split_prepared(self._pv(buf), c_long(buf.stride(0)), v_off, self._p(split_out),
+                                                                c_long(split_out.stride(0)), split_out.shape[1] // 2, split_col_off,
+                                                                self._p(split_inv), self._p(ws), B, L, heads, head_dim, self._stream())
+        self._check(rc, "psalm_causal_attention_f32_split_prepared")
+        return split_out
+
     def causal_attention_split(self, buf, q_off, k_off, v_off, split_out, split_inv, split_col_off, cos, sin, key_mask, B, L, heads,
                                head_dim, rot):
         if buf.dtype != torch.float32 or split_out.dtype != torch.float16 or split_inv.dtype != torch.float32:
```

Measured after the change: 56.69 images/s, median of 6. +1.4%, better.
